# fbreitwieser/krakenuniq

Hardware: AMD Instinct MI355X
Metric: Mreads/s (150 bp) (higher is better)
Workload: dtype u64

## Files before the change

krakenuniq_amd/csrc/ku_api.cpp:

```cpp
#include "ku_build.h"
#include "ku_ctx.h"

static thread_local std::string g_last_error;
void ku_set_error(const std::string &s) { g_last_error = s; }

extern "C" const char *ku_strerror(int status) {
  switch (status) {
    case KU_OK: return "ok";
    case KU_EINVAL: return "invalid argument";
    case KU_EDATA: return "malformed database / index / taxonomy data";
    case KU_ENOINPUT: return "cannot open input";
    case KU_ENOMEM: return "out of memory";
    case KU_EHIP: return "HIP runtime error or no usable gfx950 device";
    case KU_ESTATE: return "call order violated";
    case KU_EUNSUP: return "not supported by this build";
    default: return "unknown status";
  }
}
extern "C" const char *ku_last_error(void) { return g_last_error.c_str(); }
extern "C" int ku_abi_version(void) { return KU_ABI_VERSION; }
extern "C" int ku_device_count(void) {
  int n = 0;
  if (hipGetDeviceCount(&n) != hipSuccess) return 0;
  return n;
// ... 151 lines not shown
  return n <= cap ? KU_OK : fail(KU_EINVAL, "ku_db_chunk_plan: bounds array too small");
}

int ku_db_raw(const ku_db *db, const uint8_t **pairs, const uint64_t **offsets) {
  if (!db || !pairs || !offsets) return KU_EINVAL;
  *pairs = db->pairs;
  *offsets = db->offsets;
  return KU_OK;
}

extern "C" int ku_db_values(const ku_db *db, uint32_t *out, uint64_t *n) {
  if (!db || !n) return fail(KU_EINVAL, "ku_db_values: null argument");
  std::lock_guard<std::mutex> lk(db->values_mu);
  if (!db->values_ready) {
    const uint64_t np = db->info.key_ct, ps = db->info.key_len + 4, kl = db->info.key_len;
    constexpr uint32_t SMALL = 1u << 26;
    std::vector<std::atomic<uint64_t>> bits(SMALL / 64);
    for (auto &w : bits) w.store(0, std::memory_order_relaxed);
    unsigned nthr = std::max(1u, std::min(16u, std::thread::hardware_concurrency()));
    if (np < (1u << 20)) nthr = 1;
    std::vector<std::vector<uint32_t>> large(nthr);
    std::vector<std::thread> team;
    for (unsigned t = 0; t < nthr; ++t)
      team.emplace_back([&, t] {
        const uint64_t lo = np * t / nthr, hi = np * (t + 1) / nthr;
        uint32_t last = 0;
        for (uint64_t i = lo; i < hi; ++i) {
          uint32_t v;
          memcpy(&v, db->pairs + i * ps + kl, 4);
          if (v == last) continue;
          last = v;
          if (v >= SMALL) {
            large[t].push_back(v);
            if (large[t].size() >= (1u << 20)) {
              std::sort(large[t].begin(), large[t].end());
              large[t].erase(std::unique(large[t].begin(), large[t].end()), large[t].end());
            }
            continue;
          }
          std::atomic<uint64_t> &w = bits[v >> 6];
          const uint64_t m = 1ull << (v & 63);
          if (!(w.load(std::memory_order_relaxed) & m)) w.fetch_or(m, std::memory_order_relaxed);
        }
      });
    for (auto &th : team) th.join();
    std::vector<uint32_t> &vals = db->values;
    for (uint64_t wi = 0; wi < bits.size(); ++wi) {
      uint64_t w = bits[wi].load(std::memory_order_relaxed);
      if (wi == 0) w &= ~1ull;
      while (w) {
        vals.push_back((uint32_t)(wi * 64 + (uint64_t)__builtin_ctzll(w)));
        w &= w - 1;
      }
    }
    const size_t n_small = vals.size();
    for (auto &l : large) vals.insert(vals.end(), l.begin(), l.end());
    std::sort(vals.begin() + n_small, vals.end());
    vals.erase(std::unique(vals.begin() + n_small, vals.end()), vals.end());
    db->values_ready = true;
  }
  const uint64_t count = db->values.size();
  if (out) {
    if (count > *n) return fail(KU_EINVAL, "ku_db_values: output array too small");
    memcpy(out, db->values.data(), count * 4);
  }
  *n = count;
  return KU_OK;
}

extern "C" int ku_tax_open(const char *path, ku_tax **out) {
  if (!path || !out) return fail(KU_EINVAL, "ku_tax_open: null argument");
  *out = nullptr;
  FILE *f = fopen(path, "r");
  if (!f) return fail(KU_ENOINPUT, std::string("unable to open taxonomy index file ") + path);
  ku_tax *t = new ku_tax();
  char *line = nullptr;
  size_t lcap = 0;
  ssize_t ll;
  while ((ll = getline(&line, &lcap, f)) > 0) {
    if (line[ll - 1] == '\n') line[--ll] = 0;
    if (ll == 0) continue;
    char *p = line, *end;
    unsigned long id = strtoul(p, &end, 10);
    if (end == p) continue;
    p = end;
    unsigned long par = strtoul(p, &end, 10);
    if (end == p) continue;
    p = end;
    if (*p) ++p;
    char *tab = strchr(p, '\t');
    std::string name, rank;
    if (tab) { name.assign(p, tab - p); rank.assign(tab + 1); } else name.assign(p);
    if ((uint32_t)id > 1 && id == par) {
      free(line); fclose(f); delete t;
      return fail(KU_EDATA, "taxDB: the parent of " + std::to_string(id) + " is itself");
    }
    t->add((uint32_t)id, (uint32_t)par, name, rank);
  }
  free(line);
  fclose(f);
  t->add(0, 0, "unclassified", "no rank");
  t->finish();
  *out = t;
  return KU_OK;
}

extern "C" int ku_tax_from_arrays(const uint32_t *ids, const uint32_t *parents, uint64_t n, ku_tax **out) {
  if (!out || (n && (!ids || !parents))) return fail(KU_EINVAL, "ku_tax_from_arrays: null argument");
  ku_tax *t = new ku_tax();
  for (uint64_t i = 0; i < n; ++i) t->add(ids[i], parents[i], "", "");
  t->add(0, 0, "unclassified", "no rank");
  t->finish();
  *out = t;
  return KU_OK;
}
extern "C" void ku_tax_close(ku_tax *t) { delete t; }
extern "C" uint64_t ku_tax_size(const ku_tax *t) { return t ? t->ids.size() : 0; }
extern "C" int ku_tax_ids(const ku_tax *t, uint32_t *ids) {
  if (!t || (!ids && !t->ids.empty())) return fail(KU_EINVAL, "ku_tax_ids: null argument");
  if (!t->ids.empty()) memcpy(ids, t->ids.data(), t->ids.size() * 4);
  return KU_OK;
}
extern "C" uint32_t ku_tax_parent(const ku_tax *t, uint32_t taxid) {
  if (!t || taxid == 0) return KU_AMBIG;
  auto it = t->row.find(taxid);
  return it == t->row.end() ? KU_AMBIG : t->parent_map[it->second];
}

hipStream_t ku_ctx_stream_of(ku_ctx *ctx) { return ctx->stream; }
unsigned long long *ku_ctx_exact_unique_of(ku_ctx *ctx) { return ctx->d_exact_unique; }
int ku_ctx_device_of(const ku_ctx *ctx) { return ctx->device; }
int ku_ctx_cus_of(const ku_ctx *ctx) { return ctx->n_cu; }
uint32_t ku_ctx_k_of(const ku_ctx *ctx) { return ctx->m.db.k; }

int ctx_activate(ku_ctx *ctx) {
  if (hipSetDevice(ctx->device) != hipSuccess) return fail(KU_EHIP, "hipSetDevice failed");
  return KU_OK;
}

extern "C" int ku_ctx_create(int device, ku_ctx **out) {
  if (!out) return fail(KU_EINVAL, "ku_ctx_create: null argument");
  *out = nullptr;
  KU_TRY(ku_check_device(device));
  hipDeviceProp_t prop;
  HIP_TRY(hipGetDeviceProperties(&prop, device));
  if (strncmp(prop.gcnArchName, "gfx950", 6) != 0)
    return fail(KU_EHIP, std::string("device is ") + prop.gcnArchName + ", this library is built for gfx950 only");
  ku_ctx *ctx = new ku_ctx();
  ctx->device = device;
  ctx->n_cu = prop.multiProcessorCount > 0 ? prop.multiProcessorCount : 256;
  HIP_TRY(hipSetDevice(device));
  HIP_TRY(hipStreamCreateWithFlags(&ctx->stream, hipStreamNonBlocking));
  HIP_TRY(hipMalloc((void **)&ctx->d_scalar, 128));
  if (const char *e = getenv("KU_LAYOUT")) ctx->hash_layout = strcmp(e, "sorted") != 0;
  if (const char *e = getenv("KU_LOAD_FACTOR")) {
    double f = atof(e);
    if (f >= 0.05 && f <= 0.9) { ctx->load_factor = f; ctx->load_factor_set = true; }
  }
  *out = ctx;
  return KU_OK;
}

void store_free(DbStore &d) {
  if (d.d_table) (void)hipFree(d.d_table);
  if (d.db_owned && d.d_pairs) (void)hipFree(d.d_pairs);
  if (d.offsets_owned && d.d_offsets) (void)hipFree(d.d_offsets);
  d = DbStore{};
}
void ctx_drop_count_cache(ku_ctx *ctx) {
  ctx->count_cache.clear();
  ctx->count_cache_store = ctx->count_cache_pairs = nullptr;
  ctx->count_cache_lines = 0;
}
static void ctx_free_db(ku_ctx *ctx) {
  ctx_drop_count_cache(ctx);
  if (ctx->pf.valid) store_free(ctx->pf.store);
  ctx->pf.valid = false;
  store_free(ctx->m);
  for (DbStore &e : ctx->extra) store_free(e);
  ctx->extra.clear();
  ctx->db_loaded = false;
}
void ctx_free_sparse(ku_ctx *ctx) {
  KuSparseDev &d = ctx->sp.dev;
  for (void *p : {(void *)d.l_key, (void *)d.l_first, (void *)d.u_key, (void *)d.u_distinct, (void *)d.u_last, (void *)d.u_maxfirst,
                  (void *)d.g_key, (void *)d.dense, (void *)d.err, (void *)ctx->sp.d_counters})
    if (p) (void)hipFree(p);
  for (DevBuf *b : {&ctx->sp.unit, &ctx->sp.carry_l, &ctx->sp.carry_u, &ctx->sp.out, &ctx->sp.u_cnt, &ctx->sp.u_flag, &ctx->sp.list, &ctx->sp.tail_row,
                    &ctx->sp.t_seqs, &ctx->sp.t_off, &ctx->sp.t_len, &ctx->sp.t_taxa, &ctx->sp.t_unit})
    b->release();
  ctx->sp = ku_ctx::Sparse{};
}
int sparse_give_up(ku_ctx *ctx, hipStream_t also) {
  (void)ctx_sync_all_streams(ctx);
  if (also) (void)hipStreamSynchronize(also);
  (void)hipGetLastError();
  ctx_free_sparse(ctx);
  ctx->sp.gave_up = true;
  return KU_OK;
}
static void ctx_free_tax(ku_ctx *ctx) {
  for (uint32_t **p : {&ctx->d_node_parent, &ctx->d_node_slot, &ctx->d_node_taxid, &ctx->d_slot_node, &ctx->d_slot_taxid,
                       &ctx->d_slot_anc_off, &ctx->d_slot_anc}) {
    if (*p) (void)hipFree(*p);
    *p = nullptr;
  }
  if (ctx->cnt.registers) (void)hipFree(ctx->cnt.registers);
  if (ctx->cnt.hll_floor) (void)hipFree(ctx->cnt.hll_floor);
  if (ctx->cnt.n_kmers) (void)hipFree(ctx->cnt.n_kmers);
  if (ctx->cnt.n_reads) (void)hipFree(ctx->cnt.n_reads);
  if (ctx->d_exact_set) (void)hipFree(ctx->d_exact_set);
  if (ctx->d_exact_unique) (void)hipFree(ctx->d_exact_unique);
  ctx->d_exact_set = ctx->d_exact_unique = nullptr;
  ctx->exact_mask = 0;
  ctx_free_sparse(ctx);
  ctx->cnt = KuCountsDev{};
  ctx->tax_set = false;
}

int ctx_sync_all_streams(ku_ctx *ctx) {
  int st = KU_OK;
  for (hipStream_t s : {ctx->stream, ctx->k_streams[0], ctx->k_streams[1], ctx->h2d_stream, ctx->d2h_stream, ctx->fetch_stream, ctx->pf.stream})
    if (s && hipStreamSynchronize(s) != hipSuccess && st == KU_OK) st = fail(KU_EHIP, "ku_ctx_synchronize: a stream of the context failed");
  return st;
}

extern "C" void ku_ctx_destroy(ku_ctx *ctx) {
  if (!ctx) return;
  rle_times_print();
  (void)hipSetDevice(ctx->device);
  (void)ctx_sync_all_streams(ctx);
  ctx_free_db(ctx);
  ctx_free_tax(ctx);
  for (DevBuf *b : {&ctx->b_seqs, &ctx->b_off, &ctx->b_len, &ctx->b_calls, &ctx->b_taxa, &ctx->b_hits, &ctx->b_ws, &ctx->b_runs,
                    &ctx->b_roff, &ctx->b_rcnt})
    b->release();
  if (ctx->d_scalar) (void)hipFree(ctx->d_scalar);
  if (ctx->pf.d_scalar) (void)hipFree(ctx->pf.d_scalar);
  if (ctx->pf.stream) (void)hipStreamDestroy(ctx->pf.stream);
  for (RleJob &j : ctx->rle) j.release();
  if (ctx->h2d_stream) (void)hipStreamDestroy(ctx->h2d_stream);
  if (ctx->d2h_stream) (void)hipStreamDestroy(ctx->d2h_stream);
  for (hipStream_t &ks : ctx->k_streams) if (ks) { (void)hipStreamDestroy(ks); ks = nullptr; }
  if (ctx->main_ev) (void)hipEventDestroy(ctx->main_ev);
  if (ctx->fetch_stream) (void)hipStreamDestroy(ctx->fetch_stream);
  if (ctx->stream) (void)hipStreamDestroy(ctx->stream);
  delete ctx;
}

static int store_scan_values(ku_ctx *ctx, DbStore &d) {
  d.values.clear();
  uint32_t *d_bitmap = nullptr, *d_list = nullptr, *d_count = ctx->d_scalar;
  const uint32_t cap = 1u << 24;
  HIP_TRY(hipMalloc((void **)&d_bitmap, 1ull << 29));
  if (hipMalloc((void **)&d_list, (size_t)cap * 4) != hipSuccess) { (void)hipFree(d_bitmap); return fail(KU_ENOMEM, "hipMalloc values list"); }
  int st = KU_OK;
  uint32_t count = 0;
  if (hipMemsetAsync(d_bitmap, 0, 1ull << 29, ctx->stream) != hipSuccess ||
      hipMemsetAsync(d_count, 0, 4, ctx->stream) != hipSuccess)
    st = fail(KU_EHIP, "memset failed");
  if (st == KU_OK) st = ku_launch_mark_values(d.d_pairs, d.db.n_pairs, d_bitmap, ctx->stream);
  if (st == KU_OK) st = ku_launch_collect_values(d_bitmap, d_list, cap, d_count, ctx->stream);
  if (st == KU_OK && hipMemcpyAsync(&count, d_count, 4, hipMemcpyDeviceToHost, ctx->stream) != hipSuccess) st = fail(KU_EHIP, "memcpy failed");
  if (st == KU_OK && hipStreamSynchronize(ctx->stream) != hipSuccess) st = fail(KU_EHIP, "value scan kernel failed");
  if (st == KU_OK && count > cap) st = fail(KU_EUNSUP, "more than 2^24 distinct taxids in the database");
  if (st == KU_OK) {
    d.values.resize(count);
    if (count && hipMemcpy(d.values.data(), d_list, (size_t)count * 4, hipMemcpyDeviceToHost) != hipSuccess) st = fail(KU_EHIP, "memcpy failed");
    std::sort(d.values.begin(), d.values.end());
    if (!d.values.empty() && d.values[0] == 0) d.values.erase(d.values.begin());
  }
  (void)hipFree(d_bitmap);
  (void)hipFree(d_list);
  return st;
}

static void fill_db_dev(DbStore &d, uint64_t n_pairs, uint64_t pair_base, uint32_t k, uint32_t nt, uint32_t idx_type,
                        uint64_t bin_lo, uint64_t bin_hi) {
  d.db.pairs = d.d_pairs;
  d.db.table = nullptr;
  d.db.n_lines = 0;
  d.db.offsets = d.d_offsets;
  d.db.pair_base = pair_base;
  d.db.n_pairs = n_pairs;
  d.db.bin_lo = bin_lo;
  d.db.bin_hi = bin_hi;
  d.db.k = k;
  d.db.nt = nt;
  d.db.xor_mask = idx_type == 1 ? 0u : ku_index2_xor_mask(nt);
}

int store_upload(ku_ctx *ctx, DbStore &d, const ku_db *db, uint64_t bin_lo, uint64_t bin_hi, bool scan_values, hipStream_t stream) {
  if (!stream) stream = ctx->stream;
  const uint64_t p0 = db->offsets[bin_lo], p1 = db->offsets[bin_hi], np = p1 - p0;
  const uint32_t kl = db->info.key_len, ps = kl + 4;
  HIP_TRY(hipMalloc((void **)&d.d_pairs, std::max<uint64_t>(np, 1) * 12));
  d.db_owned = true;
  if (kl == 8) {
    if (np) HIP_TRY(hipMemcpy(d.d_pairs, db->pairs + p0 * 12, np * 12, hipMemcpyHostToDevice));
  } else if (np) {
    void *d_raw = nullptr;
    HIP_TRY(hipMalloc(&d_raw, np * ps));
    hipError_t e = hipMemcpy(d_raw, db->pairs + p0 * ps, np * ps, hipMemcpyHostToDevice);
    int st = e == hipSuccess ? ku_launch_repack((const uint8_t *)d_raw, np, kl, d.d_pairs, stream) : KU_EHIP;
    if (st == KU_OK && hipStreamSynchronize(stream) != hipSuccess) st = KU_EHIP;
    (void)hipFree(d_raw);
    if (st != KU_OK) return fail(st, "pair repack failed");
  }
  const uint64_t no = bin_hi - bin_lo + 1;
  HIP_TRY(hipMalloc((void **)&d.d_offsets, no * 8));
  d.offsets_owned = true;
  HIP_TRY(hipMemcpy(d.d_offsets, db->offsets + bin_lo, no * 8, hipMemcpyHostToDevice));
  fill_db_dev(d, np, p0, db->info.k, db->info.nt, db->info.idx_type, bin_lo, bin_hi);
  return scan_values ? store_scan_values(ctx, d) : KU_OK;
}

extern "C" int ku_ctx_load_db(ku_ctx *ctx, const ku_db *db, uint64_t bin_lo, uint64_t bin_hi) {
  if (!ctx || !db) return fail(KU_EINVAL, "ku_ctx_load_db: null argument");
  KU_TRY(rle_idle(ctx, "ku_ctx_load_db"));
  if (bin_lo > bin_hi || bin_hi > db->info.n_bins) return fail(KU_EINVAL, "bin range out of bounds");
  KU_TRY(ctx_activate(ctx));
  ctx_free_tax(ctx);
  ctx_free_db(ctx);
  KU_TRY(store_upload(ctx, ctx->m, db, bin_lo, bin_hi));
  ctx->db_loaded = true;
  return KU_OK;
}

bool store_whole(const DbStore &d) { return d.db.bin_lo == 0 && d.db.bin_hi == (1ull << (2 * d.db.nt)); }

extern "C" int ku_ctx_add_db(ku_ctx *ctx, const ku_db *db) {
  if (!ctx || !db) return fail(KU_EINVAL, "ku_ctx_add_db: null argument");
  KU_TRY(rle_idle(ctx, "ku_ctx_add_db"));
  if (!ctx->db_loaded) return fail(KU_ESTATE, "load the first database before adding further ones");
  if (ctx->tax_set) return fail(KU_ESTATE, "add every database before the taxonomy is set");
  if (db->info.k != ctx->m.db.k)
    return fail(KU_EINVAL, "different k-mer sizes in the databases: " + std::to_string(ctx->m.db.k) + " vs " + std::to_string(db->info.k));
  if (!store_whole(ctx->m)) return fail(KU_EUNSUP, "hierarchical multi-database runs need the first database resident as a whole");
  if (ctx->extra.size() >= 7) return fail(KU_EUNSUP, "at most 8 databases");
  KU_TRY(ctx_activate(ctx));
  ctx->extra.emplace_back();
  int st = store_upload(ctx, ctx->extra.back(), db, 0, db->info.n_bins);
  if (st != KU_OK) { store_free(ctx->extra.back()); ctx->extra.pop_back(); }
  return st;
}

extern "C" int ku_ctx_adopt_db(ku_ctx *ctx, void *d_pairs, uint64_t n_pairs, const uint64_t *d_offsets, uint32_t k,
                               uint32_t nt, uint32_t idx_type, uint64_t bin_lo, uint64_t bin_hi) {
  if (!ctx || (!d_pairs && n_pairs) || !d_offsets) return fail(KU_EINVAL, "ku_ctx_adopt_db: null argument");
  KU_TRY(rle_idle(ctx, "ku_ctx_adopt_db"));
  if (k < 1 || k > 31 || nt < 1 || nt > 15 || nt > k || (idx_type != 1 && idx_type != 2) || bin_lo > bin_hi ||
      bin_hi > (1ull << (2 * nt)))
    return fail(KU_EINVAL, "ku_ctx_adopt_db: bad geometry");
  KU_TRY(ctx_activate(ctx));
  ctx_free_tax(ctx);
  ctx_free_db(ctx);
  ctx->m.d_pairs = (uint32_t *)d_pairs;
  ctx->m.d_offsets = const_cast<uint64_t *>(d_offsets);
  uint64_t pair_base = 0;
  HIP_TRY(hipMemcpy(&pair_base, d_offsets, 8, hipMemcpyDeviceToHost));
  fill_db_dev(ctx->m, n_pairs, pair_base, k, nt, idx_type, bin_lo, bin_hi);
  ctx->db_loaded = true;
  return store_scan_values(ctx, ctx->m);
}

extern "C" int ku_ctx_db_layout(ku_ctx *ctx, uint32_t *is_hash, uint64_t *resident_bytes) {
  if (!ctx) return fail(KU_EINVAL, "null context");
  if (!ctx->db_loaded) return fail(KU_ESTATE, "no database loaded");
  const bool hash = ctx->m.db.table != nullptr;
  if (is_hash) *is_hash = hash ? 1u : 0u;
  if (resident_bytes)
    *resident_bytes = (hash ? ctx->m.db.n_lines * 128 : ctx->m.db.n_pairs * 12) + (ctx->m.db.bin_hi - ctx->m.db.bin_lo + 1) * 8;
  return KU_OK;
}

static std::vector<uint32_t> ctx_all_values(const ku_ctx *ctx) {
  std::vector<uint32_t> v(ctx->m.values);
  for (const DbStore &e : ctx->extra) v.insert(v.end(), e.values.begin(), e.values.end());
  std::sort(v.begin(), v.end());
  v.erase(std::unique(v.begin(), v.end()), v.end());
  return v;
}

extern "C" int ku_ctx_db_values(ku_ctx *ctx, uint32_t *out, uint64_t *n) {
  if (!ctx || !n) return fail(KU_EINVAL, "ku_ctx_db_values: null argument");
  if (!ctx->db_loaded) return fail(KU_ESTATE, "no database loaded");
  const std::vector<uint32_t> v = ctx_all_values(ctx);
  if (out) {
    if (*n < v.size()) return fail(KU_EINVAL, "output array too small");
    if (!v.empty()) memcpy(out, v.data(), v.size() * 4);
// ... 294 lines not shown
```

krakenuniq_amd/csrc/ku_api_classify.cpp:

```cpp
#include "ku_ctx.h"

int check_ready(ku_ctx *ctx) {
  if (!ctx) return fail(KU_EINVAL, "null context");
  if (!ctx->db_loaded) return fail(KU_ESTATE, "no database loaded");
  if (!ctx->tax_set) return fail(KU_ESTATE, "taxonomy not set");
  return ctx_activate(ctx);
}

extern "C" int ku_lookup_device(ku_ctx *ctx, const void *d_seqs, uint64_t n_bytes, const ku_opts *opts,
                                uint32_t *d_taxa, void *stream) {
  KU_TRY(check_ready(ctx));
  KU_TRY(rle_idle(ctx, "ku_lookup_device"));
  if (n_bytes && (!d_seqs || !d_taxa)) return fail(KU_EINVAL, "ku_lookup_device: null buffer");
  const uint32_t flags = opts ? opts->flags : 0;
  const bool counts = !(flags & (KU_F_NO_COUNTS | KU_F_QUICK));
  hipStream_t s = stream ? (hipStream_t)stream : ctx->stream;
  const size_t nd = 1 + ctx->extra.size();
  for (size_t i = 0; i < nd; ++i) {
    const DbStore &d = i ? ctx->extra[i - 1] : ctx->m;
    int st = ku_launch_lookup(d.db, ctx->cnt, (const uint8_t *)d_seqs, n_bytes, d_taxa, counts && i + 1 == nd, i > 0,
                              (flags & KU_F_MERGE_CHUNK) != 0, ctx->n_cu, s);
    if (st != KU_OK) return fail(st, "lookup kernel launch failed");
  }
  return KU_OK;
}

int ku_ctx_route_info(const ku_ctx *ctx, uint64_t *bin_lo, uint64_t *bin_hi, int *is_hash, int *single_db) {
  if (!ctx || !ctx->db_loaded || !ctx->tax_set) return fail(KU_ESTATE, "no database / taxonomy on this context");
  if (bin_lo) *bin_lo = ctx->m.db.bin_lo;
  if (bin_hi) *bin_hi = ctx->m.db.bin_hi;
  if (is_hash) *is_hash = ctx->m.db.table != nullptr;
  if (single_db) *single_db = ctx->extra.empty();
  return KU_OK;
}
int ku_ctx_route_scan(ku_ctx *ctx, const void *d_seqs, uint64_t n_bytes, uint32_t *d_taxa, const KuRouteDev &rt, hipStream_t s) {
  KU_TRY(check_ready(ctx));
  int st = ku_launch_route_scan(ctx->m.db, (const uint8_t *)d_seqs, n_bytes, d_taxa, rt, ctx->n_cu, s);
  return st == KU_OK ? KU_OK : fail(st, "route scan kernel launch failed");
}
int ku_ctx_route_resolve_prepare(ku_ctx *ctx, const ku_opts *opts, hipStream_t s) {
  KU_TRY(check_ready(ctx));
  const uint32_t flags = opts ? opts->flags : 0;
  const uint32_t max_len = opts ? opts->max_read_len : 0;
  if (max_len == 0 || (flags & (KU_F_QUICK | KU_F_KEEP_SLOTS)) || getenv("KU_NO_FUSED")) return KU_EUNSUP;
  const uint32_t max_n = ku_max_kmers(ctx->m.db.k, max_len);
  if (max_n > ku_route_resolve_max_kmers()) return KU_EUNSUP;
  if (max_n > 128) {
    const uint64_t ws = ku_short_workspace_bytes(std::max(max_n, 193u), ctx->tax.n_slots, ~0ull >> 8, ctx->n_cu);
    if (ws > ctx->b_ws.cap) {
      HIP_TRY(hipStreamSynchronize(s));
      if (ctx->b_ws.reserve(ws) != KU_OK) { (void)hipGetLastError(); return KU_EUNSUP; }
    }
  }
  return KU_OK;
}
int ku_ctx_route_resolve(ku_ctx *ctx, const uint64_t *d_off, const uint32_t *d_len, uint64_t n_reads, const ku_opts *opts, uint32_t *d_calls,
                         uint32_t *d_taxa, uint32_t *d_hits, const uint32_t *d_kb, const uint32_t *d_ret, hipStream_t s) {
  const uint32_t flags = opts ? opts->flags : 0;
  const uint32_t max_len = opts ? opts->max_read_len : 0;
  const uint32_t max_n = ku_max_kmers(ctx->m.db.k, max_len);
  int st = ku_launch_route_resolve(ctx->m.db, ctx->tax, ctx->cnt, d_off, d_len, n_reads, max_n, flags, d_calls, d_taxa, d_hits, d_kb, d_ret,
                                   ctx->b_ws.p, ctx->b_ws.cap, ctx->n_cu, s);
  return st == KU_OK ? KU_OK : fail(st, "routed resolve kernel launch failed");
}
int ku_ctx_route_owner(ku_ctx *ctx, const void *d_rec, uint64_t n_rec, const uint32_t *d_kb, uint32_t *d_slots, bool do_counts, hipStream_t s) {
  KU_TRY(check_ready(ctx));
  int st = ku_launch_route_owner(ctx->m.db, ctx->cnt, d_rec, n_rec, d_kb, d_slots, do_counts, ctx->n_cu, s);
  return st == KU_OK ? KU_OK : fail(st, "route owner kernel launch failed");
}

int ku_exact_owned_step(ku_ctx *ctx, const void *d_seqs, const uint64_t *d_off, const uint32_t *d_len, uint64_t n_reads, uint64_t n_bytes,
                        const ku_opts *opts, uint32_t *d_taxa, hipStream_t s) {
  KU_TRY(check_ready(ctx));
  if (!ctx->d_exact_set) return fail(KU_ESTATE, "exact counting is not enabled on this context");
  if (!ctx->extra.empty()) return fail(KU_EUNSUP, "exact counting on a shard goes with one database");
  ku_opts o = opts ? *opts : ku_opts{0, 1, 0, 0};
  if (o.flags & (KU_F_QUICK | KU_F_NO_COUNTS)) return fail(KU_EUNSUP, "exact counting goes with the plain classification only");
  o.flags |= KU_F_KEEP_SLOTS | KU_F_MERGE_CHUNK;
  HIP_TRY(hipMemsetAsync(d_taxa, 0xFE, n_bytes * 4, s));
  KU_TRY(ku_lookup_device(ctx, d_seqs, n_bytes, &o, d_taxa, s));
  int st = ku_launch_exact(ctx->m.db.k, (const uint8_t *)d_seqs, d_off, d_len, n_reads, d_taxa, ctx->d_exact_set, ctx->exact_mask,
                           ctx->d_exact_unique, ctx->d_scalar + 6, ctx->n_cu, s);
  if (st != KU_OK) return fail(st, "exact counting kernel launch failed");
  return ku_launch_replace_u32(d_taxa, n_bytes, KU_FOREIGN_MARK, 0u, s);
}

extern "C" int ku_lookup_stats_device(ku_ctx *ctx, const void *d_seqs, uint64_t n_bytes, uint64_t *stats_out,
                                      void *stream) {
  KU_TRY(check_ready(ctx));
  KU_TRY(rle_idle(ctx, "ku_lookup_stats_device"));
  if (!stats_out || (n_bytes && !d_seqs)) return fail(KU_EINVAL, "ku_lookup_stats_device: null argument");
  hipStream_t s = stream ? (hipStream_t)stream : ctx->stream;
  unsigned long long *d_stats = (unsigned long long *)(ctx->d_scalar + 8);
  HIP_TRY(hipMemsetAsync(d_stats, 0, 32, s));
  int st = ku_launch_lookup_stats(ctx->m.db, (const uint8_t *)d_seqs, n_bytes, d_stats, ctx->n_cu, s);
  if (st != KU_OK) return fail(st, "stats kernel launch failed");
  HIP_TRY(hipMemcpyAsync(stats_out, d_stats, 32, hipMemcpyDeviceToHost, s));
  HIP_TRY(hipStreamSynchronize(s));
  return KU_OK;
}

extern "C" int ku_resolve_device(ku_ctx *ctx, const void *d_seqs, const uint64_t *d_seq_off, const uint32_t *d_seq_len,
                                 uint64_t n_reads, const ku_opts *opts, uint32_t *d_calls, uint32_t *d_taxa,
                                 uint32_t *d_hits, void *stream) {
  KU_TRY(check_ready(ctx));
  KU_TRY(rle_idle(ctx, "ku_resolve_device"));
  if (n_reads && (!d_seq_off || !d_seq_len || !d_calls || !d_taxa)) return fail(KU_EINVAL, "ku_resolve_device: null buffer");
  const uint32_t flags = opts ? opts->flags : 0;
  if ((flags & KU_F_QUICK) && !d_seqs) return fail(KU_EINVAL, "quick mode needs the sequence buffer");
  hipStream_t s = stream ? (hipStream_t)stream : ctx->stream;
  uint32_t max_len = opts ? opts->max_read_len : 0;
  if (max_len == 0 && n_reads) {
    KU_TRY(ku_launch_max_len(d_seq_len, n_reads, ctx->d_scalar + 4, s));
    HIP_TRY(hipMemcpyAsync(&max_len, ctx->d_scalar + 4, 4, hipMemcpyDeviceToHost, s));
    HIP_TRY(hipStreamSynchronize(s));
  }
  uint64_t ws = (flags & KU_F_QUICK) ? 0 : ku_resolve_workspace_bytes(max_len, ctx->m.db.k, ctx->n_cu);
  if (ws > ctx->b_ws.cap) {
    HIP_TRY(hipStreamSynchronize(s));
    if (ctx->b_ws.reserve(ws) != KU_OK) return fail(KU_ENOMEM, "resolve workspace allocation failed");
  }
  if (ws) HIP_TRY(hipMemsetAsync(ctx->b_ws.p, 0, ws, s));
  int st = ku_launch_resolve(ctx->m.db, ctx->tax, ctx->cnt, (const uint8_t *)d_seqs, d_seq_off, d_seq_len, n_reads, flags,
                             opts ? opts->min_hits : 1, max_len, d_calls, d_taxa, d_hits, ctx->b_ws.p, ctx->b_ws.cap,
                             ctx->n_cu, s);
  return st == KU_OK ? KU_OK : fail(st, "resolve kernel launch failed");
}

int classify_device_impl(ku_ctx *ctx, const void *d_seqs, uint64_t n_bytes, const uint64_t *d_seq_off,
                                const uint32_t *d_seq_len, uint64_t n_reads, const ku_opts *opts, uint32_t *d_calls,
                                uint32_t *d_taxa, uint32_t *d_hits, void *stream, const uint64_t *h_off, const uint32_t *h_len) {
  KU_TRY(check_ready(ctx));
  const uint32_t flags = opts ? opts->flags : 0;
  const bool exact = ctx->d_exact_set != nullptr;
  if (exact && !store_whole(ctx->m)) return fail(KU_EUNSUP, "exact counting on a shard runs through the multi-GPU driver (ku_mgpu_enable_exact)");
  if (exact && (flags & (KU_F_KEEP_SLOTS | KU_F_NO_COUNTS)))
    return fail(KU_EUNSUP, "exact counting goes with a whole classification (no slot output / count-less runs)");
  const bool sparse = ctx->sp.on && !(flags & KU_F_NO_COUNTS);
  if (sparse && !h_len) return fail(KU_EUNSUP, "the sparse-mode emulation runs through the host-buffer entry points (it needs the read lengths on the host)");
  if (sparse && (flags & KU_F_KEEP_SLOTS)) return fail(KU_EUNSUP, "the sparse-mode emulation does not combine with slot output");
  const uint32_t short_max = (getenv("KU_NO_FUSED") || !ctx->extra.empty() || exact || sparse) ? 0 : ku_short_max_kmers(ctx->m.db);
  if (short_max && !(flags & (KU_F_QUICK | KU_F_KEEP_SLOTS)) && n_reads) {
    if (!d_seqs || !d_seq_off || !d_seq_len || !d_calls || !d_taxa) return fail(KU_EINVAL, "ku_classify_batch_device: null buffer");
    hipStream_t s = stream ? (hipStream_t)stream : ctx->stream;
    uint32_t max_len = opts ? opts->max_read_len : 0;
    if (max_len == 0) {
      KU_TRY(ku_launch_max_len(d_seq_len, n_reads, ctx->d_scalar + 4, s));
      HIP_TRY(hipMemcpyAsync(&max_len, ctx->d_scalar + 4, 4, hipMemcpyDeviceToHost, s));
      HIP_TRY(hipStreamSynchronize(s));
    }
    const uint32_t max_n = ku_max_kmers(ctx->m.db.k, max_len);
    bool fused = max_n <= short_max;
    if (!fused && max_n <= ku_short_max_kmers_windowed(ctx->m.db) && !getenv("KU_NO_WINDOWED")) {
      const uint64_t ws = ku_short_workspace_bytes(max_n, ctx->tax.n_slots, n_reads, ctx->n_cu);
      if (ws > ctx->b_ws.cap) HIP_TRY(hipStreamSynchronize(s));
      fused = ctx->b_ws.reserve(ws) == KU_OK;
      if (!fused) (void)hipGetLastError();
    }
    if (fused) {
      int st = ku_launch_classify_short(ctx->m.db, ctx->tax, ctx->cnt, (const uint8_t *)d_seqs, n_bytes, d_seq_off, d_seq_len,
                                        n_reads, max_n, flags, d_calls, d_taxa, d_hits, ctx->b_ws.p, ctx->b_ws.cap, ctx->n_cu, s);
      return st == KU_OK ? KU_OK : fail(st, "fused short-read kernel launch failed");
    }
    ku_opts o = opts ? *opts : ku_opts{0, 1, 0, 0};
    o.max_read_len = max_len;
    KU_TRY(ku_lookup_device(ctx, d_seqs, n_bytes, &o, d_taxa, stream));
    return ku_resolve_device(ctx, d_seqs, d_seq_off, d_seq_len, n_reads, &o, d_calls, d_taxa, d_hits, stream);
  }
  KU_TRY(ku_lookup_device(ctx, d_seqs, n_bytes, opts, d_taxa, stream));
  if (sparse && n_reads) {
    int st = sparse_pass(ctx, d_seqs, d_seq_off, d_seq_len, h_off, h_len, n_reads, n_bytes, d_taxa,
                         (flags & KU_F_QUICK) ? std::max(1u, opts ? opts->min_hits : 1u) : 0u, stream ? (hipStream_t)stream : ctx->stream);
    if (st == KU_ENOMEM) {
      sparse_give_up(ctx, (hipStream_t)stream);
    } else if (st != KU_OK) return st;
  }
  if (exact) {
    if (n_reads && (!d_seqs || !d_seq_off || !d_seq_len || !d_taxa)) return fail(KU_EINVAL, "ku_classify_batch_device: null buffer");
    int st = ku_launch_exact(ctx->m.db.k, (const uint8_t *)d_seqs, d_seq_off, d_seq_len, n_reads, d_taxa, ctx->d_exact_set,
                             ctx->exact_mask, ctx->d_exact_unique, ctx->d_scalar + 6, ctx->n_cu,
                             stream ? (hipStream_t)stream : ctx->stream,
                             (flags & KU_F_QUICK) ? std::max(1u, opts ? opts->min_hits : 1u) : 0u);
    if (st != KU_OK) return fail(st, "exact counting kernel launch failed");
  }
  return ku_resolve_device(ctx, d_seqs, d_seq_off, d_seq_len, n_reads, opts, d_calls, d_taxa, d_hits, stream);
}

extern "C" int ku_classify_batch_device(ku_ctx *ctx, const void *d_seqs, uint64_t n_bytes, const uint64_t *d_seq_off,
                                        const uint32_t *d_seq_len, uint64_t n_reads, const ku_opts *opts,
                                        uint32_t *d_calls, uint32_t *d_taxa, uint32_t *d_hits, void *stream) {
  if (ctx) KU_TRY(rle_idle(ctx, "ku_classify_batch_device"));
  return classify_device_impl(ctx, d_seqs, n_bytes, d_seq_off, d_seq_len, n_reads, opts, d_calls, d_taxa, d_hits, stream, nullptr, nullptr);
}

extern "C" int ku_classify_batch(ku_ctx *ctx, const char *seqs, uint64_t n_bytes, const uint64_t *seq_off,
                                 const uint32_t *seq_len, uint64_t n_reads, const ku_opts *opts, uint32_t *calls,
                                 uint32_t *taxa, uint32_t *hits) {
  KU_TRY(check_ready(ctx));
  KU_TRY(rle_idle(ctx, "ku_classify_batch"));
  if ((n_bytes && !seqs) || (n_reads && (!seq_off || !seq_len || !calls))) return fail(KU_EINVAL, "ku_classify_batch: null buffer");
  if (n_reads == 0) return KU_OK;
  ku_opts o = opts ? *opts : ku_opts{0, 1, 0, 0};
  if (o.max_read_len == 0) for (uint64_t i = 0; i < n_reads; ++i) o.max_read_len = std::max(o.max_read_len, seq_len[i]);
  for (uint64_t i = 0; i < n_reads; ++i)
    if (seq_off[i] + seq_len[i] > n_bytes) return fail(KU_EINVAL, "read " + std::to_string(i) + " exceeds the sequence buffer");
  if (ctx->b_seqs.reserve(n_bytes + 16) || ctx->b_off.reserve(n_reads * 8) || ctx->b_len.reserve(n_reads * 4) ||
      ctx->b_calls.reserve(n_reads * 4) || ctx->b_taxa.reserve((n_bytes + 16) * 4) || ctx->b_hits.reserve(n_reads * 4))
    return fail(KU_ENOMEM, "device batch buffers");
  hipStream_t s = ctx->stream;
  HIP_TRY(hipMemcpyAsync(ctx->b_seqs.p, seqs, n_bytes, hipMemcpyHostToDevice, s));
  HIP_TRY(hipMemcpyAsync(ctx->b_off.p, seq_off, n_reads * 8, hipMemcpyHostToDevice, s));
  HIP_TRY(hipMemcpyAsync(ctx->b_len.p, seq_len, n_reads * 4, hipMemcpyHostToDevice, s));
  KU_TRY(classify_device_impl(ctx, ctx->b_seqs.p, n_bytes, (const uint64_t *)ctx->b_off.p, (const uint32_t *)ctx->b_len.p,
                              n_reads, &o, (uint32_t *)ctx->b_calls.p, (uint32_t *)ctx->b_taxa.p,
                              (uint32_t *)ctx->b_hits.p, s, seq_off, seq_len));
  HIP_TRY(hipMemcpyAsync(calls, ctx->b_calls.p, n_reads * 4, hipMemcpyDeviceToHost, s));
  if (taxa) HIP_TRY(hipMemcpyAsync(taxa, ctx->b_taxa.p, n_bytes * 4, hipMemcpyDeviceToHost, s));
  if (hits) HIP_TRY(hipMemcpyAsync(hits, ctx->b_hits.p, n_reads * 4, hipMemcpyDeviceToHost, s));
  HIP_TRY(hipStreamSynchronize(s));
  return KU_OK;
}

int rle_and_fetch(ku_ctx *ctx, const uint32_t *d_taxa, const uint64_t *d_off, const uint32_t *d_len, uint64_t n_reads,
                         uint64_t runs_cap, bool quick, uint32_t *calls, uint32_t *hits, uint64_t *run_off,
                         uint32_t *run_cnt, uint64_t *n_runs) {
  hipStream_t s = ctx->stream;
  unsigned long long *d_counter = (unsigned long long *)(ctx->d_scalar + 2);
  if (quick) {
    HIP_TRY(hipMemsetAsync(d_counter, 0, 8, s));
    HIP_TRY(hipMemsetAsync(ctx->b_roff.p, 0, n_reads * 8, s));
    HIP_TRY(hipMemsetAsync(ctx->b_rcnt.p, 0, n_reads * 4, s));
  } else {
    KU_TRY(ku_launch_rle(d_taxa, ctx->m.db.k, d_off, d_len, n_reads, runs_cap , ctx->b_runs.p, runs_cap, d_counter,
                         (uint64_t *)ctx->b_roff.p, (uint32_t *)ctx->b_rcnt.p, ctx->n_cu, s));
  }
  unsigned long long total = 0;
  HIP_TRY(hipMemcpyAsync(&total, d_counter, 8, hipMemcpyDeviceToHost, s));
  HIP_TRY(hipMemcpyAsync(calls, ctx->b_calls.p, n_reads * 4, hipMemcpyDeviceToHost, s));
  if (hits) HIP_TRY(hipMemcpyAsync(hits, ctx->b_hits.p, n_reads * 4, hipMemcpyDeviceToHost, s));
  HIP_TRY(hipMemcpyAsync(run_off, ctx->b_roff.p, n_reads * 8, hipMemcpyDeviceToHost, s));
  HIP_TRY(hipMemcpyAsync(run_cnt, ctx->b_rcnt.p, n_reads * 4, hipMemcpyDeviceToHost, s));
  HIP_TRY(hipStreamSynchronize(s));
  if (total > runs_cap) return fail(KU_EHIP, "run-length encoder overflowed its bound");
  *n_runs = ctx->n_runs = total;
  ctx->fetch_runs_src = ctx->b_runs.p;
  ctx->last_calls_dev = ctx->b_calls.p;
  return KU_OK;
}
```

krakenuniq_amd/csrc/ku_api_rle.cpp:

```cpp
#include "ku_ctx.h"


static int sparse_tail_insert(ku_ctx *ctx, const KuSparseDev &d, const std::vector<char> &text, const std::vector<uint32_t> &lens,
                              uint32_t unit, hipStream_t s, uint32_t *pos_end) {
  ku_ctx::Sparse &sp = ctx->sp;
  const uint64_t n_reads = lens.size(), n_bytes = text.size();
  if (pos_end) *pos_end = (uint32_t)n_bytes;
  if (n_reads == 0) return KU_OK;
  std::vector<uint64_t> off(n_reads);
  uint64_t at = 0;
  for (uint64_t r = 0; r < n_reads; ++r) { off[r] = at; at += (uint64_t)lens[r] + 1; }
  if (at != n_bytes) return fail(KU_ESTATE, "sparse-mode emulation: the open unit's reads are inconsistent");
  if (sp.t_seqs.reserve(n_bytes + 16) || sp.t_off.reserve(n_reads * 8) || sp.t_len.reserve(n_reads * 4) || sp.t_taxa.reserve((n_bytes + 16) * 4) ||
      sp.t_unit.reserve(n_reads * 4))
    return fail(KU_ENOMEM, "device memory for the open work unit's reads");
  HIP_TRY(hipMemcpyAsync(sp.t_seqs.p, text.data(), n_bytes, hipMemcpyHostToDevice, s));
  HIP_TRY(hipMemcpyAsync(sp.t_off.p, off.data(), n_reads * 8, hipMemcpyHostToDevice, s));
  HIP_TRY(hipMemcpyAsync(sp.t_len.p, lens.data(), n_reads * 4, hipMemcpyHostToDevice, s));
  std::vector<uint32_t> units(n_reads, unit);
  HIP_TRY(hipMemcpyAsync(sp.t_unit.p, units.data(), n_reads * 4, hipMemcpyHostToDevice, s));
  HIP_TRY(hipStreamSynchronize(s));
  int st = ku_launch_lookup(ctx->m.db, ctx->cnt, (const uint8_t *)sp.t_seqs.p, n_bytes, (uint32_t *)sp.t_taxa.p, false, false, false,
                            ctx->n_cu, s);
  if (st != KU_OK) return fail(st, "lookup kernel launch failed");
// ... 58 lines not shown
    HIP_TRY(hipMemcpyAsync(&c, sp.d_counters, 8, hipMemcpyDeviceToHost, s));
    HIP_TRY(hipMemcpyAsync(&err, sp.dev.err, 4, hipMemcpyDeviceToHost, s));
    HIP_TRY(hipStreamSynchronize(s));
    if (err) return fail(KU_ENOMEM, "sparse-mode emulation: a device table is full");
    sp.g_count = c;
  }
  sp.tail_open = false;
  sp.tail_text.clear();
  sp.tail_len.clear();
  return KU_OK;
}

struct RleTimes {
  double t[10] = {};
  double x[6] = {};
  double kernel_ms = 0;
  double kernel_sum_ms = 0, cover_end = 0;
  unsigned long long reads = 0;
  static inline const bool on = getenv("KU_RLE_TIMES") != nullptr;
  static inline hipEvent_t ref = nullptr;
  static double now() { timespec ts; clock_gettime(CLOCK_MONOTONIC, &ts); return (double)ts.tv_sec + 1e-9 * (double)ts.tv_nsec; }
  struct Lap {
    double &slot;
    const double t0 = on ? now() : 0.0;
    ~Lap() { if (on) slot += now() - t0; }
  };
  void count_finish() { if (on) t[4] += 1; }
  void count_exact_pass(double units, double n_reads) { if (on) { x[2] += 1; x[3] += units; x[4] += n_reads; } }
  void add_kernels(hipEvent_t k0, hipEvent_t k1, uint64_t n_reads) {
    float ms = 0, a = 0, b = 0;
    if (ref && hipEventElapsedTime(&ms, k0, k1) == hipSuccess && hipEventElapsedTime(&a, ref, k0) == hipSuccess &&
        hipEventElapsedTime(&b, ref, k1) == hipSuccess) {
      kernel_sum_ms += ms;
      kernel_ms += std::max(0.0, (double)b - std::max((double)a, cover_end));
      cover_end = std::max(cover_end, (double)b);
      reads += n_reads;
    } else (void)hipGetLastError();
  }
  void print() const {
    if (on && t[4] > 0)
      fprintf(stderr, "ku_classify_batch_rle over %.0f batches: checks %.3f s, plan + enqueue %.3f s, waiting for the device %.3f s, behind the wait %.3f s; "
                      "kernels %.3f ms for %llu reads (HIP events on their streams: the time the batches' intervals cover; their sum is %.3f ms); of the enqueue: buffers + plan %.3f s, uploads %.3f s, launches %.3f s, "
                      "copies back + events %.3f s; of buffers + plan: room in the emulation's run-wide set %.3f s\n",
              t[4], t[0], t[1], t[2], t[3], kernel_ms, reads, kernel_sum_ms, t[5], t[6], t[7], t[8], t[9]);
    if (on && x[2] > 0)
      fprintf(stderr, "ku_classify_batch_rle, behind the wait: flagging again %.3f s, %.0f exact passes over %.0f work units (%.0f reads) %.3f s, of it %.3f s waiting for their kernels\n", x[0], x[2],
              x[3], x[4], x[1], x[5]);
  }
};
static RleTimes g_rle;
void rle_times_print() { g_rle.print(); }

static int sparse_fast_exact(ku_ctx *ctx, RleJob &j, const std::vector<uint32_t> &flagged, const std::vector<uint8_t> &flag_all,
                             bool last_is_open, hipStream_t s) {
  ku_ctx::Sparse &sp = ctx->sp;
  const uint32_t *h_len = j.b.seq_len;
  const std::vector<uint64_t> &unit_first_read = j.unit_first_read;
  const uint32_t *d_u_cnt = (const uint32_t *)j.u_cnt.p;
  const void *d_runs = j.runs_in_ctx ? ctx->b_runs.p : j.runs.p;
  const uint64_t *d_roff = (const uint64_t *)(j.runs_in_ctx ? ctx->b_roff.p : j.roff.p);
  const uint32_t *d_rcnt = (const uint32_t *)(j.runs_in_ctx ? ctx->b_rcnt.p : j.rcnt.p);
  const bool with_tail = j.cont_tail && !flagged.empty() && flagged[0] == 0 && !j.tail_len.empty();
  const uint64_t tail_bytes = with_tail ? j.tail_text.size() : 0;
  size_t at = 0;
  bool first_pass = true;
  while (at < flagged.size()) {
    size_t end = at;
    uint64_t bases = first_pass ? tail_bytes : 0, n_list = 0;
    while (end < flagged.size() && end - at < KU_SPARSE_MAX_UNITS) {
      const uint32_t u = flagged[end];
      uint64_t ub = 0;
      for (uint64_t r = unit_first_read[u]; r < unit_first_read[u + 1]; ++r) ub += h_len[r];
      if (end > at && bases + ub > (1ull << 25)) break;
      bases += ub;
      n_list += unit_first_read[u + 1] - unit_first_read[u];
      ++end;
    }
    const bool has_open = last_is_open && end == flagged.size();
    std::vector<uint32_t> list(3 * n_list);
    uint64_t li = 0;
    for (size_t f = at; f < end; ++f) {
      const uint32_t u = flagged[f];
      for (uint64_t r = unit_first_read[u]; r < unit_first_read[u + 1]; ++r, ++li) {
        list[li] = (uint32_t)r;
        list[n_list + li] = (uint32_t)(f - at) | (flag_all[f] ? 0x80000000u : 0u);
        list[2 * n_list + li] = u;
      }
    }
    if (sp.list.reserve(std::max<uint64_t>(n_list, 1) * 12) != KU_OK) return fail(KU_ENOMEM, "device memory for the flagged work units' reads");
    KU_TRY(sparse_reserve_global(ctx, bases + sp.n_carry_l, s));
    KuSparseDev d;
    KU_TRY(sparse_pass_tables(ctx, bases + sp.n_carry_l + sp.n_carry_u, &d, s));
    if (first_pass && j.cont_carry)
      KU_TRY(ku_launch_sparse_carry_in(d, (const unsigned long long *)sp.carry_l.p, sp.n_carry_l, (const uint32_t *)sp.carry_u.p, sp.n_carry_u, s));
    uint32_t pos_base = 0;
    if (first_pass && with_tail) KU_TRY(sparse_tail_insert(ctx, d, j.tail_text, j.tail_len, 0u, s, &pos_base));
    if (n_list) HIP_TRY(hipMemcpyAsync(sp.list.p, list.data(), n_list * 12, hipMemcpyHostToDevice, s));
    const uint32_t *dl = (const uint32_t *)sp.list.p;
    KU_TRY(ku_launch_sparse_insert_runs(d, ctx->m.db.k, (const uint8_t *)j.seqs.p, (const uint64_t *)j.off.p, (const uint32_t *)j.len.p,
                                        dl, dl + n_list, dl + 2 * n_list, n_list, d_runs, d_roff, d_rcnt, ctx->d_slot_taxid, ctx->tax.n_slots,
                                        d_u_cnt, ctx->n_cu, s, pos_base));
    const uint32_t n_local = (uint32_t)(end - at);
    KU_TRY(ku_launch_sparse_close(d, has_open ? n_local - 1 : n_local, s, !j.cont_carry));
    if (first_pass && j.cont_carry) sp.n_carry_l = sp.n_carry_u = 0;
    unsigned long long c[3] = {0, 0, 0};
    if (has_open) {
      HIP_TRY(hipMemsetAsync(sp.d_counters + 1, 0, 16, s));
      KU_TRY(ku_launch_sparse_carry_out(d, n_local - 1, (unsigned long long *)sp.carry_l.p, (uint32_t *)sp.carry_u.p, sp.d_counters + 1,
                                        sp.cap_carry_l, sp.cap_carry_u, s));
    }
    HIP_TRY(hipMemcpyAsync(c, sp.d_counters, 24, hipMemcpyDeviceToHost, s));
    { RleTimes::Lap lap{g_rle.x[5]}; HIP_TRY(hipStreamSynchronize(s)); }
    sp.g_count = std::max<uint64_t>(sp.g_count, c[0]);
    if (has_open) {
      sp.n_carry_l = std::min<uint64_t>(c[1], sp.cap_carry_l);
      sp.n_carry_u = std::min<uint64_t>(c[2], sp.cap_carry_u);
    }
    first_pass = false;
    at = end;
  }
  return KU_OK;
}

static bool rle_fused_eligible(ku_ctx *ctx, uint32_t flags, uint32_t max_n, uint64_t n_bytes, uint64_t n_reads, bool monotonic) {
  if (getenv("KU_NO_FUSED") || getenv("KU_NO_FUSED_RLE") || !ctx->extra.empty() || ctx->d_exact_set) return false;
  if (flags & (KU_F_QUICK | KU_F_KEEP_SLOTS)) return false;
  const uint32_t short_max = ku_short_max_kmers(ctx->m.db);
  if (!short_max) return false;
  if (max_n > short_max && (max_n > ku_short_max_kmers_windowed(ctx->m.db) || getenv("KU_NO_WINDOWED"))) return false;
  if (n_reads >= (1ull << 32)) return false;
  const bool sparse = ctx->sp.on && !(flags & KU_F_NO_COUNTS);
  if (sparse) {
    const ku_ctx::Sparse &sp = ctx->sp;
    if (getenv("KU_NO_SPARSE_FAST") || !monotonic || sp.unit_nt == 0 || sp.unit_nt > (1ull << 24) || n_bytes + (1ull << 26) >= (1ull << 32)) return false;
    const uint64_t max_units = n_bytes / sp.unit_nt + 2;
    if (max_units * ctx->tax.n_slots > (1ull << 29)) return false;
  }
  return true;
}

static uint64_t rle_workspace_bytes(const ku_ctx *ctx, uint32_t max_n, uint64_t n_reads) {
  if (max_n <= ku_short_max_kmers(ctx->m.db) || max_n > ku_short_max_kmers_windowed(ctx->m.db)) return 0;
  return ku_short_workspace_bytes(max_n, ctx->tax.n_slots, n_reads, ctx->n_cu);
}

struct RlePlan {
  std::vector<uint64_t> seg;
  uint64_t total_waves = 0;
  uint32_t chunk = 0;
  uint64_t runs_cap = 0;
  uint64_t ws = 0;
  uint64_t n_seg() const { return seg.size() - 1; }
};
static RlePlan rle_plan(const ku_ctx *ctx, uint64_t n_bytes, uint64_t n_reads, uint32_t max_n, const uint64_t *seq_off, bool test_hook) {
  RlePlan p;
  uint64_t n_seg = 1;
  constexpr uint64_t seg_bytes = 16ull << 20;
  if (seq_off && !getenv("KU_NO_H2D_OVERLAP")) n_seg = std::min<uint64_t>(8, std::max<uint64_t>(1, n_bytes / seg_bytes));
  p.seg.assign(n_seg + 1, 0);
  for (uint64_t g = 1; g < n_seg; ++g) {
    const uint64_t target = n_bytes / n_seg * g;
    p.seg[g] = std::max<uint64_t>(p.seg[g - 1], (uint64_t)(std::lower_bound(seq_off, seq_off + n_reads, target) - seq_off));
  }
  p.seg[n_seg] = n_reads;
  uint64_t max_seg_reads = 0;
  for (uint64_t g = 0; g < n_seg; ++g) {
    p.total_waves += ku_short_grid_waves(p.seg[g + 1] - p.seg[g], max_n, ctx->n_cu);
    max_seg_reads = std::max(max_seg_reads, p.seg[g + 1] - p.seg[g]);
  }
  const uint64_t reads_per_wave = n_reads / std::max<uint64_t>(p.total_waves, 1);
  p.chunk = reads_per_wave >= 64 ? 256u : (reads_per_wave >= 16 ? 64u : 16u);
  p.runs_cap = n_bytes / 6 + 4 * n_reads + p.total_waves * p.chunk + 4096;
  if (const char *e = test_hook ? getenv("KU_RUNS_CAP") : nullptr) p.runs_cap = std::max<uint64_t>(1, (uint64_t)atoll(e));
  p.ws = rle_workspace_bytes(ctx, max_n, max_seg_reads);
  return p;
}

int rle_idle(const ku_ctx *ctx, const char *who) {
  if (ctx->rle_in_flight) return fail(KU_ESTATE, std::string(who) + ": batches are in flight (ku_classify_batch_rle_finish first)");
  return KU_OK;
}

extern "C" uint64_t ku_device_rle_runs_cap(const ku_ctx *ctx, uint64_t n_bytes, uint64_t n_reads, uint32_t max_read_len) {
  if (!ctx || !ctx->tax_set) return 0;
  return rle_plan(ctx, n_bytes, n_reads, ku_max_kmers(ctx->m.db.k, max_read_len), nullptr, false).runs_cap;
}

extern "C" int ku_classify_batch_device_rle(ku_ctx *ctx, const void *d_seqs, uint64_t n_bytes, const uint64_t *d_seq_off,
                                            const uint32_t *d_seq_len, uint64_t n_reads, const ku_opts *opts, uint32_t *d_calls,
                                            ku_run *d_runs, uint64_t runs_cap, uint64_t *d_run_off, uint32_t *d_run_cnt,
                                            uint64_t *d_n_runs, void *stream) {
  KU_TRY(check_ready(ctx));
  KU_TRY(rle_idle(ctx, "ku_classify_batch_device_rle"));
  if (!d_n_runs || (n_reads && (!d_seqs || !d_seq_off || !d_seq_len || !d_calls || !d_runs || !d_run_off || !d_run_cnt)))
    return fail(KU_EINVAL, "ku_classify_batch_device_rle: null buffer");
  const ku_opts o = opts ? *opts : ku_opts{0, 1, 0, 0};
  hipStream_t s = stream ? (hipStream_t)stream : ctx->stream;
  HIP_TRY(hipMemsetAsync(d_n_runs, 0, 8, s));
  if (n_reads == 0) return KU_OK;
  if (o.max_read_len == 0) return fail(KU_EINVAL, "ku_classify_batch_device_rle: opts->max_read_len (the longest read of the batch) is required");
  const uint32_t max_n = ku_max_kmers(ctx->m.db.k, o.max_read_len);
  if (ctx->sp.on && !(o.flags & KU_F_NO_COUNTS))
    return fail(KU_EUNSUP, "the sparse-mode emulation runs through the host-buffer entry points (it needs the read lengths on the host)");
  if (!store_whole(ctx->m) || !rle_fused_eligible(ctx, o.flags, max_n, n_bytes, n_reads, true))
    return fail(KU_EUNSUP, "ku_classify_batch_device_rle: the fused kernel does not apply to this context / these options (ku_classify_batch_device does)");
  const RlePlan p = rle_plan(ctx, n_bytes, n_reads, max_n, nullptr, false);
  if (p.ws > ctx->b_ws.cap) HIP_TRY(hipStreamSynchronize(s));
  if (ctx->b_ws.reserve(p.ws)) return fail(KU_ENOMEM, "device memory for the windowed kernel's workspace");
  KuRunsOut ro{};
  ro.runs = (uint2 *)d_runs;
  ro.counter = (unsigned long long *)d_n_runs;
  ro.cap = runs_cap;
  ro.chunk = p.chunk;
  ro.run_off = d_run_off;
  ro.run_cnt = d_run_cnt;
  if (p.total_waves * p.chunk <= runs_cap && p.total_waves * p.chunk < (1ull << 31)) {
    HIP_TRY(hipMemsetD32Async((hipDeviceptr_t)d_n_runs, (int)(p.total_waves * p.chunk), 1, s));
    ro.pre_base1 = 1;
  }
  int st = ku_launch_classify_short(ctx->m.db, ctx->tax, ctx->cnt, (const uint8_t *)d_seqs, n_bytes, d_seq_off, d_seq_len, n_reads, max_n, o.flags,
                                    d_calls, nullptr, nullptr, ctx->b_ws.p, ctx->b_ws.cap, ctx->n_cu, s, &ro, nullptr);
  return st == KU_OK ? KU_OK : fail(st, "fused kernel launch failed");
}


static int plan_work_units(ku_ctx *ctx, RleJob &j, const RleBatch &b, bool sparse) {
  const ku_ctx::Sparse &sp = ctx->sp;
  j.sparse = sparse;
  j.cont_carry = j.cont_tail = j.open_after = false;
  j.n_units = 0;
  j.kmers = 0;
  j.unit_first_read.clear();
  j.tail_text.clear();
  j.tail_len.clear();
  if (!sparse) return KU_OK;
  if (j.pin_unit.reserve(b.n_reads * 4)) return fail(KU_ENOMEM, "page-locked memory for the work-unit plan");
  uint32_t *h_unit = (uint32_t *)j.pin_unit.p;
  uint64_t acc = sp.acc_nt;
  uint32_t cur = 0;
  j.cont_carry = sp.open;
  j.cont_tail = sp.tail_open && !sp.open;
  j.unit_first_read.push_back(0);
  for (uint64_t r = 0; r < b.n_reads; ++r) {
    h_unit[r] = cur;
    acc += b.seq_len[r];
    if (acc >= sp.unit_nt) { ++cur; acc = 0; j.unit_first_read.push_back(r + 1); }
  }
  j.open_after = acc > 0;
  j.acc_after = acc;
  j.n_units = cur + (j.unit_first_read.back() < b.n_reads ? 1u : 0u);
  if (j.unit_first_read.back() < b.n_reads) j.unit_first_read.push_back(b.n_reads);
  for (uint64_t r = 0; r < b.n_reads; ++r) j.kmers += ku_max_kmers(ctx->m.db.k, b.seq_len[r]);
  return KU_OK;
}

static int sparse_fast_view(ku_ctx *ctx, RleJob &j, KuSparseFast *sf) {
  ku_ctx::Sparse &sp = ctx->sp;
  uint64_t in_flight_kmers = 0;
  for (const RleJob &q : ctx->rle) if (q.busy && &q != &j && q.sparse) in_flight_kmers += q.kmers;
  { RleTimes::Lap lap{g_rle.t[9]}; KU_TRY(sparse_reserve_global(ctx, j.kmers + in_flight_kmers + sp.n_carry_l, ctx->stream)); }
  sf->g_key = sp.dev.g_key;
  sf->g_mask = sp.dev.g_mask;
  sf->g_count = sp.dev.g_count;
  sf->dense = sp.dev.dense;
  sf->u_cnt = (uint32_t *)j.u_cnt.p;
  sf->err = sp.dev.err;
  sf->n_slots = ctx->tax.n_slots;
  sf->unit_base = 0;
  ctx->m.seen_dirty = true;
  return KU_OK;
}

static int queue_uploads_and_launches(ku_ctx *ctx, RleJob &j, const RleBatch &b, const RlePlan &p, hipStream_t s, KuSparseFast *sf, bool *clock_started) {
  const bool sparse = sf != nullptr;
  unsigned long long *h_tot = (unsigned long long *)j.pin.p;
  const uint32_t *h_unit = (const uint32_t *)j.pin_unit.p;
  HIP_TRY(hipEventRecord(ctx->main_ev, ctx->stream));
  HIP_TRY(hipStreamWaitEvent(s, ctx->main_ev, 0));
  unsigned long long *d_counter = j.d_counter;
  if (sparse) {
    if (ku_launch_zero3(d_counter, 2, j.u_cnt.p, std::max<uint64_t>((uint64_t)j.n_units * ctx->tax.n_slots, 1), j.u_flag.p,
                        ((uint64_t)std::max<uint32_t>(j.n_units, 1) + 3) / 4, s) != KU_OK)
      return fail(KU_EHIP, "clearing the batch counters failed");
  }
  h_tot[3] = p.total_waves * (unsigned long long)p.chunk;
  HIP_TRY(hipMemcpyAsync(d_counter, &h_tot[3], 8, hipMemcpyHostToDevice, s));
  KuRunsOut ro{};
  ro.runs = (uint2 *)j.runs.p;
  ro.counter = d_counter;
  ro.cap = p.runs_cap;
  ro.chunk = p.chunk;
  if (RleTimes::on) { KU_TRY(ensure_event(j.t_k0, hipEventDefault)); KU_TRY(ensure_event(j.t_k1, hipEventDefault)); }
  uint64_t waves_before = 0;
  for (uint64_t g = 0; g < p.n_seg(); ++g) {
    const uint64_t a = p.seg[g], e = p.seg[g + 1];
    const uint64_t lo = g == 0 ? 0 : b.seq_off[a], hi = g + 1 == p.n_seg() ? b.n_bytes : b.seq_off[e];
    hipStream_t cs = ctx->h2d_stream;
    {
      RleTimes::Lap lap{g_rle.t[6]};
      if (hi > lo) HIP_TRY(hipMemcpyAsync((char *)j.seqs.p + lo, b.seqs + lo, hi - lo, hipMemcpyHostToDevice, cs));
      if (e > a) {
        HIP_TRY(hipMemcpyAsync((uint64_t *)j.off.p + a, b.seq_off + a, (e - a) * 8, hipMemcpyHostToDevice, cs));
        HIP_TRY(hipMemcpyAsync((uint32_t *)j.len.p + a, b.seq_len + a, (e - a) * 4, hipMemcpyHostToDevice, cs));
        if (sparse) HIP_TRY(hipMemcpyAsync((uint32_t *)j.unit.p + a, h_unit + a, (e - a) * 4, hipMemcpyHostToDevice, cs));
      }
      HIP_TRY(hipEventRecord(j.seg_events[g], cs));
      HIP_TRY(hipStreamWaitEvent(s, j.seg_events[g], 0));
    }
    if (e == a) continue;
    RleTimes::Lap lap{g_rle.t[7]};
    ro.run_off = (uint64_t *)j.roff.p + a;
    ro.run_cnt = (uint32_t *)j.rcnt.p + a;
    ro.pre_base1 = (uint32_t)(1 + waves_before);
    waves_before += ku_short_grid_waves(e - a, b.max_n, ctx->n_cu);
    if (sparse) sf->unit_of = (const uint32_t *)j.unit.p + a;
    if (RleTimes::on && !*clock_started) {
      if (!RleTimes::ref) { KU_TRY(ensure_event(RleTimes::ref, hipEventDefault)); HIP_TRY(hipEventRecord(RleTimes::ref, s)); }
      HIP_TRY(hipEventRecord(j.t_k0, s));
      *clock_started = true;
    }
    int st = ku_launch_classify_short(ctx->m.db, ctx->tax, ctx->cnt, (const uint8_t *)j.seqs.p, b.n_bytes, (const uint64_t *)j.off.p + a,
                                      (const uint32_t *)j.len.p + a, e - a, b.max_n, b.o.flags, (uint32_t *)j.calls.p + a, nullptr, nullptr,
                                      j.ws.p, j.ws.cap, ctx->n_cu, s, &ro, sf);
    if (st != KU_OK) { (void)hipStreamSynchronize(ctx->h2d_stream); (void)hipStreamSynchronize(s); return fail(st, "fused kernel launch failed"); }
  }
  return KU_OK;
}

static int queue_open_unit_step(ku_ctx *ctx, RleJob &j, hipStream_t s) {
  ku_ctx::Sparse &sp = ctx->sp;
  if (ctx->prev_kernels_done) HIP_TRY(hipStreamWaitEvent(s, ctx->prev_kernels_done, 0));
  if (j.cont_tail && j.n_units)
    KU_TRY(ku_launch_add_u32((uint32_t *)j.u_cnt.p, (const uint32_t *)sp.tail_row.p, ctx->tax.n_slots, s));
  KU_TRY(ku_launch_sparse_flag_units((const uint32_t *)j.u_cnt.p, (uint64_t)j.n_units * ctx->tax.n_slots, ctx->tax.n_slots, sp.dev.dense,
                                     (uint8_t *)j.u_flag.p, s));
  if (j.open_after && !(j.cont_carry && j.n_units == 1))
    HIP_TRY(hipMemcpyAsync(sp.tail_row.p, (const uint32_t *)j.u_cnt.p + (size_t)(j.n_units - 1) * ctx->tax.n_slots, (size_t)ctx->tax.n_slots * 4,
                           hipMemcpyDeviceToDevice, s));
  return KU_OK;
}

static int queue_copies_back(ku_ctx *ctx, RleJob &j, const RleBatch &b, uint64_t runs_cap, hipStream_t s) {
  unsigned long long *h_tot = (unsigned long long *)j.pin.p;
  const hipStream_t ds = ctx->d2h_stream;
  HIP_TRY(hipEventRecord(j.kernels_done, s));
  ctx->prev_kernels_done = j.kernels_done;
  HIP_TRY(hipStreamWaitEvent(ds, j.kernels_done, 0));
  HIP_TRY(hipMemcpyAsync(b.calls, j.calls.p, b.n_reads * 4, hipMemcpyDeviceToHost, ds));
  HIP_TRY(hipMemcpyAsync(b.run_off, j.roff.p, b.n_reads * 8, hipMemcpyDeviceToHost, ds));
  HIP_TRY(hipMemcpyAsync(b.run_cnt, j.rcnt.p, b.n_reads * 4, hipMemcpyDeviceToHost, ds));
  HIP_TRY(hipMemcpyAsync(&h_tot[0], j.d_counter, 8, hipMemcpyDeviceToHost, ds));
  j.runs_copied = b.runs ? std::min<uint64_t>(b.runs_cap, runs_cap) : 0;
  if (j.runs_copied) HIP_TRY(hipMemcpyAsync(b.runs, j.runs.p, j.runs_copied * 8, hipMemcpyDeviceToHost, ds));
  if (j.sparse) {
    HIP_TRY(hipMemcpyAsync((uint8_t *)j.pin.p + 64, j.u_flag.p, std::max<uint32_t>(j.n_units, 1), hipMemcpyDeviceToHost, ds));
    HIP_TRY(hipMemcpyAsync(&h_tot[1], ctx->sp.dev.g_count, 8, hipMemcpyDeviceToHost, ds));
    HIP_TRY(hipMemcpyAsync(&h_tot[2], ctx->sp.dev.err, 4, hipMemcpyDeviceToHost, ds));
  }
  HIP_TRY(hipEventRecord(j.done, ds));
  return KU_OK;
}

static void advance_emulation_state(ku_ctx::Sparse &sp, RleJob &j, const RleBatch &b) {
  const bool whole_batch_one_open_unit = j.n_units == 1 && j.open_after;
  if (j.cont_tail && !whole_batch_one_open_unit) {
    j.tail_text.swap(sp.tail_text);
    j.tail_len.swap(sp.tail_len);
    sp.tail_text.clear();
    sp.tail_len.clear();
  }
  if (j.cont_carry && whole_batch_one_open_unit) {
  } else if (j.open_after) {
    if (!(j.cont_tail && whole_batch_one_open_unit)) { sp.tail_text.clear(); sp.tail_len.clear(); }
    sparse_tail_append(sp, b.seqs, b.seq_off, b.seq_len, j.unit_first_read[j.n_units - 1], b.n_reads);
    sp.tail_open = true;
    sp.open = false;
  } else {
    sp.tail_open = false;
    sp.open = false;
    sp.tail_text.clear();
    sp.tail_len.clear();
  }
  sp.acc_nt = j.acc_after;
}

static int rle_job_enqueue(ku_ctx *ctx, RleJob &j, const RleBatch &b) {
  RleTimes::Lap lap_all{g_rle.t[1]};
  hipStream_t &ks = ctx->k_streams[(&j - &ctx->rle[0]) & 1];
  KU_TRY(ensure_stream(ks));
  KU_TRY(ensure_event(ctx->main_ev));
  const hipStream_t s = ks;
  const bool sparse = ctx->sp.on && !(b.o.flags & KU_F_NO_COUNTS);
  RlePlan p;
  KuSparseFast sf{};
  {
    RleTimes::Lap lap{g_rle.t[5]};
    p = rle_plan(ctx, b.n_bytes, b.n_reads, b.max_n, b.monotonic ? b.seq_off : nullptr, true);
    KU_TRY(plan_work_units(ctx, j, b, sparse));
    KU_TRY(j.reserve(b.n_bytes, b.n_reads, p.runs_cap, p.ws, p.n_seg(), sparse, j.n_units, ctx->tax.n_slots));
    KU_TRY(ensure_stream(ctx->h2d_stream));
    KU_TRY(ensure_stream(ctx->d2h_stream));
    if (sparse) {
      if (ctx->sp.tail_row.reserve((size_t)ctx->tax.n_slots * 4)) return fail(KU_ENOMEM, "device memory for the work-unit counters");
      KU_TRY(sparse_fast_view(ctx, j, &sf));
    }
  }
  bool clock_started = false;
  KU_TRY(queue_uploads_and_launches(ctx, j, b, p, s, sparse ? &sf : nullptr, &clock_started));
  {
    RleTimes::Lap lap{g_rle.t[8]};
    if (sparse) KU_TRY(queue_open_unit_step(ctx, j, s));
    if (clock_started) HIP_TRY(hipEventRecord(j.t_k1, s));
    KU_TRY(queue_copies_back(ctx, j, b, p.runs_cap, s));
  }
  if (sparse && j.n_units) advance_emulation_state(ctx->sp, j, b);
  j.b = b;
  j.runs_cap = p.runs_cap;
  j.settled = false;
  j.runs_in_ctx = false;
  j.busy = true;
  return KU_OK;
}

static int rle_job_finish(ku_ctx *ctx, RleJob &j, uint64_t *n_runs, bool *classified) {
  hipStream_t s = ctx->stream;
  *classified = false;
  ctx->last_runs_copied = 0;
  if (j.settled) {
    j.busy = false;
    *n_runs = ctx->n_runs = j.n_runs;
    *classified = true;
    return KU_OK;
  }
  { RleTimes::Lap lap{g_rle.t[2]}; HIP_TRY(hipEventSynchronize(j.done)); }
  RleTimes::Lap lap_rest{g_rle.t[3]};
  g_rle.count_finish();
  if (RleTimes::on && j.t_k0 && j.b.n_reads) g_rle.add_kernels(j.t_k0, j.t_k1, j.b.n_reads);
  j.busy = false;
  ku_ctx::Sparse &sp = ctx->sp;
  const unsigned long long *h_tot = (const unsigned long long *)j.pin.p;
  const uint8_t *h_flag = (const uint8_t *)j.pin.p + 64;
  const unsigned long long total = h_tot[0];
  if (j.b.hits) memset(j.b.hits, 0, j.b.n_reads * 4);
  ctx->last_calls_dev = j.calls.p;
  if (total > j.runs_cap) {
    if (ctx->b_taxa.reserve((j.b.n_bytes + 16) * 4) || ctx->b_runs.reserve((j.b.n_bytes + 1) * 8) || ctx->b_roff.reserve(j.b.n_reads * 8) ||
        ctx->b_rcnt.reserve(j.b.n_reads * 4) || ctx->b_calls.reserve(j.b.n_reads * 4))
      return fail(KU_ENOMEM, "device batch buffers");
    if (ctx->b_ws.reserve(rle_workspace_bytes(ctx, j.b.max_n, j.b.n_reads))) return fail(KU_ENOMEM, "device batch buffers");
    int st = ku_launch_classify_short(ctx->m.db, ctx->tax, ctx->cnt, (const uint8_t *)j.seqs.p, j.b.n_bytes, (const uint64_t *)j.off.p,
                                      (const uint32_t *)j.len.p, j.b.n_reads, j.b.max_n, j.b.o.flags | KU_F_NO_COUNTS, (uint32_t *)ctx->b_calls.p,
                                      (uint32_t *)ctx->b_taxa.p, nullptr, ctx->b_ws.p, ctx->b_ws.cap, ctx->n_cu, s);
    if (st != KU_OK) return fail(st, "fused kernel launch failed");
    KU_TRY(rle_and_fetch(ctx, (const uint32_t *)ctx->b_taxa.p, (const uint64_t *)j.off.p, (const uint32_t *)j.len.p, j.b.n_reads, j.b.n_bytes + 1,
                         false, j.b.calls, nullptr, j.b.run_off, j.b.run_cnt, n_runs));
    j.runs_in_ctx = true;
  } else {
    *n_runs = ctx->n_runs = total;
    ctx->fetch_runs_src = j.runs.p;
    ctx->last_runs_copied = j.runs_copied;
  }
  *classified = true;
  if (j.sparse && sp.on) {
    if ((uint32_t)h_tot[2]) return fail(KU_ENOMEM, "sparse-mode emulation: the run-wide set is full");
    sp.g_count = std::max<uint64_t>(sp.g_count, h_tot[1]);
    std::vector<uint32_t> flagged;
    std::vector<uint8_t> flag_all;
    const bool carry_stays_open = j.cont_carry && j.n_units == 1 && j.open_after;
    bool any_flag = false;
    for (uint32_t u = 0; u < j.n_units; ++u) any_flag |= !(u + 1 == j.n_units && j.open_after) && h_flag[u];
    {
      RleTimes::Lap lap{g_rle.x[0]};
      if (any_flag && !getenv("KU_NO_REFLAG")) {
        KU_TRY(ensure_stream(ctx->fetch_stream));
        hipStream_t fs = ctx->fetch_stream;
        const size_t fb = ((size_t)j.n_units + 3) & ~(size_t)3;
        HIP_TRY(hipMemsetAsync(j.u_flag.p, 0, fb, fs));
        KU_TRY(ku_launch_sparse_flag_units((const uint32_t *)j.u_cnt.p, (uint64_t)j.n_units * ctx->tax.n_slots, ctx->tax.n_slots, sp.dev.dense,
                                           (uint8_t *)j.u_flag.p, fs));
        HIP_TRY(hipMemcpyAsync((uint8_t *)j.pin.p + 64, j.u_flag.p, j.n_units, hipMemcpyDeviceToHost, fs));
        HIP_TRY(hipStreamSynchronize(fs));
      }
      for (uint32_t u = 0; u < j.n_units; ++u) {
        const bool open = u + 1 == j.n_units && j.open_after;
        if (u == 0 && j.cont_carry) { flagged.push_back(u); flag_all.push_back(1); }
        else if (!open && h_flag[u]) { flagged.push_back(u); flag_all.push_back(0); }
      }
    }
    if (!flagged.empty()) {
      RleTimes::Lap lap{g_rle.x[1]};
      for (const RleJob &q : ctx->rle)
        if (q.busy && q.kernels_done) HIP_TRY(hipStreamWaitEvent(s, q.kernels_done, 0));
      KU_TRY(sparse_fast_exact(ctx, j, flagged, flag_all, carry_stays_open, s));
      uint64_t n_flagged_reads = 0;
      for (uint32_t u : flagged) n_flagged_reads += j.unit_first_read[u + 1] - j.unit_first_read[u];
      g_rle.count_exact_pass((double)flagged.size(), (double)n_flagged_reads);
    }
  }
  return KU_OK;
}

int rle_drain_batches(ku_ctx *ctx) {
  for (RleJob &q : ctx->rle)
    if (q.busy && q.done) HIP_TRY(hipEventSynchronize(q.done));
  return KU_OK;
}

static RleJob &rle_next_job(ku_ctx *ctx) {
  RleJob &j = ctx->rle[(ctx->rle_head + ctx->rle_in_flight) % KU_RLE_MAX_IN_FLIGHT];
  static const int counter_at[KU_RLE_MAX_IN_FLIGHT] = {26, 20, 22, 24};
  if (!j.d_counter) j.d_counter = (unsigned long long *)(ctx->d_scalar + counter_at[&j - &ctx->rle[0]]);
  return j;
}

static int rle_check_batch(RleBatch &b) {
  if ((b.n_bytes && !b.seqs) || (b.n_reads && (!b.seq_off || !b.seq_len || !b.calls || !b.run_off || !b.run_cnt)))
    return fail(KU_EINVAL, "ku_classify_batch_rle: null buffer");
  b.o.flags &= ~KU_F_KEEP_SLOTS;
  RleTimes::Lap lap{g_rle.t[0]};
  if (b.o.max_read_len == 0) for (uint64_t i = 0; i < b.n_reads; ++i) b.o.max_read_len = std::max(b.o.max_read_len, b.seq_len[i]);
  b.monotonic = true;
  for (uint64_t i = 0; i < b.n_reads; ++i) {
    if (b.seq_off[i] + b.seq_len[i] > b.n_bytes) return fail(KU_EINVAL, "read " + std::to_string(i) + " exceeds the sequence buffer");
    if (i && b.seq_off[i] < b.seq_off[i - 1] + b.seq_len[i - 1]) b.monotonic = false;
  }
  return KU_OK;
}

static int rle_staged_batch(ku_ctx *ctx, const RleBatch &b, uint64_t *n_runs) {
  const uint64_t n_bytes = b.n_bytes, n_reads = b.n_reads;
  const uint64_t runs_cap = n_bytes + 1;
  if (ctx->b_seqs.reserve(n_bytes + 16) || ctx->b_off.reserve(n_reads * 8) || ctx->b_len.reserve(n_reads * 4) ||
      ctx->b_calls.reserve(n_reads * 4) || ctx->b_taxa.reserve((n_bytes + 16) * 4) || ctx->b_hits.reserve(n_reads * 4) ||
      ctx->b_runs.reserve(runs_cap * 8) || ctx->b_roff.reserve(n_reads * 8) || ctx->b_rcnt.reserve(n_reads * 4))
    return fail(KU_ENOMEM, "device batch buffers");
  hipStream_t s = ctx->stream;
  HIP_TRY(hipMemcpyAsync(ctx->b_seqs.p, b.seqs, n_bytes, hipMemcpyHostToDevice, s));
  HIP_TRY(hipMemcpyAsync(ctx->b_off.p, b.seq_off, n_reads * 8, hipMemcpyHostToDevice, s));
  HIP_TRY(hipMemcpyAsync(ctx->b_len.p, b.seq_len, n_reads * 4, hipMemcpyHostToDevice, s));
  KU_TRY(classify_device_impl(ctx, ctx->b_seqs.p, n_bytes, (const uint64_t *)ctx->b_off.p, (const uint32_t *)ctx->b_len.p,
                              n_reads, &b.o, (uint32_t *)ctx->b_calls.p, (uint32_t *)ctx->b_taxa.p,
                              (uint32_t *)ctx->b_hits.p, s, b.seq_off, b.seq_len));
  return rle_and_fetch(ctx, (const uint32_t *)ctx->b_taxa.p, (const uint64_t *)ctx->b_off.p, (const uint32_t *)ctx->b_len.p, n_reads,
                       runs_cap, (b.o.flags & KU_F_QUICK) != 0, b.calls, b.hits, b.run_off, b.run_cnt, n_runs);
}

static void rle_warm_up(ku_ctx *ctx, uint64_t n_reads) {
  (void)ku_launch_warm_scratch(ctx->n_cu, ctx->stream);
  const RleTimes keep = g_rle;
  const uint64_t wn = (std::min<uint64_t>(std::max<uint64_t>(n_reads, 1), 65536) + 1) & ~1ull, stride = 101;
  const size_t per_slot = (size_t)wn * (4 + 4 + 4 + 8) + (size_t)wn * 8 * 8;
  PinBuf w;
  if (w.reserve((size_t)wn * (stride + 12) + KU_RLE_MAX_IN_FLIGHT * per_slot + 4096) == 0) {
    memset(w.p, 0, w.cap);
    char *text = (char *)w.p;
    uint64_t *w_off = (uint64_t *)(text + ((wn * stride + 63) & ~63ull));
    uint32_t *w_len = (uint32_t *)(w_off + wn);
    char *slots = (char *)(w_len + wn);
    for (uint64_t r = 0; r < wn; ++r) {
      char *t = text + r * stride;
      for (int i = 0; i < 100; ++i) t[i] = "ACGTTGCAAGCTTCGA"[(i * 7 + i / 16 + r) & 15];
      t[100] = '\n';
      w_off[r] = r * stride;
      w_len[r] = 100;
    }
    const ku_opts wo = {KU_F_NO_COUNTS, 1, 100, 0};
    uint64_t w_runs = 0;
    int flying = 0;
    for (int rep = 0; rep < 12; ++rep) {
      if (flying == 3) { (void)ku_classify_batch_rle_finish(ctx, &w_runs); --flying; }
      char *sl = slots + (size_t)(rep % KU_RLE_MAX_IN_FLIGHT) * per_slot;
      uint64_t *roff = (uint64_t *)sl;
      uint32_t *calls = (uint32_t *)(roff + wn), *hits = calls + wn, *rcnt = hits + wn;
      ku_run *runs = (ku_run *)(rcnt + wn);
      if (ku_classify_batch_rle_enqueue(ctx, text, wn * stride, w_off, w_len, wn, &wo, calls, hits, roff, rcnt, runs, wn * 8) == KU_OK) ++flying;
    }
    while (flying-- > 0) (void)ku_classify_batch_rle_finish(ctx, &w_runs);
    if (ctx->fetch_stream) {
      (void)hipMemcpyAsync(w.p, ctx->rle[0].seqs.p, std::min<size_t>(ctx->rle[0].seqs.cap, 1u << 20), hipMemcpyDeviceToHost, ctx->fetch_stream);
      (void)hipStreamSynchronize(ctx->fetch_stream);
    }
    (void)hipDeviceSynchronize();
    w.release();
  }
  (void)hipGetLastError();
  g_rle = keep;
}

extern "C" int ku_classify_batch_rle_reserve(ku_ctx *ctx, uint64_t n_bytes, uint64_t n_reads, uint32_t max_read_len, uint32_t n_jobs) {
  KU_TRY(check_ready(ctx));
  KU_TRY(rle_idle(ctx, "ku_classify_batch_rle_reserve"));
  if (!ku_short_max_kmers(ctx->m.db)) return KU_OK;
  KU_TRY(ensure_stream(ctx->h2d_stream));
  KU_TRY(ensure_stream(ctx->d2h_stream));
  KU_TRY(ensure_stream(ctx->fetch_stream));
  const RlePlan p = rle_plan(ctx, n_bytes, n_reads, ku_max_kmers(ctx->m.db.k, max_read_len), nullptr, false);
  const bool sparse = ctx->sp.on && ctx->sp.unit_nt;
  const uint64_t n_units = sparse ? n_bytes / ctx->sp.unit_nt + 2 : 0;
  for (uint32_t q = 0; q < std::min<uint32_t>(n_jobs, KU_RLE_MAX_IN_FLIGHT); ++q)
    KU_TRY(ctx->rle[q].reserve(n_bytes, n_reads, p.runs_cap, p.ws, 2, sparse, n_units, ctx->tax.n_slots));
  if (sparse && ctx->sp.tail_row.reserve((size_t)ctx->tax.n_slots * 4)) return fail(KU_ENOMEM, "device memory for the work-unit counters");
  if (!getenv("KU_NO_WARMUP")) rle_warm_up(ctx, n_reads);
  return KU_OK;
}

extern "C" int ku_classify_batch_rle_in_flight(const ku_ctx *ctx) { return ctx ? ctx->rle_in_flight : 0; }
extern "C" uint64_t ku_classify_batch_rle_copied(const ku_ctx *ctx) { return ctx ? ctx->last_runs_copied : 0; }

static int rle_run_job(ku_ctx *ctx, RleJob &j, const RleBatch &b, bool to_end, uint64_t *n_runs) {
  for (int attempt = 0;; ++attempt) {
    bool classified = false;
    int st = rle_job_enqueue(ctx, j, b);
    if (to_end && st == KU_OK) st = rle_job_finish(ctx, j, n_runs, &classified);
    if (to_end) j.busy = false;
    if (st != KU_ENOMEM || attempt || !(ctx->sp.on && !(b.o.flags & KU_F_NO_COUNTS))) return st;
    sparse_give_up(ctx);
    if (classified) return KU_OK;
  }
}

extern "C" int ku_classify_batch_rle_enqueue(ku_ctx *ctx, const char *seqs, uint64_t n_bytes, const uint64_t *seq_off,
                                             const uint32_t *seq_len, uint64_t n_reads, const ku_opts *opts, uint32_t *calls,
                                             uint32_t *hits, uint64_t *run_off, uint32_t *run_cnt, ku_run *runs, uint64_t runs_cap) {
  KU_TRY(check_ready(ctx));
  if (ctx->rle_in_flight >= KU_RLE_MAX_IN_FLIGHT)
    return fail(KU_ESTATE, "ku_classify_batch_rle_enqueue: " + std::to_string(KU_RLE_MAX_IN_FLIGHT) + " batches are in flight (ku_classify_batch_rle_finish first)");
  RleBatch b{seqs, n_bytes, seq_off, seq_len, n_reads, opts ? *opts : ku_opts{0, 1, 0, 0}, 0, true, calls, hits, run_cnt, run_off, runs, runs_cap};
  KU_TRY(rle_check_batch(b));
  b.max_n = ku_max_kmers(ctx->m.db.k, b.o.max_read_len);
  RleJob &j = rle_next_job(ctx);
  const bool fused = n_reads && rle_fused_eligible(ctx, b.o.flags, b.max_n, n_bytes, n_reads, b.monotonic);
  const bool in_steps = fused && !(ctx->sp.on && !(b.o.flags & KU_F_NO_COUNTS) && ctx->sp.open);
  if (in_steps) {
    KU_TRY(rle_run_job(ctx, j, b, false, nullptr));
    ++ctx->rle_in_flight;
    return KU_OK;
  }
  if (ctx->rle_in_flight) return fail(KU_ESTATE, "ku_classify_batch_rle_enqueue: this batch takes a path that cannot overlap with the batch in flight "
                                                 "(ku_classify_batch_rle_finish first, then enqueue it again)");
  uint64_t nr = 0;
  ctx->n_runs = 0;
  if (fused) KU_TRY(rle_run_job(ctx, j, b, true, &nr));
  else if (n_reads) {
    KU_TRY(rle_staged_batch(ctx, b, &nr));
    j.runs_in_ctx = true;
  }
  j.settled = true;
  j.busy = true;
  j.n_runs = nr;
  j.runs_copied = 0;
  ++ctx->rle_in_flight;
  return KU_OK;
}

extern "C" int ku_classify_batch_rle_finish(ku_ctx *ctx, uint64_t *n_runs) {
  if (!ctx || !n_runs) return fail(KU_EINVAL, "ku_classify_batch_rle_finish: null argument");
  *n_runs = 0;
  if (!ctx->rle_in_flight) return fail(KU_ESTATE, "ku_classify_batch_rle_finish: no batch is in flight");
  KU_TRY(ctx_activate(ctx));
  RleJob &j = ctx->rle[ctx->rle_head];
  ctx->rle_head = (ctx->rle_head + 1) % KU_RLE_MAX_IN_FLIGHT;
  --ctx->rle_in_flight;
  bool classified = false;
  int st = rle_job_finish(ctx, j, n_runs, &classified);
  j.busy = false;
  if (st == KU_ENOMEM && classified && ctx->sp.on) st = sparse_give_up(ctx);
  return st;
}

extern "C" int ku_classify_batch_rle(ku_ctx *ctx, const char *seqs, uint64_t n_bytes, const uint64_t *seq_off,
                                     const uint32_t *seq_len, uint64_t n_reads, const ku_opts *opts, uint32_t *calls,
                                     uint32_t *hits, uint64_t *run_off, uint32_t *run_cnt, uint64_t *n_runs) {
  if (!n_runs) return fail(KU_EINVAL, "ku_classify_batch_rle: null buffer");
  *n_runs = 0;
  KU_TRY(check_ready(ctx));
  KU_TRY(rle_idle(ctx, "ku_classify_batch_rle"));
  KU_TRY(ku_classify_batch_rle_enqueue(ctx, seqs, n_bytes, seq_off, seq_len, n_reads, opts, calls, hits, run_off, run_cnt, nullptr, 0));
  return ku_classify_batch_rle_finish(ctx, n_runs);
}

extern "C" int ku_ctx_replace_calls(ku_ctx *ctx, const uint32_t *new_calls, uint64_t n_reads, uint64_t *n_dropped) {
  KU_TRY(check_ready(ctx));
  if (n_dropped) *n_dropped = 0;
  if (n_reads == 0) return KU_OK;
  if (!new_calls) return fail(KU_EINVAL, "ku_ctx_replace_calls: null argument");
  KU_TRY(rle_idle(ctx, "ku_ctx_replace_calls"));
  if (!ctx->last_calls_dev) return fail(KU_ESTATE, "ku_ctx_replace_calls: the context holds no batch");
  if (ctx->b_hits.reserve(n_reads * 4) != KU_OK) return fail(KU_ENOMEM, "device batch buffers");
  hipStream_t s = ctx->stream;
  unsigned long long *d_dropped = (unsigned long long *)(ctx->d_scalar + 16);
  HIP_TRY(hipMemsetAsync(d_dropped, 0, 8, s));
  HIP_TRY(hipMemcpyAsync(ctx->b_hits.p, new_calls, n_reads * 4, hipMemcpyHostToDevice, s));
  KU_TRY(ku_launch_replace_calls((const uint32_t *)ctx->last_calls_dev, (const uint32_t *)ctx->b_hits.p, n_reads, ctx->d_node_taxid, ctx->tax.n_nodes,
                                 ctx->cnt.n_reads, d_dropped, s));
  HIP_TRY(hipMemcpyAsync((void *)ctx->last_calls_dev, ctx->b_hits.p, n_reads * 4, hipMemcpyDeviceToDevice, s));
  unsigned long long dropped = 0;
  HIP_TRY(hipMemcpyAsync(&dropped, d_dropped, 8, hipMemcpyDeviceToHost, s));
  HIP_TRY(hipStreamSynchronize(s));
  if (n_dropped) *n_dropped = dropped;
  return KU_OK;
}

extern "C" int ku_fetch_runs(ku_ctx *ctx, ku_run *runs, uint64_t n_runs) {
  if (!ctx) return fail(KU_EINVAL, "ku_fetch_runs: null context");
  if (n_runs > ctx->n_runs) return fail(KU_EINVAL, "ku_fetch_runs: the last batch holds " + std::to_string(ctx->n_runs) + " runs");
  if (n_runs == 0) return KU_OK;
  if (!runs) return fail(KU_EINVAL, "ku_fetch_runs: null buffer");
  if (!ctx->fetch_runs_src) return fail(KU_ESTATE, "ku_fetch_runs: no batch was classified");
  KU_TRY(ctx_activate(ctx));
  if (!ctx->fetch_stream) HIP_TRY(hipStreamCreateWithFlags(&ctx->fetch_stream, hipStreamNonBlocking));
  HIP_TRY(hipMemcpyAsync(runs, ctx->fetch_runs_src, n_runs * 8, hipMemcpyDeviceToHost, ctx->fetch_stream));
  HIP_TRY(hipStreamSynchronize(ctx->fetch_stream));
  return KU_OK;
}
```

krakenuniq_amd/csrc/ku_ctx.h:

```cpp
#pragma once
#include <fcntl.h>
#include <sys/mman.h>
#include <sys/stat.h>
#include <time.h>
#include <unistd.h>

#include <algorithm>
#include <atomic>
#include <mutex>
#include <thread>
#include <cstdio>
#include <cstdlib>
#include <cstring>
#include <string>
#include <unordered_map>
#include <vector>

#include "ku_host.h"
#include "ku_internal.h"

void ku_set_error(const std::string &s);
static inline int fail(int code, const std::string &msg) {
  ku_set_error(msg);
  return code;
// ... 9 lines not shown
  do {                          \
    int s_ = (expr);            \
    if (s_ != KU_OK) return s_; \
  } while (0)

static inline int ensure_stream(hipStream_t &s) { if (!s) HIP_TRY(hipStreamCreateWithFlags(&s, hipStreamNonBlocking)); return KU_OK; }
static inline int ensure_event(hipEvent_t &e, unsigned flags = hipEventDisableTiming) { if (!e) HIP_TRY(hipEventCreateWithFlags(&e, flags)); return KU_OK; }
static inline uint32_t ku_max_kmers(uint32_t k, uint32_t len) { return len >= k ? len - k + 1 : 0; }

struct ku_db {
  const uint8_t *pairs = nullptr;
  const uint64_t *offsets = nullptr;
  ku_db_info info{};
  void *map_kdb = nullptr, *map_idx = nullptr;
  size_t map_kdb_sz = 0, map_idx_sz = 0;
  mutable std::mutex values_mu;
  mutable std::vector<uint32_t> values;
  mutable bool values_ready = false;
};

struct DevBuf {
  void *p = nullptr;
  size_t cap = 0;
  int reserve(size_t bytes) {
    if (bytes <= cap) return KU_OK;
    if (p) (void)hipFree(p);
    p = nullptr; cap = 0;
    size_t want = bytes + bytes / 4 + 256;
    if (hipMalloc(&p, want) != hipSuccess) {
      if (hipMalloc(&p, bytes) != hipSuccess) { p = nullptr; return KU_ENOMEM; }
      want = bytes;
    }
    cap = want;
    return KU_OK;
  }
  void release() { if (p) (void)hipFree(p); p = nullptr; cap = 0; }
};

struct PinBuf {
  void *p = nullptr;
  size_t cap = 0;
  int reserve(size_t bytes) {
    if (bytes <= cap) return KU_OK;
    if (p) (void)hipHostFree(p);
    p = nullptr; cap = 0;
    const size_t want = bytes + bytes / 4 + 256;
    if (hipHostMalloc(&p, want, hipHostMallocDefault) != hipSuccess) { (void)hipGetLastError(); p = nullptr; return KU_ENOMEM; }
    cap = want;
    return KU_OK;
  }
  void release() { if (p) (void)hipHostFree(p); p = nullptr; cap = 0; }
};

struct RleBatch {
  const char *seqs;
  uint64_t n_bytes;
  const uint64_t *seq_off;
  const uint32_t *seq_len;
  uint64_t n_reads;
  ku_opts o;
  uint32_t max_n;
  bool monotonic;
  uint32_t *calls, *hits, *run_cnt;
  uint64_t *run_off;
  ku_run *runs;
  uint64_t runs_cap;
};

struct RleJob {
  DevBuf seqs, off, len, calls, runs, roff, rcnt, ws, unit, u_cnt, u_flag;
  PinBuf pin;
  PinBuf pin_unit;
  unsigned long long *d_counter = nullptr;
  hipEvent_t kernels_done = nullptr, done = nullptr;
  hipEvent_t t_k0 = nullptr, t_k1 = nullptr;
  std::vector<hipEvent_t> seg_events;
  bool busy = false;
  bool settled = false;
  bool runs_in_ctx = false;
  uint64_t runs_copied = 0;
  uint64_t n_runs = 0;
  RleBatch b{};
  uint64_t runs_cap = 0;
  bool sparse = false;
  bool cont_carry = false;
  bool cont_tail = false;
  bool open_after = false;
  uint32_t n_units = 0;
  uint64_t kmers = 0;
  uint64_t acc_after = 0;
  std::vector<uint64_t> unit_first_read;
  std::vector<char> tail_text;
  std::vector<uint32_t> tail_len;
  int reserve(uint64_t n_bytes, uint64_t n_reads, uint64_t runs_cap_, uint64_t ws_bytes, size_t n_seg, bool sparse_, uint64_t units, uint64_t n_slots) {
    if (seqs.reserve(n_bytes + 16) || off.reserve(n_reads * 8) || len.reserve(n_reads * 4) || calls.reserve(n_reads * 4) ||
        runs.reserve(runs_cap_ * 8) || roff.reserve(n_reads * 8) || rcnt.reserve(n_reads * 4) || ws.reserve(ws_bytes))
      return fail(KU_ENOMEM, "device batch buffers");
    units = std::max<uint64_t>(units, 1);
    if (sparse_ && (pin_unit.reserve(n_reads * 4) || unit.reserve(n_reads * 4) || u_cnt.reserve(std::max<uint64_t>(units * n_slots, 1) * 4) ||
                    u_flag.reserve((units + 3) & ~3ull)))
      return fail(KU_ENOMEM, "device memory for the work-unit counters");
    if (pin.reserve(64 + (size_t)units + 64)) return fail(KU_ENOMEM, "page-locked memory for the batch totals");
    KU_TRY(ensure_event(done));
    KU_TRY(ensure_event(kernels_done));
    seg_events.resize(std::max(seg_events.size(), n_seg), nullptr);
    for (hipEvent_t &e : seg_events) KU_TRY(ensure_event(e));
    return KU_OK;
  }
  void release() {
    for (DevBuf *d : {&seqs, &off, &len, &calls, &runs, &roff, &rcnt, &ws, &unit, &u_cnt, &u_flag}) d->release();
    pin.release();
    pin_unit.release();
    for (hipEvent_t *e : {&kernels_done, &done, &t_k0, &t_k1}) { if (*e) (void)hipEventDestroy(*e); *e = nullptr; }
    for (hipEvent_t e : seg_events) if (e) (void)hipEventDestroy(e);
    seg_events.clear();
  }
};

struct DbStore {
  bool db_owned = false, offsets_owned = false;
  bool hash_layout = true;
  bool seen_dirty = false;
  void *d_table = nullptr;
  uint64_t n_dup = 0;
  uint64_t table_lines = 0;
  uint32_t *d_pairs = nullptr;
  uint64_t *d_offsets = nullptr;
  KuDbDev db{};
  std::vector<uint32_t> values;
  std::vector<unsigned long long> slot_counts;
};

struct ku_ctx {
  int device = 0;
  int n_cu = 256;
  hipStream_t stream = nullptr;
  bool db_loaded = false, tax_set = false;
  bool hash_layout = true;
  double load_factor = 0.2;
  bool load_factor_set = false;
  DbStore m;
  std::vector<DbStore> extra;
  std::vector<uint32_t> h_node_taxid, h_slot_taxid;
  uint32_t *d_node_parent = nullptr, *d_node_slot = nullptr, *d_node_taxid = nullptr, *d_slot_node = nullptr,
           *d_slot_taxid = nullptr, *d_slot_anc_off = nullptr, *d_slot_anc = nullptr;
  KuTaxDev tax{};
  KuCountsDev cnt{};
  DevBuf b_seqs, b_off, b_len, b_calls, b_taxa, b_hits, b_ws, b_runs, b_roff, b_rcnt;
  hipStream_t h2d_stream = nullptr, d2h_stream = nullptr, fetch_stream = nullptr;
  hipStream_t k_streams[2] = {nullptr, nullptr};
  hipEvent_t main_ev = nullptr;
  hipEvent_t prev_kernels_done = nullptr;
  uint32_t *d_scalar = nullptr;
  RleJob rle[KU_RLE_MAX_IN_FLIGHT];
  int rle_head = 0, rle_in_flight = 0;
  const void *fetch_runs_src = nullptr;
  const void *last_calls_dev = nullptr;
  uint64_t last_runs_copied = 0;
  std::vector<unsigned long long> count_cache;
  const void *count_cache_store = nullptr, *count_cache_pairs = nullptr;
  uint64_t count_cache_lines = 0;
  uint64_t n_runs = 0;
  unsigned long long *d_exact_set = nullptr, *d_exact_unique = nullptr;
  uint64_t exact_mask = 0;
  struct Prefetch {
    bool valid = false;
    const ku_db *db = nullptr;
    uint64_t bin_lo = 0, bin_hi = 0;
    DbStore store;
    hipStream_t stream = nullptr;
    uint32_t *d_scalar = nullptr;
  } pf;
  struct Sparse {
    bool on = false;
    uint64_t unit_nt = 500000;
    uint64_t acc_nt = 0;
    bool open = false;
    KuSparseDev dev{};
    unsigned long long *d_counters = nullptr;
    DevBuf unit, carry_l, carry_u, out;
    DevBuf u_cnt, u_flag, list;
    uint64_t n_carry_l = 0, n_carry_u = 0, cap_carry_l = 0, cap_carry_u = 0;
    uint64_t g_count = 0;
    bool gave_up = false;
    bool tail_open = false;
    std::vector<char> tail_text;
    std::vector<uint32_t> tail_len;
    DevBuf tail_row;
    DevBuf t_seqs, t_off, t_len, t_taxa, t_unit;
  } sp;
};


struct ku_batch {
  ku_ctx *ctx = nullptr;
  uint64_t n_bytes = 0, n_reads = 0;
  uint32_t max_len = 0;
  bool finished = false;
  void *d_seqs = nullptr;
  uint64_t *d_off = nullptr;
  uint32_t *d_len = nullptr, *d_taxa = nullptr;
  std::vector<uint64_t> h_off;
  std::vector<uint32_t> h_len;
};

int ctx_activate(ku_ctx *ctx);
int ctx_sync_all_streams(ku_ctx *ctx);
void store_free(DbStore &d);
void ctx_drop_count_cache(ku_ctx *ctx);
void ctx_free_sparse(ku_ctx *ctx);
int sparse_give_up(ku_ctx *ctx, hipStream_t also = nullptr);
int store_upload(ku_ctx *ctx, DbStore &d, const ku_db *db, uint64_t bin_lo, uint64_t bin_hi, bool scan_values = true, hipStream_t stream = nullptr);
bool store_whole(const DbStore &d);
int store_finalize(ku_ctx *ctx, DbStore &d, hipStream_t stream = nullptr, uint32_t *d_scalar = nullptr);
int sparse_reserve_global(ku_ctx *ctx, uint64_t incoming, hipStream_t s);
int sparse_pass_tables(ku_ctx *ctx, uint64_t n_entries, KuSparseDev *view, hipStream_t s);
int sparse_pass(ku_ctx *ctx, const void *d_seqs, const uint64_t *d_off, const uint32_t *d_len, const uint64_t *h_off, const uint32_t *h_len, uint64_t n_reads, uint64_t n_bytes, const uint32_t *d_taxa, uint32_t quick_min_hits, hipStream_t s);
int sparse_close_open_unit(ku_ctx *ctx);
int ctx_seen_harvest(ku_ctx *ctx);
int check_ready(ku_ctx *ctx);
int classify_device_impl(ku_ctx *ctx, const void *d_seqs, uint64_t n_bytes, const uint64_t *d_seq_off, const uint32_t *d_seq_len, uint64_t n_reads, const ku_opts *opts, uint32_t *d_calls, uint32_t *d_taxa, uint32_t *d_hits, void *stream, const uint64_t *h_off, const uint32_t *h_len);
int rle_and_fetch(ku_ctx *ctx, const uint32_t *d_taxa, const uint64_t *d_off, const uint32_t *d_len, uint64_t n_reads, uint64_t runs_cap, bool quick, uint32_t *calls, uint32_t *hits, uint64_t *run_off, uint32_t *run_cnt, uint64_t *n_runs);
int sparse_tail_to_carry(ku_ctx *ctx);
int sparse_tail_close(ku_ctx *ctx);
void rle_times_print();
int rle_idle(const ku_ctx *ctx, const char *who);
int rle_drain_batches(ku_ctx *ctx);
```

krakenuniq_amd/csrc/ku_internal.h:

```cpp
#pragma once
#include <hip/hip_runtime.h>
#include <stdint.h>

#include <string>

#include "../../include/krakenuniq_amd.h"

struct KuDbDev {
  const uint32_t *pairs;
  const uint4 *table;
  uint64_t n_lines;
  const uint64_t *offsets;
  uint64_t pair_base;
  uint64_t n_pairs;
  uint64_t bin_lo, bin_hi;
  uint32_t k, nt;
  uint32_t xor_mask;
  uint32_t pad;
};

struct KuTaxDev {
  const uint32_t *node_parent;
  const uint32_t *node_slot;
  const uint32_t *node_taxid;
// ... 20 lines not shown
#define KU_ROUTE_MAX_RECORDS ((1u << 27) - 2u)
__host__ __device__ static inline uint32_t ku_route_maxn(uint32_t k, uint32_t nt) {
  const uint32_t w = k - nt + 1, room = 57u - k;
  const uint32_t a = w < room ? w : room;
  return a < 31u ? a : 31u;
}
struct KuRouteDev {
  const uint64_t *own_lo, *own_hi;
  unsigned long long *cursor;
  uint4 *q_rec;
  uint64_t cap;
  uint32_t world;
  uint32_t chunk;
};
struct KuSparseDev {
  unsigned long long *l_key;
  uint32_t *l_first;
  uint64_t l_mask;
  unsigned long long *u_key;
  uint32_t *u_distinct, *u_last, *u_maxfirst;
  uint64_t u_mask;
  unsigned long long *g_key;
  uint64_t g_mask;
  uint32_t *dense;
  uint32_t *err;
  unsigned long long *g_count;
};
#define KU_SPARSE_MAX_UNITS 16000u
#define KU_SPARSE_MAX_SLOTS (1u << 18)
int ku_launch_sparse_insert(const KuSparseDev &s, uint32_t k, const uint8_t *d_seqs, const uint64_t *d_seq_off,
                            const uint32_t *d_seq_len, const uint32_t *d_unit, uint64_t n_reads, const uint32_t *d_taxa,
                            uint32_t quick_min_hits, int n_cu, hipStream_t stream);
int ku_launch_sparse_clear(const KuSparseDev &s, hipStream_t stream);
int ku_launch_zero3(void *a, uint64_t a_dwords, void *b, uint64_t b_dwords, void *c, uint64_t c_dwords, hipStream_t stream);
int ku_launch_add_u32(uint32_t *dst, const uint32_t *src, uint64_t n, hipStream_t stream);
int ku_launch_sparse_close(const KuSparseDev &s, uint32_t n_closed, hipStream_t stream, bool skip_hits = false);
int ku_launch_sparse_carry_out(const KuSparseDev &s, uint32_t unit, unsigned long long *d_carry_l, uint32_t *d_carry_u,
                               unsigned long long *d_counters, uint64_t cap_l, uint64_t cap_u, hipStream_t stream);
int ku_launch_sparse_carry_in(const KuSparseDev &s, const unsigned long long *d_carry_l, uint64_t n_l, const uint32_t *d_carry_u,
                              uint64_t n_u, hipStream_t stream);
int ku_launch_sparse_flag_units(const uint32_t *d_u_cnt, uint64_t n_cells, uint32_t n_slots, const uint32_t *d_dense, uint8_t *d_unit_flag,
                                hipStream_t stream);
int ku_launch_sparse_insert_runs(const KuSparseDev &s, uint32_t k, const uint8_t *d_seqs, const uint64_t *d_seq_off, const uint32_t *d_seq_len,
                                 const uint32_t *d_list_read, const uint32_t *d_list_unit, const uint32_t *d_list_urow, uint64_t n_list,
                                 const void *d_runs, const uint64_t *d_run_off, const uint32_t *d_run_cnt, const uint32_t *d_slot_taxid,
                                 uint32_t n_slots, const uint32_t *d_u_cnt, int n_cu, hipStream_t stream, uint32_t pos_base = 0);
int ku_launch_sparse_rehash(const KuSparseDev &s, const unsigned long long *d_old_keys, uint64_t old_cells, hipStream_t stream);
int ku_launch_sparse_export(const KuSparseDev &s, unsigned long long *d_out, uint64_t cap, unsigned long long *d_counter,
                            hipStream_t stream);
int ku_launch_warm_scratch(int n_cu, hipStream_t stream);
int ku_launch_seen(int what, void *d_table, uint64_t n_lines, const KuSparseDev &s, unsigned long long *d_count, hipStream_t stream);

#define KU_ROLLUP_BINS 80
int ku_launch_rollup_dense(const uint8_t *d_registers, const uint32_t *d_member_off, const uint32_t *d_member_slot,
                           const uint8_t *d_clade_dense, uint32_t n_clades, uint32_t *d_hist, hipStream_t stream);
#define KU_ROLLUP_HOT 48
struct KuRollupPlan {
  const uint32_t *dense;
  const uint32_t *slot_fast;
  const uint32_t *slot_off, *slot_clade;
  const unsigned long long *set_off;
  const uint32_t *set_cells;
  const uint16_t *clade_hot;
  const uint32_t *hot_clades;
  uint32_t n_hot, pad;
  uint32_t *set, *hist, *err;
  const uint32_t *bm_of;
  uint32_t *bm;
};
int ku_launch_rollup_sparse(const unsigned long long *d_g_key, uint64_t g_cells, const KuRollupPlan &plan, int n_cu, hipStream_t stream);
int ku_launch_rollup_table(const void *d_table, uint64_t n_lines, const KuRollupPlan &plan, int n_cu, hipStream_t stream);
#define KU_BM_WORDS (1u << 20)
#define KU_BM_NONE 0xFFFFFFFFu
#define KU_FAST_SKIP 0xFFFFFFFFu
#define KU_FAST_WALK 0xFFFFFFFEu
int ku_launch_bitmap_or_children(uint32_t *d_bm, const uint32_t *d_parents, uint32_t n_parents, const uint32_t *d_child_off,
                                 const uint32_t *d_child, hipStream_t stream);
int ku_launch_bitmap_hist(const uint32_t *d_bm, const uint32_t *d_bm_clade, uint32_t n_bm, uint32_t *d_hist, hipStream_t stream);
int ku_launch_replace_calls(const uint32_t *d_old, const uint32_t *d_new, uint64_t n, const uint32_t *d_node_taxid, uint32_t n_nodes,
                            unsigned long long *d_n_reads, unsigned long long *d_dropped, hipStream_t stream);

struct ku_db;
int ku_db_raw(const ku_db *db, const uint8_t **pairs, const uint64_t **offsets);

struct ku_ctx;
int ku_ctx_sparse_on(const ku_ctx *ctx);
uint64_t ku_ctx_sparse_unit_nt(const ku_ctx *ctx);
int ku_ctx_sparse_pass_slots(ku_ctx *ctx, const void *d_seqs, const uint64_t *d_off, const uint32_t *d_len, const uint64_t *h_off,
                             const uint32_t *h_len, uint64_t n_reads, uint64_t n_bytes, const uint32_t *d_taxa, uint32_t quick_min_hits,
                             hipStream_t s);
int ku_ctx_sparse_move_open_unit(ku_ctx *src, ku_ctx *dst);
int ku_ctx_sparse_finish(ku_ctx *ctx, uint32_t *h_dense);
int ku_ctx_sparse_set_dense(ku_ctx *ctx, const uint32_t *h_dense);
int ku_ctx_sparse_absorb(ku_ctx *dst, ku_ctx *src);
int ku_launch_sparse_absorb(const KuSparseDev &s, const unsigned long long *d_keys, uint64_t n, hipStream_t stream);

int ku_ctx_route_info(const ku_ctx *ctx, uint64_t *bin_lo, uint64_t *bin_hi, int *is_hash, int *single_db);
int ku_ctx_route_scan(ku_ctx *ctx, const void *d_seqs, uint64_t n_bytes, uint32_t *d_taxa, const KuRouteDev &rt, hipStream_t s);
int ku_ctx_route_resolve_prepare(ku_ctx *ctx, const ku_opts *opts, hipStream_t s);
int ku_ctx_route_resolve(ku_ctx *ctx, const uint64_t *d_off, const uint32_t *d_len, uint64_t n_reads, const ku_opts *opts, uint32_t *d_calls,
                         uint32_t *d_taxa, uint32_t *d_hits, const uint32_t *d_kb, const uint32_t *d_ret, hipStream_t s);
int ku_ctx_route_owner(ku_ctx *ctx, const void *d_rec, uint64_t n_rec, const uint32_t *d_kb, uint32_t *d_slots, bool do_counts, hipStream_t s);
struct ku_ctx;
hipStream_t ku_ctx_stream_of(ku_ctx *ctx);
unsigned long long *ku_ctx_exact_unique_of(ku_ctx *ctx);
int ku_ctx_device_of(const ku_ctx *ctx);
int ku_ctx_cus_of(const ku_ctx *ctx);
uint32_t ku_ctx_k_of(const ku_ctx *ctx);
void ku_set_error(const std::string &s);

int ku_launch_lookup(const KuDbDev &db, const KuCountsDev &cnt, const uint8_t *d_seqs, uint64_t n_bytes,
                     uint32_t *d_taxa, bool do_counts, bool prior, bool merge_chunk, int n_cu, hipStream_t stream);
int ku_launch_route_scan(const KuDbDev &db, const uint8_t *d_seqs, uint64_t n_bytes, uint32_t *d_taxa, const KuRouteDev &rt, int n_cu,
                         hipStream_t stream);
unsigned ku_route_scan_grid(uint64_t n_bytes, int n_cu);
uint64_t ku_route_prefix_work_bytes(uint64_t n_rec);
int ku_launch_route_prefix(const void *d_rec, uint64_t n_rec, uint64_t cap, const unsigned long long *d_cursor, uint32_t *d_kb,
                           unsigned long long *d_tot, void *d_work, hipStream_t stream);
int ku_launch_route_owner(const KuDbDev &db, const KuCountsDev &cnt, const void *d_rec, uint64_t n_rec, const uint32_t *d_kb,
                          uint32_t *d_slots, bool do_counts, int n_cu, hipStream_t stream);
int ku_launch_route_gather(uint32_t *d_taxa, uint64_t n, const uint32_t *d_kb, const uint32_t *d_ret, hipStream_t stream);
int ku_launch_lookup_stats(const KuDbDev &db, const uint8_t *d_seqs, uint64_t n_bytes, unsigned long long *d_stats,
                           int n_cu, hipStream_t stream);
int ku_launch_resolve(const KuDbDev &db, const KuTaxDev &tax, const KuCountsDev &cnt, const uint8_t *d_seqs,
                      const uint64_t *d_seq_off, const uint32_t *d_seq_len, uint64_t n_reads, uint32_t flags,
                      uint32_t min_hits, uint32_t max_read_len, uint32_t *d_calls, uint32_t *d_taxa,
                      uint32_t *d_hits, void *d_workspace, uint64_t workspace_bytes, int n_cu,
                      hipStream_t stream);
struct KuRunsOut {
  uint2 *runs;
  unsigned long long *counter;
  unsigned long long cap;
  uint64_t *run_off;
  uint32_t *run_cnt;
  uint32_t chunk;
  uint32_t pre_base1;
};
struct KuSparseFast {
  unsigned long long *g_key;
  uint64_t g_mask;
  unsigned long long *g_count;
  const uint32_t *dense;
  uint32_t *u_cnt;
  const uint32_t *unit_of;
  uint32_t *err;
  uint32_t n_slots;
  uint32_t unit_base;
};
struct KuRouteIn {
  const uint32_t *kb;
  const uint32_t *ret;
};
#define KU_SPARSE_SWITCH_INSERTS 1025u
uint32_t ku_short_max_kmers(const KuDbDev &db);
uint32_t ku_short_max_kmers_windowed(const KuDbDev &db);
uint64_t ku_short_workspace_bytes(uint32_t max_kmers, uint32_t n_slots, uint64_t n_reads, int n_cu);
int ku_launch_classify_short(const KuDbDev &db, const KuTaxDev &tax, const KuCountsDev &cnt, const uint8_t *d_seqs,
                             uint64_t n_bytes, const uint64_t *d_seq_off, const uint32_t *d_seq_len, uint64_t n_reads,
                             uint32_t max_kmers, uint32_t flags, uint32_t *d_calls, uint32_t *d_taxa, uint32_t *d_hits,
                             void *d_workspace, uint64_t workspace_bytes, int n_cu, hipStream_t stream,
                             const KuRunsOut *runs_out = nullptr, const KuSparseFast *sparse = nullptr);
uint32_t ku_route_resolve_max_kmers();
int ku_launch_route_resolve(const KuDbDev &db, const KuTaxDev &tax, const KuCountsDev &cnt, const uint64_t *d_seq_off,
                            const uint32_t *d_seq_len, uint64_t n_reads, uint32_t max_kmers, uint32_t flags, uint32_t *d_calls,
                            uint32_t *d_taxa, uint32_t *d_hits, const uint32_t *d_kb, const uint32_t *d_ret, void *d_workspace,
                            uint64_t workspace_bytes, int n_cu, hipStream_t stream, const KuRunsOut *runs_out = nullptr);
uint64_t ku_short_grid_waves(uint64_t n_reads, uint32_t max_kmers, int n_cu);
uint64_t ku_resolve_workspace_bytes(uint32_t max_read_len, uint32_t k, int n_cu);
int ku_launch_exact(uint32_t k, const uint8_t *d_seqs, const uint64_t *d_seq_off, const uint32_t *d_seq_len, uint64_t n_reads,
                    const uint32_t *d_taxa, unsigned long long *d_set, uint64_t mask, unsigned long long *d_unique,
                    uint32_t *d_overflow, int n_cu, hipStream_t stream, uint32_t quick_min_hits = 0);
int ku_launch_rle(const uint32_t *d_taxa, uint32_t k, const uint64_t *d_seq_off, const uint32_t *d_seq_len,
                  uint64_t n_reads, uint64_t n_bytes, void *d_runs, uint64_t runs_cap, unsigned long long *d_counter,
                  uint64_t *d_run_off, uint32_t *d_run_cnt, int n_cu, hipStream_t stream);
int ku_launch_max_len(const uint32_t *d_seq_len, uint64_t n_reads, uint32_t *d_out, hipStream_t stream);
int ku_launch_quick_chunked(const KuTaxDev &tax, const KuCountsDev &cnt, uint32_t k, const uint64_t *d_seq_off,
                            const uint32_t *d_seq_len, uint64_t n_reads, uint32_t flags, uint32_t min_hits, uint32_t *d_calls,
                            uint32_t *d_taxa, uint32_t *d_hits, int n_cu, hipStream_t stream);
int ku_launch_merge_max_u32(uint32_t *dst, const uint32_t *src, uint64_t n, hipStream_t stream);
int ku_launch_merge_max_u8(uint8_t *dst, const uint8_t *src, uint64_t n, hipStream_t stream);
int ku_launch_replace_u32(uint32_t *p, uint64_t n, uint32_t from, uint32_t to, hipStream_t stream);
#define KU_FOREIGN_MARK 0xFEFEFEFEu
int ku_exact_owned_step(ku_ctx *ctx, const void *d_seqs, const uint64_t *d_off, const uint32_t *d_len, uint64_t n_reads, uint64_t n_bytes,
                        const ku_opts *opts, uint32_t *d_taxa, hipStream_t s);
int ku_launch_merge_add_u64(unsigned long long *dst, const unsigned long long *src, uint64_t n, hipStream_t stream);
int ku_launch_repack(const uint8_t *d_raw, uint64_t n_pairs, uint32_t key_len, uint32_t *d_pairs,
                     hipStream_t stream);
int ku_launch_mark_values(const uint32_t *d_pairs, uint64_t n_pairs, uint32_t *d_bitmap, hipStream_t stream);
int ku_launch_collect_values(const uint32_t *d_bitmap, uint32_t *d_out, uint32_t cap, uint32_t *d_count,
                             hipStream_t stream);
int ku_launch_remap_values(uint32_t *d_pairs, uint64_t n_pairs, const uint32_t *d_slot_taxid, uint32_t n_slots,
                           uint32_t *d_err, hipStream_t stream);
int ku_launch_build_table(const uint32_t *d_pairs, uint64_t n_pairs, void *d_table, uint64_t n_lines, uint32_t k,
                          uint32_t m, uint32_t xor_mask, unsigned long long *d_spilled, hipStream_t stream);
int ku_launch_count_table(const void *d_table, uint64_t n_lines, unsigned long long *d_counts, hipStream_t stream);
int ku_launch_count_slots(const uint32_t *d_pairs, uint64_t n_pairs, unsigned long long *d_counts,
                          uint32_t n_slots, hipStream_t stream);
```

krakenuniq_amd/csrc/ku_short.hip:

```cpp
#include <cstdlib>
#include <type_traits>

#include "ku_device.h"

#define KS_WAVES 4
#ifndef KS_KCT_LOG2
#define KS_KCT_LOG2 8
#endif
#define KS_FLOOR_EVERY 64u
#define KS_HQ 64
#define KS_PAD 16
#ifdef KU_ABLATION
#define KS_ABL(bit) ((ablate & (bit)) != 0)
#else
#define KS_ABL(bit) false
#endif

template <int ITEMS> struct KsGeom {
  static constexpr int MAXN = 64 * ITEMS;
  static constexpr int NWORDS = (MAXN + 31 + 15) / 16 + 3;
  static constexpr int NCODES = (MAXN + 64) / 16 + 4;
  static constexpr int NAMB = (NWORDS + 1) / 2 + 2;
  static constexpr int NMM = MAXN + 64 + 32;
  static constexpr int TCAP_LOG2 = ITEMS <= 2 ? 8 : (ITEMS <= 4 ? 9 : 10);
  static constexpr int KCT_LOG2 = KS_KCT_LOG2;
  static constexpr int RCT_LOG2 = 6;
};

template <int ITEMS, bool WIN, bool SCAN, bool HQ> struct KsWaveLds {
  using G = KsGeom<ITEMS>;
  static constexpr int TCAP = 1 << G::TCAP_LOG2;
  std::conditional_t<HQ, uint2, uint32_t> hq[HQ ? KS_HQ : 0];
  uint32_t codes[SCAN ? G::NCODES : 0];
  uint32_t amb[SCAN ? G::NAMB : 0];
  uint32_t mm[SCAN ? G::NMM : 0];
  uint32_t tkey[TCAP];
  uint32_t tcnt[TCAP];
  uint32_t kk[SCAN ? 1 << G::KCT_LOG2 : 0], kc[SCAN ? 1 << G::KCT_LOG2 : 0];
  uint32_t rk[1 << G::RCT_LOG2], rc[1 << G::RCT_LOG2];
  uint32_t misc[4];
  uint16_t tlist[WIN ? TCAP : G::MAXN];
};

struct __attribute__((packed, aligned(4))) KsQuad {
  uint32_t x, y, z, w;
};
__device__ __forceinline__ uint64_t ks_quad_key(const KsQuad &q) { return ((uint64_t)q.y << 32) | q.x; }
__device__ __forceinline__ uint4 ks_quad_header(const KsQuad &q) { return make_uint4(q.x, q.y, q.z, q.w); }

__device__ __forceinline__ bool ks_less64(uint64_t a, uint64_t b) { return (int64_t)(a - b) < 0; }

__device__ __forceinline__ void ks_wave_sync() {
  __builtin_amdgcn_fence(__ATOMIC_RELEASE, "wavefront");
  __builtin_amdgcn_wave_barrier();
  __builtin_amdgcn_fence(__ATOMIC_ACQUIRE, "wavefront");
}

template <int LOG2>
__device__ __forceinline__ void ks_ct_flush(uint32_t *key, uint32_t *cnt, uint32_t *used, unsigned long long *global,
                                            uint32_t lane, uint32_t *hot = nullptr) {
  ks_wave_sync();
  for (uint32_t i = lane; i < (1u << LOG2); i += 64) {
    uint32_t kk = key[i];
#ifdef KS_DIAG_NOHOT
    if (kk == 1) kk = 0;
#endif
    if (hot && kk == 1) { *hot += cnt[i]; kk = 0; }
    if (kk) atomicAdd(&global[kk - 1], (unsigned long long)cnt[i]);
    key[i] = 0;
    cnt[i] = 0;
  }
  if (lane == 0) *used = 0;
  ks_wave_sync();
}

__device__ __forceinline__ uint32_t ks_bmin4(uint32_t a, uint32_t b) {
  const uint32_t m = ((((a | 0x80808080u) - b) & 0x80808080u) >> 7) * 0xFFu;
  return (b & m) | (a & ~m);
}

#define KS_RCT_SLOT 0x40000000u
__device__ __forceinline__ uint32_t ks_rct_node(uint32_t id, const KuTaxDev &tax) {
  return (id & KS_RCT_SLOT) ? ((id & ~KS_RCT_SLOT) ? tax.slot_node[id & ~KS_RCT_SLOT] : 0u) : id;
}
template <int LOG2>
__device__ __forceinline__ void ks_rct_add(uint32_t *key, uint32_t *cnt, uint32_t *used, uint32_t id, const KuTaxDev &tax,
                                           unsigned long long *global) {
  uint32_t h = (id * 2654435761u) >> (32 - LOG2);
#pragma unroll 1
  for (int probe = 0; probe < 8; ++probe) {
    uint32_t cur = key[h];
    if (cur == 0) { key[h] = id + 1; *used += 1; cur = id + 1; }
    if (cur == id + 1) { cnt[h] += 1; return; }
    h = (h + 1) & ((1u << LOG2) - 1);
  }
  atomicAdd(&global[ks_rct_node(id, tax)], 1ull);
}
template <int LOG2>
__device__ __forceinline__ void ks_rct_flush(uint32_t *key, uint32_t *cnt, uint32_t *used, const KuTaxDev &tax,
                                             unsigned long long *global, uint32_t lane, uint32_t *hot = nullptr) {
  ks_wave_sync();
  for (uint32_t i = lane; i < (1u << LOG2); i += 64) {
    uint32_t kk = key[i];
#ifdef KS_DIAG_NOHOT
    if (kk - 1 == KS_RCT_SLOT) kk = 0;
#endif
    if (hot && kk - 1 == KS_RCT_SLOT) { *hot += cnt[i]; kk = 0; }
    if (kk) atomicAdd(&global[ks_rct_node(kk - 1, tax)], (unsigned long long)cnt[i]);
    key[i] = 0;
    cnt[i] = 0;
  }
  if (lane == 0) *used = 0;
  ks_wave_sync();
}

template <int LOG2, bool TRACK>
__device__ __forceinline__ void ks_tab_add(uint32_t *t_key, uint32_t *t_cnt, uint32_t *n_distinct, uint32_t slot, uint32_t count) {
  uint32_t h = (slot * 2654435761u) >> (32 - LOG2);
  for (;;) {
    uint32_t cur = __hip_atomic_load(&t_key[h], __ATOMIC_RELAXED, __HIP_MEMORY_SCOPE_WORKGROUP);
    if (cur == 0) {
      uint32_t old = atomicCAS(&t_key[h], 0u, slot + 1);
      if (TRACK && old == 0) atomicAdd(n_distinct, 1u);
      cur = old == 0 ? slot + 1 : old;
    }
    if (cur == slot + 1) {
      atomicAdd(&t_cnt[h], count);
      break;
    }
    h = (h + 1) & ((1u << LOG2) - 1);
  }
}

template <int LOG2>
__device__ __forceinline__ uint32_t ks_tab_resolve(uint32_t *t_key, uint32_t *t_cnt, uint16_t *t_list, uint32_t *list_len,
                                                   const KuTaxDev &tax, uint32_t lane, uint32_t *urow = nullptr) {
  constexpr uint32_t TCAP = 1u << LOG2;
  if (lane == 0) *list_len = 0;
  ks_wave_sync();
  for (uint32_t i = lane; i < TCAP; i += 64)
    if (t_key[i]) t_list[atomicAdd(list_len, 1u)] = (uint16_t)i;
  ks_wave_sync();
  const uint32_t n_list = *list_len;
  uint32_t my_max = 0;
  for (uint32_t e = lane; e < n_list; e += 64) {
    const uint32_t pos = t_list[e];
    const uint32_t sl = t_key[pos] - 1;
    if (urow) atomicAdd(&urow[sl], t_cnt[pos] & 0xffffu);
    uint32_t score = 0;
    for (uint32_t i = tax.slot_anc_off[sl], i_end = tax.slot_anc_off[sl + 1]; i < i_end; ++i) {
      const uint32_t s = tax.slot_anc[i];
      uint32_t h = (s * 2654435761u) >> (32 - LOG2);
// ... 24 lines not shown
    res = firstt ? node : ku_lca_nodes(tax.node_parent, res, node);
    firstt = false;
    last = my_min;
  }
  ks_wave_sync();
  for (uint32_t e = lane; e < n_list; e += 64) {
    const uint32_t pos = t_list[e];
    t_key[pos] = 0;
    t_cnt[pos] = 0;
  }
  ks_wave_sync();
  return res;
}

__device__ __forceinline__ uint32_t ks_gload(const uint32_t *p) {
  return __hip_atomic_load(p, __ATOMIC_RELAXED, __HIP_MEMORY_SCOPE_AGENT);
}
__device__ __noinline__ void ks_floor_scan(const uint8_t *registers, uint32_t *hll_floor, uint32_t rs, uint32_t lane) {
  const uint4 *row = reinterpret_cast<const uint4 *>(registers + (size_t)rs * KU_HLL_M) + 4 * lane;
  const uint32_t cur = ks_gload(&hll_floor[rs]);
  uint32_t lo = 0x7f7f7f7fu;
#pragma unroll
  for (int q = 0; q < 4; ++q) {
    const uint4 x = row[q];
    lo = ks_bmin4(lo, ks_bmin4(ks_bmin4(x.x, x.y), ks_bmin4(x.z, x.w)));
  }
  lo = min(min(lo & 0xffu, (lo >> 8) & 0xffu), min((lo >> 16) & 0xffu, lo >> 24));
  lo = ku_wave_min_u32(lo);
  if (lane == 0 && lo > cur) atomicMax(&hll_floor[rs], lo);
}

__device__ __noinline__ void ks_hq_drain(const uint2 *q, uint32_t fill, uint8_t *registers, uint32_t lane) {
  ks_wave_sync();
  if (lane < fill) {
    const uint2 e = q[lane];
    uint8_t *r = registers + (size_t)e.x * KU_HLL_M + (e.y & (KU_HLL_M - 1u));
    ku_hll_raise(r, (uint32_t)*r, e.y >> KU_HLL_P);
  }
  ks_wave_sync();
}

__device__ __noinline__ void ks_spill_add(uint32_t *g_key, uint32_t *g_cnt, uint32_t mask, uint32_t slot, uint32_t count) {
  uint32_t h = (slot * 2654435761u) & mask;
  for (;;) {
    uint32_t cur = ks_gload(&g_key[h]);
    if (cur == 0) {
      uint32_t old = atomicCAS(&g_key[h], 0u, slot + 1);
      cur = old == 0 ? slot + 1 : old;
    }
    if (cur == slot + 1) {
      atomicAdd(&g_cnt[h], count);
      break;
    }
    h = (h + 1) & mask;
  }
}
__device__ __noinline__ void ks_spill_migrate(uint32_t *t_key, uint32_t *t_cnt, uint32_t tcap, uint32_t *g_key, uint32_t *g_cnt,
                                              uint32_t mask, bool wipe, uint32_t lane) {
  if (wipe) {
    for (uint32_t i = lane; i <= mask; i += 64) { g_key[i] = 0; g_cnt[i] = 0; }
    __threadfence();
  }
  ks_wave_sync();
  for (uint32_t i = lane; i < tcap; i += 64) {
    const uint32_t kk = t_key[i];
    if (kk) {
      ks_spill_add(g_key, g_cnt, mask, kk - 1, t_cnt[i] & 0xffffu);
      t_key[i] = 0;
      t_cnt[i] = 0;
    }
  }
  ks_wave_sync();
}
__device__ __noinline__ uint32_t ks_spill_resolve(uint32_t *g_key, uint32_t *g_cnt, uint32_t mask, const uint32_t *slot_anc_off,
                                                  const uint32_t *slot_anc, const uint32_t *slot_node, const uint32_t *node_parent,
                                                  uint32_t lane) {
  __threadfence();
  uint32_t my_max = 0;
  for (uint32_t pos = lane; pos <= mask; pos += 64) {
    const uint32_t kk = ks_gload(&g_key[pos]);
    if (!kk) continue;
    uint32_t score = 0;
    for (uint32_t i = slot_anc_off[kk - 1], i_end = slot_anc_off[kk]; i < i_end; ++i) {
      const uint32_t s = slot_anc[i];
      uint32_t h = (s * 2654435761u) & mask;
      for (;;) {
        const uint32_t cur = ks_gload(&g_key[h]);
        if (cur == s + 1) { score += ks_gload(&g_cnt[h]) & 0xffffu; break; }
        if (cur == 0) break;
        h = (h + 1) & mask;
      }
    }
    atomicAdd(&g_cnt[pos], score << 16);
    my_max = max(my_max, score);
  }
  my_max = ku_wave_max_u32(my_max);
  __threadfence();
  uint32_t last = 0, res = 0;
  bool firstt = true;
  for (;;) {
    uint32_t my_min = 0xFFFFFFFFu;
    for (uint32_t pos = lane; pos <= mask; pos += 64) {
      const uint32_t kk = ks_gload(&g_key[pos]);
      if (kk && (ks_gload(&g_cnt[pos]) >> 16) == my_max && kk - 1 > last) my_min = min(my_min, kk - 1);
    }
    my_min = ku_wave_min_u32(my_min);
    if (my_min == 0xFFFFFFFFu) break;
    const uint32_t node = slot_node[my_min];
    res = firstt ? node : ku_lca_nodes(node_parent, res, node);
    firstt = false;
    last = my_min;
  }
  for (uint32_t pos = lane; pos <= mask; pos += 64)
    if (ks_gload(&g_key[pos])) { g_key[pos] = 0; g_cnt[pos] = 0; }
  __threadfence();
  return res;
}

template <int ITEMS>
__device__ __forceinline__ uint32_t ks_g_insert_items(unsigned long long *g_key, uint64_t g_mask, const uint32_t (&slot)[ITEMS],
                                                      const uint64_t (&hash)[ITEMS], const bool (&want)[ITEMS], uint32_t *err) {
  unsigned long long key[ITEMS], old[ITEMS];
  uint64_t h[ITEMS];
#pragma unroll
  for (int j = 0; j < ITEMS; ++j) {
    key[j] = ((unsigned long long)(slot[j] + 1) << 32) | ks_encode(hash[j]);
    h[j] = ks_mix(key[j]) & g_mask;
  }
#pragma unroll
  for (int j = 0; j < ITEMS; ++j) old[j] = want[j] ? atomicCAS(&g_key[h[j]], 0ull, key[j]) : key[j];
  uint32_t fresh_n = 0;
#pragma unroll
  for (int j = 0; j < ITEMS; ++j) {
    bool fresh = want[j] && old[j] == 0ull;
    if (want[j] && old[j] != 0ull && old[j] != key[j]) {
      bool placed = false;
      for (uint32_t probe = 1; probe < 4096 && !placed; ++probe) {
        h[j] = (h[j] + 1) & g_mask;
        const unsigned long long o = atomicCAS(&g_key[h[j]], 0ull, key[j]);
        fresh = o == 0ull;
        placed = o == 0ull || o == key[j];
      }
      if (!placed) atomicOr(err, 4u);
    }
    fresh_n += (uint32_t)__popcll(__ballot(fresh));
  }
  return fresh_n;
}

#ifndef KS_OCC2
#define KS_OCC2 6
#endif
#define KS_OCC(ITEMS) ((ITEMS) == 2 ? KS_OCC2 : 4)
template <int ITEMS, bool DO_COUNTS, int KK, int MM, bool WIN, int OUT, bool ROUTE = false>
__global__ __launch_bounds__(64 * KS_WAVES, KS_OCC(ITEMS)) void ku_classify_short_kernel(
    KuDbDev db, KuTaxDev tax, KuCountsDev cnt, const uint8_t *__restrict__ seqs, uint64_t n_bytes,
    const uint64_t *__restrict__ seq_off, const uint32_t *__restrict__ seq_len, uint64_t n_reads,
    uint32_t *__restrict__ calls, uint32_t *__restrict__ taxa, uint32_t ablate, uint32_t floor_every,
    uint32_t *__restrict__ spill, uint32_t spill_cap, KuRunsOut ro, KuSparseFast sf, KuRouteIn rin) {
  using G = KsGeom<ITEMS>;
  constexpr uint32_t TCAP = 1u << G::TCAP_LOG2;
  using Lds = KsWaveLds<ITEMS, WIN, !ROUTE, DO_COUNTS && !ROUTE>;
  __shared__ Lds s_w[KS_WAVES];

  const uint32_t lane = threadIdx.x & 63u;
  const uint32_t wv = (uint32_t)__builtin_amdgcn_readfirstlane((int)(threadIdx.x >> 6));
  Lds &sw = s_w[wv];
  uint32_t *codes = sw.codes, *amb = sw.amb, *mmv = sw.mm;
  uint32_t *t_key = sw.tkey, *t_cnt = sw.tcnt;
  uint16_t *t_list = sw.tlist;
  uint16_t *amb16 = reinterpret_cast<uint16_t *>(amb);
  uint32_t *misc = sw.misc;
  const uint32_t k = KK ? (uint32_t)KK : db.k, m = KK ? (uint32_t)MM : db.nt, w = k - m + 1;
  const uint32_t key_shift = ku_key_shift(m);
  const uint32_t *tab = reinterpret_cast<const uint32_t *>(db.table);

  for (uint32_t i = lane; i < TCAP; i += 64) { t_key[i] = 0; t_cnt[i] = 0; }
  if (!ROUTE)
    for (uint32_t i = lane; i < (1u << G::KCT_LOG2); i += 64) { sw.kk[i] = 0; sw.kc[i] = 0; }
  for (uint32_t i = lane; i < (1u << G::RCT_LOG2); i += 64) { sw.rk[i] = 0; sw.rc[i] = 0; }
  if (lane < 4) misc[lane] = 0;
  ks_wave_sync();

  const uint32_t n_waves = gridDim.x * KS_WAVES;
  uint32_t *g_key = WIN ? spill + ((uint64_t)blockIdx.x * KS_WAVES + wv) * 2ull * spill_cap : nullptr;
  uint32_t *g_cnt = WIN ? g_key + spill_cap : nullptr;
  bool spill_used = false;
  unsigned long long ch_pos = 0, ch_end = 0;
  if (OUT != 0 && ro.pre_base1) {
    ch_pos = ((unsigned long long)(ro.pre_base1 - 1u) + (unsigned long long)blockIdx.x * KS_WAVES + wv) * ro.chunk;
    ch_end = ch_pos + ro.chunk;
  }
  auto runs_room = [&](uint32_t need, uint32_t keep, unsigned long long &keep_base) {
    if (ch_pos + need <= ch_end) return;
    const uint32_t want_min = keep ? 2u * (keep + need) : need;
    const uint32_t want = want_min > ro.chunk ? want_min : ro.chunk;
    unsigned long long b = 0;
    if (lane == 0) b = atomicAdd(ro.counter, (unsigned long long)want);
    b = ((unsigned long long)(uint32_t)__builtin_amdgcn_readfirstlane((int)(uint32_t)(b >> 32)) << 32) |
        (uint32_t)__builtin_amdgcn_readfirstlane((int)(uint32_t)b);
    if (keep) {
      __threadfence();
      for (uint32_t i = lane; i < keep; i += 64) {
        if (keep_base + i < ro.cap && b + i < ro.cap) {
          const uint32_t *src = reinterpret_cast<const uint32_t *>(ro.runs + keep_base + i);
          ro.runs[b + i] = make_uint2(ks_gload(src), ks_gload(src + 1));
        }
      }
      keep_base = b;
    }
    ch_pos = b + keep;
    ch_end = b + want;
  };
  uint32_t sp_fresh = 0;
  uint32_t fl_reads =
      floor_every ? (((uint32_t)blockIdx.x * KS_WAVES + wv) * 40503u >> 8) % floor_every : 0u;
  uint32_t fl_scan = 0;
  uint32_t hq_fill = 0;
  uint2 *hq = reinterpret_cast<uint2 *>(sw.hq);
  uint32_t len_n = 0;
  uint64_t off_n = 0;
  {
    const uint64_t r0 = (uint64_t)blockIdx.x * KS_WAVES + wv;
    if (ks_less64(r0, n_reads)) { len_n = seq_len[r0]; off_n = seq_off[r0]; }
  }
  constexpr uint32_t S1_LANES = ROUTE ? 0u : (uint32_t)((G::NWORDS * 4 + 63) / 64) * 64;
  constexpr bool AHEAD = !WIN && !ROUTE && S1_LANES == 64 && OUT != 2;
  uint32_t tx0 = 0, tx1 = 0;
#ifdef KU_ABLATION
  uint32_t tf0 = 0, tf1 = 0;
#endif
  auto text_request = [&](bool first) {
    const bool want = len_n >= k && ks_less64(off_n + len_n + 6, n_bytes);
    const uint32_t *tq = reinterpret_cast<const uint32_t *>(seqs + (off_n & ~3ull)) + (min(4 * lane, (len_n - 1u) & ~3u) >> 2);
    if (!want || (KS_ABL(2048u) && !first)) tq = reinterpret_cast<const uint32_t *>(seq_off);
    tx0 = tq[0];
    tx1 = tq[1];
  };
  if (AHEAD) text_request(true);
  for (uint64_t r = (uint64_t)blockIdx.x * KS_WAVES + wv; ks_less64(r, n_reads); r += n_waves) {
    const uint32_t rlen = len_n;
    const uint64_t roff = off_n;
    {
      const uint64_t rn = r + n_waves;
      const bool more = ks_less64(rn, n_reads);
      len_n = more ? seq_len[rn] : 0u;
      off_n = more ? seq_off[rn] : 0ull;
    }
    const uint32_t n_all = rlen >= k ? rlen - k + 1 : 0;
    uint32_t rd_first = 0, rd_cnt = 0, win0 = 0;
    bool rd_table = false, rd_spill = false;
    uint32_t call_node = 0;
    unsigned long long run_base = 0;
    uint32_t run_n = 0, run_prev = 0;
    bool run_has_prev = false;
    do {
    const uint32_t len = WIN ? min(rlen - win0, (uint32_t)G::MAXN + k - 1) : rlen;
    const uint64_t off = roff + win0;
    const uint32_t n = len >= k ? len - k + 1 : 0;
    if (DO_COUNTS) {
      if (!ROUTE && fl_scan) {
        ks_floor_scan(cnt.registers, cnt.hll_floor, fl_scan - 1u, lane);
        fl_scan = 0;
      }
      const uint32_t fill_k = misc[0], fill_r = misc[1];
      if (!ROUTE && fill_k > (1u << G::KCT_LOG2) / 2) ks_ct_flush<G::KCT_LOG2>(sw.kk, sw.kc, &misc[0], cnt.n_kmers, lane);
      if (!WIN || win0 == 0)
        if (fill_r > (1u << G::RCT_LOG2) / 2) ks_rct_flush<G::RCT_LOG2>(sw.rk, sw.rc, &misc[1], tax, cnt.n_reads, lane);
    }
    uint32_t v[ITEMS];
    bool amb_k[ITEMS];
    uint64_t hh[ITEMS];
#pragma unroll
    for (int j = 0; j < ITEMS; ++j) { v[j] = 0; amb_k[j] = false; hh[j] = 0; }

    if (ROUTE) {
      uint32_t tk[ITEMS], kbv[ITEMS];
#pragma unroll
      for (int j = 0; j < ITEMS; ++j) {
        const uint32_t p = j * 64 + lane;
        tk[j] = p < n ? taxa[off + p] : KU_ROUTE_MISS;
      }
#pragma unroll
      for (int j = 0; j < ITEMS; ++j) {
        amb_k[j] = tk[j] == KU_AMBIG;
        kbv[j] = tk[j] < KU_ROUTE_MISS ? rin.kb[tk[j] >> 5] : 0u;
      }
#pragma unroll
      for (int j = 0; j < ITEMS; ++j) v[j] = tk[j] < KU_ROUTE_MISS ? rin.ret[(uint64_t)kbv[j] + (tk[j] & 31u)] : 0u;
    } else if (n > 0) {
      constexpr bool S1_CLAMP = S1_LANES / 4 > (uint32_t)G::NCODES || S1_LANES / 4 > 2u * G::NAMB;
      static_assert(G::NCODES - 1 >= G::NWORDS && 2 * G::NAMB - 1 >= G::NWORDS + 1, "no dump element behind the code words");
      const bool text_inside = ks_less64(off + len + 6, n_bytes);
      const uint32_t *text = reinterpret_cast<const uint32_t *>(seqs + (off & ~3ull));
      const uint32_t text_sh = (uint32_t)off & 3u, last_dw = (len - 1u) & ~3u;
#pragma unroll
      for (uint32_t pl = lane; pl < S1_LANES; pl += 64) {
        const uint32_t b0 = 4 * pl;
        const uint32_t valid = len - min(b0, len);
        uint32_t c8 = 0, a4 = 0xFu;
        if (text_inside) {
          uint32_t d0 = tx0, d1 = tx1;
#ifdef KU_ABLATION
          if (AHEAD && KS_ABL(2048u)) {
            if (ks_less64(r, n_waves)) { tf0 = d0; tf1 = d1; }
            else { d0 = tf0; d1 = tf1; }
          }
#endif
          if (!AHEAD) {
            const uint32_t *q = text + (min(b0, last_dw) >> 2);
            d0 = q[0];
            d1 = q[1];
          }
          ku_pack_dword(__builtin_amdgcn_alignbyte(d1, d0, text_sh), c8, a4);
        } else if (b0 < len) {
          const uint64_t a = off + b0;
          uint32_t d = 0;
          for (uint32_t j = 0; j < 4; ++j) d |= (a + j < n_bytes ? (uint32_t)seqs[a + j] : (uint32_t)'N') << (8 * j);
          ku_pack_dword(d, c8, a4);
        }
        if (valid < 4) a4 |= (1u << (4 - valid)) - 1u;
        const uint32_t q4 = pl & 3u;
        uint32_t word = c8 << (24 - 8 * q4), ab = a4 << (12 - 4 * q4);
        word |= ku_quad_xor1(word);
        ab |= ku_quad_xor1(ab);
        word |= ku_quad_xor2(word);
        ab |= ku_quad_xor2(ab);
        const uint32_t wi = pl >> 2;
        codes[S1_CLAMP ? min(wi, (uint32_t)G::NCODES - 1u) : wi] = word;
        amb16[(S1_CLAMP ? min(wi, 2u * G::NAMB - 1u) : wi) ^ 1u] = (uint16_t)ab;
      }
      ks_wave_sync();

      const uint32_t P = n + w - 1;
      uint64_t canon[ITEMS];
      bool is_fwd[ITEMS], ok[ITEMS];
      uint32_t pk[ITEMS + 1], wr[ITEMS + 1];
      uint32_t tacc = 0xFFFFFFFFu;
      bool tie = false;
      static_assert(G::MAXN + 30 + 63 < G::NMM - 1, "the sentinels reach the dump slot");
      mmv[P + lane] = (0x03FFFFFFu - lane) << KU_PK_KEYSHIFT;
      const bool tail_round = P > (uint32_t)ITEMS * 64u;
      pk[ITEMS] = 0;
      wr[ITEMS] = (uint32_t)G::NMM - 1u;
#pragma unroll
      for (int j = 0; j <= ITEMS; ++j) {
        if (j == ITEMS && !tail_round) break;
        const uint32_t p = j * 64 + lane;
        wr[j] = p < P ? p : (uint32_t)G::NMM - 1u;
        const uint32_t wi = p >> 4, sh = (p & 15u) * 2;
        const uint32_t c0 = codes[wi], c1 = codes[wi + 1], c2 = codes[wi + 2];
        const uint64_t x = ((((uint64_t)c0 << 32) | c1) << sh >> 32 << 32) | ((((uint64_t)c1 << 32) | c2) << sh >> 32);
        const uint32_t mm = (uint32_t)(x >> (64 - 2 * m));
        const uint32_t mrc = ku_revcomp32(mm, m);
        pk[j] = ku_pk_make((mm < mrc ? mm : mrc) ^ db.xor_mask, key_shift, mm <= mrc);
        if ((m & 1u) == 0) tie |= p < P && mm == mrc;
        mmv[wr[j]] = pk[j];
        if (j < ITEMS) {
          const uint64_t fwd = x >> (64 - 2 * k);
          const uint64_t rc = ku_revcomp64(fwd, k);
          is_fwd[j] = fwd <= rc;
          canon[j] = is_fwd[j] ? fwd : rc;
          const uint32_t ai = p >> 5, as = p & 31u;
          const uint32_t a = __funnelshift_l(amb[ai + 1], amb[ai], as);
          amb_k[j] = p < n && (a >> (32 - k)) != 0;
          ok[j] = p < n && !amb_k[j];
        }
      }
      ks_wave_sync();

      uint32_t key[ITEMS], aoff[ITEMS];
      bool plus[ITEMS];
      if (KS_ABL(64u)) {
#pragma unroll
        for (int j = 0; j < ITEMS; ++j) { key[j] = 0; aoff[j] = 0; plus[j] = true; }
      } else {
        uint32_t blk = 1;
        uint32_t tj[ITEMS + 1];
#pragma unroll
        for (int j = 0; j <= ITEMS; ++j) tj[j] = 0xFFFFFFFFu;
        auto doubling = [&](auto nr_c) {
          constexpr int NR = decltype(nr_c)::value;
#pragma unroll
          for (uint32_t sft = 0; sft < 5; ++sft) {
            const uint32_t st = 1u << sft;
            if (2 * st > w) break;
            uint32_t nb[NR];
#pragma unroll
            for (int j = 0; j < NR; ++j) nb[j] = mmv[j * 64 + lane + st] + (st << 1);
            ks_wave_sync();
#pragma unroll
            for (int j = 0; j < NR; ++j) {
              tj[j] = min(tj[j], (pk[j] ^ nb[j]) - 2u);
              pk[j] = min(pk[j], nb[j]);
              mmv[wr[j]] = pk[j];
            }
            ks_wave_sync();
            blk = 2 * st;
          }
        };
        if (tail_round) doubling(std::integral_constant<int, ITEMS + 1>{});
        else doubling(std::integral_constant<int, ITEMS>{});
        if (w > blk) {
#pragma unroll
          for (int j = 0; j < ITEMS; ++j) {
            const uint32_t nbj = mmv[j * 64 + lane + (w - blk)] + ((w - blk) << 1);
            tj[j] = min(tj[j], (pk[j] ^ nbj) - 2u);
            pk[j] = min(pk[j], nbj);
          }
        }
#pragma unroll
        for (int j = 0; j <= ITEMS; ++j) tacc = min(tacc, j * 64 + lane < P ? tj[j] : 0xFFFFFFFFu);
        tie |= tacc < (1u << KU_PK_KEYSHIFT) - 2u;
#pragma unroll
        for (int j = 0; j < ITEMS; ++j) {
          const uint32_t t = (pk[j] >> 1) & 31u;
          key[j] = pk[j] >> KU_PK_KEYSHIFT;
          aoff[j] = is_fwd[j] ? t : w - 1 - t;
          plus[j] = ((pk[j] & 1u) != 0) == is_fwd[j];
        }
        if (__any(tie)) {
          ks_wave_sync();
#pragma unroll
          for (int j = 0; j <= ITEMS; ++j) {
            const uint32_t p = j * 64 + lane;
            if (p < P) {
              const uint32_t wi = p >> 4, sh = (p & 15u) * 2;
              const uint64_t two = ((uint64_t)codes[wi] << 32) | codes[wi + 1];
              const uint32_t mm = (uint32_t)((two << sh) >> (64 - 2 * m));
              const uint32_t mrc = ku_revcomp32(mm, m);
              mmv[p] = (mm < mrc ? mm : mrc) ^ db.xor_mask;
            }
          }
          ks_wave_sync();
#pragma unroll
          for (int j = 0; j < ITEMS; ++j) {
            const uint32_t p = j * 64 + lane;
            if (ok[j]) {
              uint32_t bin;
              key[j] = ku_anchor_exact(mmv + p, w, key_shift, is_fwd[j], aoff[j], bin);
              const uint32_t q = p + (is_fwd[j] ? aoff[j] : w - 1 - aoff[j]);
              const uint32_t wi = q >> 4, sh = (q & 15u) * 2;
              const uint64_t two = ((uint64_t)codes[wi] << 32) | codes[wi + 1];
              const uint32_t mmf = (uint32_t)((two << sh) >> (64 - 2 * m));
              const uint32_t rcm = ku_revcomp32(mmf, m);
              plus[j] = is_fwd[j] ? (mmf <= rcm) : (rcm <= mmf);
            }
          }
        }
      }
      const uint32_t *lp[ITEMS];
      uint32_t cand[ITEMS];
      bool act[ITEMS], ovf[ITEMS];
#pragma unroll
      for (int j = 0; j < ITEMS; ++j) {
        const uint64_t locus = ku_locus_assemble(canon[j], key[j], aoff[j], plus[j], k, m);
        hh[j] = ku_fmix64(canon[j]);
        const uint64_t line = ku_locus_line(locus, db.n_lines);
// ... 257 lines not shown
      } else if (!WIN && !KS_ABL(32u)) {
        uint32_t nm = 0;
#pragma unroll
        for (int j = 0; j < ITEMS; ++j) nm += (uint32_t)__popcll(__ballot(j * 64 + lane < n && !amb_k[j] && v[j] == 0));
        if (lane == 0 && nm) atomicAdd(&urow[0], nm);
        any_miss = nm != 0;
      } else {
        unsigned long long miss_any = 0;
#pragma unroll
        for (int j = 0; j < ITEMS; ++j) {
          const bool okc = j * 64 + lane < n && !amb_k[j];
          unsigned long long todo = __ballot(okc);
          while (todo) {
            const uint32_t lead = (uint32_t)__ffsll((long long)todo) - 1u;
            const uint32_t s0 = ku_wave_bcast(v[j], lead);
            const unsigned long long same = __ballot(okc && v[j] == s0);
            if (lane == lead) atomicAdd(&urow[s0], (uint32_t)__popcll(same));
            todo &= ~same;
          }
          miss_any |= __ballot(okc && v[j] == 0);
        }
        any_miss = miss_any != 0;
      }
      if (any_miss && sf.dense[0] == 0 && !KS_ABL(256u)) {
        bool want[ITEMS];
#pragma unroll
        for (int j = 0; j < ITEMS; ++j) want[j] = j * 64 + lane < n && !amb_k[j] && v[j] == 0;
        sp_fresh += ks_g_insert_items<ITEMS>(sf.g_key, sf.g_mask, v, hh, want, sf.err);
      }
    }

    if (uni) {
#pragma unroll
      for (int j = 0; j < ITEMS; ++j) tcode[j] = v[j] ? uni_code : 0u;
    } else if (!AHEAD) {
#pragma unroll
      for (int j = 0; j < ITEMS; ++j) tcode[j] = tax.slot_taxid[v[j]];
    }
    if (OUT == 0) {
#pragma unroll
      for (int j = 0; j < ITEMS; ++j) {
        const uint32_t p = j * 64 + lane;
        if (p < n && !KS_ABL(8u)) taxa[off + p] = amb_k[j] ? KU_AMBIG : tcode[j];
      }
    } else {
      unsigned long long sm[ITEMS];
      uint32_t carry = run_prev, w_runs = 0;
#pragma unroll
      for (int j = 0; j < ITEMS; ++j) {
        tcode[j] = amb_k[j] ? KU_AMBIG : tcode[j];
        uint32_t up = ku_wave_up1(tcode[j]);
        if (lane == 0) up = carry;
        const bool first = j == 0 && lane == 0 && !run_has_prev;
        sm[j] = __ballot(j * 64 + lane < n && (tcode[j] != up || first));
        w_runs += (uint32_t)__popcll(sm[j]);
        carry = (uint32_t)__builtin_amdgcn_readlane((int)tcode[j], 63);
      }
      if (!WIN || run_n == 0) {
        unsigned long long none = 0;
        runs_room(w_runs, 0u, none);
        run_base = ch_pos;
      } else {
        runs_room(w_runs, run_n, run_base);
      }
      uint32_t before = 0;
#pragma unroll
      for (int j = 0; j < ITEMS; ++j) {
        const unsigned long long at = ch_pos + before + (uint32_t)__popcll(sm[j] & ((1ull << lane) - 1ull));
        if (((sm[j] >> lane) & 1ull) && at < ro.cap) ro.runs[at] = make_uint2(tcode[j], win0 + j * 64 + lane);
        before += (uint32_t)__popcll(sm[j]);
      }
      ch_pos += w_runs;
      run_n += w_runs;
      run_prev = carry;
      run_has_prev = true;
    }
    if (!WIN) {
      if (OUT != 0 && lane == 0) {
        ro.run_off[r] = run_base;
        ro.run_cnt[r] = run_n;
      }
      if (lane == 0) {
        calls[r] = uni || AHEAD ? uni_code : tax.node_taxid[call_node];
        if (DO_COUNTS) ks_rct_add<G::RCT_LOG2>(sw.rk, sw.rc, &misc[1], uni ? (KS_RCT_SLOT | uni_slot) : call_node, tax, cnt.n_reads);
      }
      ks_wave_sync();
      break;
    }
    uint32_t nxt = win0 + (uint32_t)G::MAXN;
    if (!ROUTE && nxt < n_all) {
      uint32_t last1 = 0;
      if (lane < (uint32_t)G::NAMB) {
        const uint32_t lo = 32u * lane;
        uint32_t wd = lo < len ? amb[lane] : 0u;
        if (len - lo < 32u && lo < len) wd &= ~0u << (32u - (len - lo));
        if (wd) last1 = lo + 32u - (uint32_t)__builtin_ctz(wd);
      }
      last1 = ku_wave_max_u32(last1);
      if (last1 > (uint32_t)G::MAXN) {
        const uint32_t skip_to = min(win0 + last1, n_all);
        if (OUT == 0) {
          if (nxt + lane < skip_to) taxa[roff + nxt + lane] = KU_AMBIG;
        } else if (skip_to > nxt && run_prev != KU_AMBIG) {
          runs_room(1u, run_n, run_base);
          if (lane == 0 && ch_pos < ro.cap) ro.runs[ch_pos] = make_uint2(KU_AMBIG, nxt);
          ch_pos += 1;
          run_n += 1;
          run_prev = KU_AMBIG;
        }
        nxt = skip_to;
      }
    }
    ks_wave_sync();
    win0 = nxt;
    } while (win0 < n_all);
    if (WIN) {
      uint32_t code;
      if (!rd_table) code = rd_first ? tax.slot_taxid[rd_first] : 0u;
      else {
        call_node = rd_spill ? ks_spill_resolve(g_key, g_cnt, spill_cap - 1, tax.slot_anc_off, tax.slot_anc, tax.slot_node, tax.node_parent, lane)
                             : ks_tab_resolve<G::TCAP_LOG2>(t_key, t_cnt, t_list, &misc[2], tax, lane);
        if (lane == 0) misc[3] = 0;
        code = tax.node_taxid[call_node];
      }
      if (lane == 0) {
        calls[r] = code;
        if (OUT != 0) {
          ro.run_off[r] = run_base;
          ro.run_cnt[r] = run_n;
        }
        if (DO_COUNTS) ks_rct_add<G::RCT_LOG2>(sw.rk, sw.rc, &misc[1], rd_table ? call_node : (KS_RCT_SLOT | rd_first), tax, cnt.n_reads);
      }
      ks_wave_sync();
    }
  }
#ifndef KS_DIAG_NOFLUSH
  if (DO_COUNTS) {
    ks_wave_sync();
    if (lane < 2) misc[2 + lane] = 0;
    if (!ROUTE && hq_fill) ks_hq_drain(hq, hq_fill, cnt.registers, lane);
    if (!ROUTE && fl_scan) ks_floor_scan(cnt.registers, cnt.hll_floor, fl_scan - 1u, lane);
    if (!ROUTE) ks_ct_flush<G::KCT_LOG2>(sw.kk, sw.kc, &misc[0], cnt.n_kmers, lane, &misc[2]);
    ks_rct_flush<G::RCT_LOG2>(sw.rk, sw.rc, &misc[1], tax, cnt.n_reads, lane, &misc[3]);
    __syncthreads();
    if (wv == 0 && lane < 2) {
      unsigned long long sum = 0;
#pragma unroll
      for (int q = 0; q < KS_WAVES; ++q) sum += s_w[q].misc[2 + lane];
      if (sum) atomicAdd(lane == 0 ? &cnt.n_kmers[0] : &cnt.n_reads[0], sum);
    }
  }
#endif
  if (OUT == 2 && lane == 0 && sp_fresh) atomicAdd(sf.g_count, (unsigned long long)sp_fresh);
}

static uint32_t ks_one_pass_max() { return getenv("KU_SHORT_ONE_PASS_MAX") ? (uint32_t)atoi(getenv("KU_SHORT_ONE_PASS_MAX")) : 192u; }
uint32_t ku_short_max_kmers(const KuDbDev &db) {
  const bool whole = db.bin_lo == 0 && db.bin_hi == (1ull << (2 * db.nt));
  return (db.table && whole) ? ks_one_pass_max() : 0;
}
uint32_t ku_short_max_kmers_windowed(const KuDbDev &db) {
  return ku_short_max_kmers(db) ? 65535u : 0u;
}

static unsigned ks_grid(uint64_t n_reads, int items, int n_cu) {
  const char *oe = getenv("KU_SHORT_BLOCKS_PER_CU");
  const uint64_t per_cu = oe ? (uint64_t)atoi(oe) : (n_reads < 500000 ? 1ull : 2ull) * KS_OCC(items);
  const uint64_t want = (n_reads + KS_WAVES - 1) / KS_WAVES, cap = (uint64_t)n_cu * per_cu;
  return (unsigned)(want < cap ? want : cap);
}
static uint32_t ks_spill_cap(uint32_t max_kmers, uint32_t n_slots) {
  const uint32_t distinct = max_kmers < n_slots ? max_kmers : n_slots;
  uint32_t cap = 1024;
  while (cap < 2 * distinct) cap <<= 1;
  return cap;
}
uint64_t ku_short_workspace_bytes(uint32_t max_kmers, uint32_t n_slots, uint64_t n_reads, int n_cu) {
  if (max_kmers <= ks_one_pass_max()) return 0;
  return (uint64_t)ks_grid(n_reads, 2, n_cu) * KS_WAVES * 2ull * ks_spill_cap(max_kmers, n_slots) * 4ull;
}

uint64_t ku_short_grid_waves(uint64_t n_reads, uint32_t max_kmers, int n_cu) {
  const bool windowed = max_kmers > ks_one_pass_max();
  return (uint64_t)ks_grid(n_reads, max_kmers <= 128 || windowed ? 2 : 3, n_cu) * KS_WAVES;
}

int ku_launch_classify_short(const KuDbDev &db, const KuTaxDev &tax, const KuCountsDev &cnt, const uint8_t *d_seqs,
                             uint64_t n_bytes, const uint64_t *d_seq_off, const uint32_t *d_seq_len, uint64_t n_reads,
                             uint32_t max_kmers, uint32_t flags, uint32_t *d_calls, uint32_t *d_taxa, uint32_t *d_hits,
                             void *d_workspace, uint64_t workspace_bytes, int n_cu, hipStream_t stream,
                             const KuRunsOut *runs_out, const KuSparseFast *sparse) {
  if (n_reads == 0) return KU_OK;
  const bool counts = !(flags & KU_F_NO_COUNTS);
  if (flags & KU_F_KEEP_SLOTS) return KU_EINVAL;
  if (sparse && (!runs_out || !counts)) return KU_EINVAL;
  if (!runs_out && !d_taxa) return KU_EINVAL;
  if (d_hits && hipMemsetAsync(d_hits, 0, n_reads * 4, stream) != hipSuccess) return KU_EHIP;
  const char *ab = getenv("KU_ABLATE");
  const uint32_t ablate = ab ? (uint32_t)atoi(ab) : 0u;
  const char *fe = getenv("KU_HLL_FLOOR_EVERY");
  const uint32_t floor_every = fe ? (uint32_t)(atoi(fe) > 0 ? atoi(fe) : 0) : KS_FLOOR_EVERY;
  const bool windowed = max_kmers > ks_one_pass_max();
  const int items = max_kmers <= 128 || windowed ? 2 : 3;
  const dim3 grid(ks_grid(n_reads, items, n_cu)), block(64 * KS_WAVES);
  uint32_t spill_cap = 0;
  if (windowed) {
    if (max_kmers > 65535u) return KU_EINVAL;
    spill_cap = ks_spill_cap(max_kmers, tax.n_slots);
    if (!d_workspace || workspace_bytes < (uint64_t)grid.x * KS_WAVES * 2ull * spill_cap * 4ull) return KU_EINVAL;
  }
  const KuRunsOut ro = runs_out ? *runs_out : KuRunsOut{};
  const KuSparseFast sf = sparse ? *sparse : KuSparseFast{};
  const int out = sparse ? 2 : (runs_out ? 1 : 0);
#define KS_LAUNCH(I, C, K, M, W, O)                                                                                          \
  hipLaunchKernelGGL((ku_classify_short_kernel<I, C, K, M, W, O>), grid, block, 0, stream, db, tax, cnt, d_seqs, n_bytes,    \
                     d_seq_off, d_seq_len, n_reads, d_calls, d_taxa, ablate, floor_every, (uint32_t *)d_workspace, spill_cap, ro, sf,   \
                     KuRouteIn{})
  const int geo = !counts || db.k != 31 ? 0 : (db.nt == 13 ? 13 : (db.nt == 15 ? 15 : 0));
#define KS_GEO(I, W, O)                                      \
  do {                                                       \
    if (!counts) KS_LAUNCH(I, false, 0, 0, W, (O) == 2 ? 1 : (O)); \
    else if (geo == 13) KS_LAUNCH(I, true, 31, 13, W, O);    \
    else if (geo == 15) KS_LAUNCH(I, true, 31, 15, W, O);    \
    else KS_LAUNCH(I, true, 0, 0, W, O);                     \
  } while (0)
#define KS_OUT(I, W)                  \
  do {                                \
    if (out == 0) KS_GEO(I, W, 0);    \
    else if (out == 1) KS_GEO(I, W, 1); \
    else KS_GEO(I, W, 2);             \
  } while (0)
  if (windowed) KS_OUT(2, true);
  else if (max_kmers <= 128) KS_OUT(2, false);
  else KS_OUT(3, false);
#undef KS_OUT
#undef KS_GEO
#undef KS_LAUNCH
  return hipGetLastError() == hipSuccess ? KU_OK : KU_EHIP;
}

uint32_t ku_route_resolve_max_kmers() { return 65535u; }
int ku_launch_route_resolve(const KuDbDev &db, const KuTaxDev &tax, const KuCountsDev &cnt, const uint64_t *d_seq_off,
                            const uint32_t *d_seq_len, uint64_t n_reads, uint32_t max_kmers, uint32_t flags, uint32_t *d_calls,
                            uint32_t *d_taxa, uint32_t *d_hits, const uint32_t *d_kb, const uint32_t *d_ret, void *d_workspace,
                            uint64_t workspace_bytes, int n_cu, hipStream_t stream, const KuRunsOut *runs_out) {
  if (n_reads == 0) return KU_OK;
  if (!d_taxa || !d_kb || !d_seq_off || !d_seq_len || !d_calls || max_kmers > 65535u) return KU_EINVAL;
  if (flags & (KU_F_KEEP_SLOTS | KU_F_QUICK)) return KU_EINVAL;
  if (d_hits && hipMemsetAsync(d_hits, 0, n_reads * 4, stream) != hipSuccess) return KU_EHIP;
  const bool counts = !(flags & KU_F_NO_COUNTS), windowed = max_kmers > 128;
  const dim3 grid(ks_grid(n_reads, 2, n_cu)), block(64 * KS_WAVES);
  uint32_t spill_cap = 0;
  if (windowed) {
    spill_cap = ks_spill_cap(max_kmers, tax.n_slots);
    if (!d_workspace || workspace_bytes < (uint64_t)grid.x * KS_WAVES * 2ull * spill_cap * 4ull) return KU_EINVAL;
  }
  const KuRunsOut ro = runs_out ? *runs_out : KuRunsOut{};
  const KuRouteIn rin{d_kb, d_ret};
#define KS_RLAUNCH(C, W, O)                                                                                                     \
  hipLaunchKernelGGL((ku_classify_short_kernel<2, C, 0, 0, W, O, true>), grid, block, 0, stream, db, tax, cnt, (const uint8_t *)nullptr, \
                     (uint64_t)0, d_seq_off, d_seq_len, n_reads, d_calls, d_taxa, 0u, 0u, (uint32_t *)d_workspace, spill_cap, ro, \
                     KuSparseFast{}, rin)
#define KS_RSEL(W, O)                  \
  do {                                 \
    if (counts) KS_RLAUNCH(true, W, O); \
    else KS_RLAUNCH(false, W, O);      \
  } while (0)
  if (windowed) { if (runs_out) KS_RSEL(true, 1); else KS_RSEL(true, 0); }
  else { if (runs_out) KS_RSEL(false, 1); else KS_RSEL(false, 0); }
#undef KS_RSEL
#undef KS_RLAUNCH
  return hipGetLastError() == hipSuccess ? KU_OK : KU_EHIP;
}
```

Before: 623.7.

## Add dynamic chunked read claiming via atomic counter in fused short-read kernel

Replaces the static grid-stride read assignment in the fused short-read classify kernel with dynamic work stealing. Each wave starts with a fixed chunk of reads, then claims further chunks of 32 reads through an atomic counter held in a per-stream device cell. The grid drops to a single round of resident blocks when claiming is on. The last wave to finish resets the cell. This targets load imbalance across waves from uneven read cost, at the price of extra atomics and per-stream cell bookkeeping, and the RLE planning now has to account for flag-dependent grid sizes.

```diff
diff --git a/krakenuniq_amd/csrc/ku_api.cpp b/krakenuniq_amd/csrc/ku_api.cpp
--- a/krakenuniq_amd/csrc/ku_api.cpp
+++ b/krakenuniq_amd/csrc/ku_api.cpp
@@ -327,6 +327,8 @@
   HIP_TRY(hipSetDevice(device));
   HIP_TRY(hipStreamCreateWithFlags(&ctx->stream, hipStreamNonBlocking));
   HIP_TRY(hipMalloc((void **)&ctx->d_scalar, 128));
+  HIP_TRY(hipMalloc((void **)&ctx->claim.d, KU_CLAIM_CELLS * 8));
+  HIP_TRY(hipMemset(ctx->claim.d, 0, KU_CLAIM_CELLS * 8));
   if (const char *e = getenv("KU_LAYOUT")) ctx->hash_layout = strcmp(e, "sorted") != 0;
   if (const char *e = getenv("KU_LOAD_FACTOR")) {
     double f = atof(e);
@@ -411,6 +413,7 @@
                     &ctx->b_roff, &ctx->b_rcnt})
     b->release();
   if (ctx->d_scalar) (void)hipFree(ctx->d_scalar);
+  if (ctx->claim.d) (void)hipFree(ctx->claim.d);
   if (ctx->pf.d_scalar) (void)hipFree(ctx->pf.d_scalar);
   if (ctx->pf.stream) (void)hipStreamDestroy(ctx->pf.stream);
   for (RleJob &j : ctx->rle) j.release();
diff --git a/krakenuniq_amd/csrc/ku_api_classify.cpp b/krakenuniq_amd/csrc/ku_api_classify.cpp
--- a/krakenuniq_amd/csrc/ku_api_classify.cpp
+++ b/krakenuniq_amd/csrc/ku_api_classify.cpp
@@ -159,7 +159,7 @@
     }
     if (fused) {
       int st = ku_launch_classify_short(ctx->m.db, ctx->tax, ctx->cnt, (const uint8_t *)d_seqs, n_bytes, d_seq_off, d_seq_len,
-                                        n_reads, max_n, flags, d_calls, d_taxa, d_hits, ctx->b_ws.p, ctx->b_ws.cap, ctx->n_cu, s);
+                                        n_reads, max_n, flags, d_calls, d_taxa, d_hits, ctx->b_ws.p, ctx->b_ws.cap, ctx->n_cu, s, ctx->claim);
       return st == KU_OK ? KU_OK : fail(st, "fused short-read kernel launch failed");
     }
     ku_opts o = opts ? *opts : ku_opts{0, 1, 0, 0};
diff --git a/krakenuniq_amd/csrc/ku_api_rle.cpp b/krakenuniq_amd/csrc/ku_api_rle.cpp
--- a/krakenuniq_amd/csrc/ku_api_rle.cpp
+++ b/krakenuniq_amd/csrc/ku_api_rle.cpp
@@ -234,7 +234,7 @@
   uint64_t ws = 0;
   uint64_t n_seg() const { return seg.size() - 1; }
 };
-static RlePlan rle_plan(const ku_ctx *ctx, uint64_t n_bytes, uint64_t n_reads, uint32_t max_n, const uint64_t *seq_off, bool test_hook) {
+static RlePlan rle_plan(const ku_ctx *ctx, uint64_t n_bytes, uint64_t n_reads, uint32_t max_n, uint32_t flags, const uint64_t *seq_off, bool test_hook) {
   RlePlan p;
   uint64_t n_seg = 1;
   constexpr uint64_t seg_bytes = 16ull << 20;
@@ -247,7 +247,7 @@
   p.seg[n_seg] = n_reads;
   uint64_t max_seg_reads = 0;
   for (uint64_t g = 0; g < n_seg; ++g) {
-    p.total_waves += ku_short_grid_waves(p.seg[g + 1] - p.seg[g], max_n, ctx->n_cu);
+    p.total_waves += ku_short_grid_waves(p.seg[g + 1] - p.seg[g], max_n, ctx->n_cu, !(flags & KU_F_NO_COUNTS));
     max_seg_reads = std::max(max_seg_reads, p.seg[g + 1] - p.seg[g]);
   }
   const uint64_t reads_per_wave = n_reads / std::max<uint64_t>(p.total_waves, 1);
@@ -258,6 +258,14 @@
   return p;
 }
 
+static RlePlan rle_plan_any_flags(const ku_ctx *ctx, uint64_t n_bytes, uint64_t n_reads, uint32_t max_n) {
+  RlePlan p = rle_plan(ctx, n_bytes, n_reads, max_n, 0, nullptr, false);
+  const RlePlan q = rle_plan(ctx, n_bytes, n_reads, max_n, KU_F_NO_COUNTS, nullptr, false);
+  p.runs_cap = std::max(p.runs_cap, q.runs_cap);
+  p.ws = std::max(p.ws, q.ws);
+  return p;
+}
+
 int rle_idle(const ku_ctx *ctx, const char *who) {
   if (ctx->rle_in_flight) return fail(KU_ESTATE, std::string(who) + ": batches are in flight (ku_classify_batch_rle_finish first)");
   return KU_OK;
@@ -265,7 +273,7 @@
 
 extern "C" uint64_t ku_device_rle_runs_cap(const ku_ctx *ctx, uint64_t n_bytes, uint64_t n_reads, uint32_t max_read_len) {
   if (!ctx || !ctx->tax_set) return 0;
-  return rle_plan(ctx, n_bytes, n_reads, ku_max_kmers(ctx->m.db.k, max_read_len), nullptr, false).runs_cap;
+  return rle_plan_any_flags(ctx, n_bytes, n_reads, ku_max_kmers(ctx->m.db.k, max_read_len)).runs_cap;
 }
 
 extern "C" int ku_classify_batch_device_rle(ku_ctx *ctx, const void *d_seqs, uint64_t n_bytes, const uint64_t *d_seq_off,
@@ -286,7 +294,7 @@
     return fail(KU_EUNSUP, "the sparse-mode emulation runs through the host-buffer entry points (it needs the read lengths on the host)");
   if (!store_whole(ctx->m) || !rle_fused_eligible(ctx, o.flags, max_n, n_bytes, n_reads, true))
     return fail(KU_EUNSUP, "ku_classify_batch_device_rle: the fused kernel does not apply to this context / these options (ku_classify_batch_device does)");
-  const RlePlan p = rle_plan(ctx, n_bytes, n_reads, max_n, nullptr, false);
+  const RlePlan p = rle_plan(ctx, n_bytes, n_reads, max_n, o.flags, nullptr, false);
   if (p.ws > ctx->b_ws.cap) HIP_TRY(hipStreamSynchronize(s));
   if (ctx->b_ws.reserve(p.ws)) return fail(KU_ENOMEM, "device memory for the windowed kernel's workspace");
   KuRunsOut ro{};
@@ -301,7 +309,7 @@
     ro.pre_base1 = 1;
   }
   int st = ku_launch_classify_short(ctx->m.db, ctx->tax, ctx->cnt, (const uint8_t *)d_seqs, n_bytes, d_seq_off, d_seq_len, n_reads, max_n, o.flags,
-                                    d_calls, nullptr, nullptr, ctx->b_ws.p, ctx->b_ws.cap, ctx->n_cu, s, &ro, nullptr);
+                                    d_calls, nullptr, nullptr, ctx->b_ws.p, ctx->b_ws.cap, ctx->n_cu, s, ctx->claim, &ro, nullptr);
   return st == KU_OK ? KU_OK : fail(st, "fused kernel launch failed");
 }
 
@@ -394,7 +402,7 @@
     ro.run_off = (uint64_t *)j.roff.p + a;
     ro.run_cnt = (uint32_t *)j.rcnt.p + a;
     ro.pre_base1 = (uint32_t)(1 + waves_before);
-    waves_before += ku_short_grid_waves(e - a, b.max_n, ctx->n_cu);
+    waves_before += ku_short_grid_waves(e - a, b.max_n, ctx->n_cu, !(b.o.flags & KU_F_NO_COUNTS));
     if (sparse) sf->unit_of = (const uint32_t *)j.unit.p + a;
     if (RleTimes::on && !*clock_started) {
       if (!RleTimes::ref) { KU_TRY(ensure_event(RleTimes::ref, hipEventDefault)); HIP_TRY(hipEventRecord(RleTimes::ref, s)); }
@@ -403,7 +411,7 @@
     }
     int st = ku_launch_classify_short(ctx->m.db, ctx->tax, ctx->cnt, (const uint8_t *)j.seqs.p, b.n_bytes, (const uint64_t *)j.off.p + a,
                                       (const uint32_t *)j.len.p + a, e - a, b.max_n, b.o.flags, (uint32_t *)j.calls.p + a, nullptr, nullptr,
-                                      j.ws.p, j.ws.cap, ctx->n_cu, s, &ro, sf);
+                                      j.ws.p, j.ws.cap, ctx->n_cu, s, ctx->claim, &ro, sf);
     if (st != KU_OK) { (void)hipStreamSynchronize(ctx->h2d_stream); (void)hipStreamSynchronize(s); return fail(st, "fused kernel launch failed"); }
   }
   return KU_OK;
@@ -477,7 +485,7 @@
   KuSparseFast sf{};
   {
     RleTimes::Lap lap{g_rle.t[5]};
-    p = rle_plan(ctx, b.n_bytes, b.n_reads, b.max_n, b.monotonic ? b.seq_off : nullptr, true);
+    p = rle_plan(ctx, b.n_bytes, b.n_reads, b.max_n, b.o.flags, b.monotonic ? b.seq_off : nullptr, true);
     KU_TRY(plan_work_units(ctx, j, b, sparse));
     KU_TRY(j.reserve(b.n_bytes, b.n_reads, p.runs_cap, p.ws, p.n_seg(), sparse, j.n_units, ctx->tax.n_slots));
     KU_TRY(ensure_stream(ctx->h2d_stream));
@@ -532,7 +540,7 @@
     if (ctx->b_ws.reserve(rle_workspace_bytes(ctx, j.b.max_n, j.b.n_reads))) return fail(KU_ENOMEM, "device batch buffers");
     int st = ku_launch_classify_short(ctx->m.db, ctx->tax, ctx->cnt, (const uint8_t *)j.seqs.p, j.b.n_bytes, (const uint64_t *)j.off.p,
                                       (const uint32_t *)j.len.p, j.b.n_reads, j.b.max_n, j.b.o.flags | KU_F_NO_COUNTS, (uint32_t *)ctx->b_calls.p,
-                                      (uint32_t *)ctx->b_taxa.p, nullptr, ctx->b_ws.p, ctx->b_ws.cap, ctx->n_cu, s);
+                                      (uint32_t *)ctx->b_taxa.p, nullptr, ctx->b_ws.p, ctx->b_ws.cap, ctx->n_cu, s, ctx->claim);
     if (st != KU_OK) return fail(st, "fused kernel launch failed");
     KU_TRY(rle_and_fetch(ctx, (const uint32_t *)ctx->b_taxa.p, (const uint64_t *)j.off.p, (const uint32_t *)j.len.p, j.b.n_reads, j.b.n_bytes + 1,
                          false, j.b.calls, nullptr, j.b.run_off, j.b.run_cnt, n_runs));
@@ -676,7 +684,7 @@
   KU_TRY(ensure_stream(ctx->h2d_stream));
   KU_TRY(ensure_stream(ctx->d2h_stream));
   KU_TRY(ensure_stream(ctx->fetch_stream));
-  const RlePlan p = rle_plan(ctx, n_bytes, n_reads, ku_max_kmers(ctx->m.db.k, max_read_len), nullptr, false);
+  const RlePlan p = rle_plan_any_flags(ctx, n_bytes, n_reads, ku_max_kmers(ctx->m.db.k, max_read_len));
   const bool sparse = ctx->sp.on && ctx->sp.unit_nt;
   const uint64_t n_units = sparse ? n_bytes / ctx->sp.unit_nt + 2 : 0;
   for (uint32_t q = 0; q < std::min<uint32_t>(n_jobs, KU_RLE_MAX_IN_FLIGHT); ++q)
diff --git a/krakenuniq_amd/csrc/ku_ctx.h b/krakenuniq_amd/csrc/ku_ctx.h
--- a/krakenuniq_amd/csrc/ku_ctx.h
+++ b/krakenuniq_amd/csrc/ku_ctx.h
@@ -185,6 +185,7 @@
   hipEvent_t main_ev = nullptr;
   hipEvent_t prev_kernels_done = nullptr;
   uint32_t *d_scalar = nullptr;
+  KuClaimCells claim;
   RleJob rle[KU_RLE_MAX_IN_FLIGHT];
   int rle_head = 0, rle_in_flight = 0;
   const void *fetch_runs_src = nullptr;
diff --git a/krakenuniq_amd/csrc/ku_internal.h b/krakenuniq_amd/csrc/ku_internal.h
--- a/krakenuniq_amd/csrc/ku_internal.h
+++ b/krakenuniq_amd/csrc/ku_internal.h
@@ -196,20 +196,33 @@
   const uint32_t *ret;
 };
 #define KU_SPARSE_SWITCH_INSERTS 1025u
+#define KU_CLAIM_CELLS 32
+struct KuClaimCells {
+  uint32_t *d = nullptr;
+  hipStream_t owner[KU_CLAIM_CELLS] = {};
+  int n_bound = 0;
+  uint32_t *cell(hipStream_t stream) {
+    for (int i = 0; i < n_bound; ++i)
+      if (owner[i] == stream) return d + 2 * i;
+    if (!d || n_bound == KU_CLAIM_CELLS) return nullptr;
+    owner[n_bound] = stream;
+    return d + 2 * n_bound++;
+  }
+};
 uint32_t ku_short_max_kmers(const KuDbDev &db);
 uint32_t ku_short_max_kmers_windowed(const KuDbDev &db);
 uint64_t ku_short_workspace_bytes(uint32_t max_kmers, uint32_t n_slots, uint64_t n_reads, int n_cu);
 int ku_launch_classify_short(const KuDbDev &db, const KuTaxDev &tax, const KuCountsDev &cnt, const uint8_t *d_seqs,
                              uint64_t n_bytes, const uint64_t *d_seq_off, const uint32_t *d_seq_len, uint64_t n_reads,
                              uint32_t max_kmers, uint32_t flags, uint32_t *d_calls, uint32_t *d_taxa, uint32_t *d_hits,
-                             void *d_workspace, uint64_t workspace_bytes, int n_cu, hipStream_t stream,
+                             void *d_workspace, uint64_t workspace_bytes, int n_cu, hipStream_t stream, KuClaimCells &cells,
                              const KuRunsOut *runs_out = nullptr, const KuSparseFast *sparse = nullptr);
 uint32_t ku_route_resolve_max_kmers();
 int ku_launch_route_resolve(const KuDbDev &db, const KuTaxDev &tax, const KuCountsDev &cnt, const uint64_t *d_seq_off,
                             const uint32_t *d_seq_len, uint64_t n_reads, uint32_t max_kmers, uint32_t flags, uint32_t *d_calls,
                             uint32_t *d_taxa, uint32_t *d_hits, const uint32_t *d_kb, const uint32_t *d_ret, void *d_workspace,
                             uint64_t workspace_bytes, int n_cu, hipStream_t stream, const KuRunsOut *runs_out = nullptr);
-uint64_t ku_short_grid_waves(uint64_t n_reads, uint32_t max_kmers, int n_cu);
+uint64_t ku_short_grid_waves(uint64_t n_reads, uint32_t max_kmers, int n_cu, bool counts);
 uint64_t ku_resolve_workspace_bytes(uint32_t max_read_len, uint32_t k, int n_cu);
 int ku_launch_exact(uint32_t k, const uint8_t *d_seqs, const uint64_t *d_seq_off, const uint32_t *d_seq_len, uint64_t n_reads,
                     const uint32_t *d_taxa, unsigned long long *d_set, uint64_t mask, unsigned long long *d_unique,
diff --git a/krakenuniq_amd/csrc/ku_short.hip b/krakenuniq_amd/csrc/ku_short.hip
--- a/krakenuniq_amd/csrc/ku_short.hip
+++ b/krakenuniq_amd/csrc/ku_short.hip
@@ -1,3 +1,4 @@
+#include <algorithm>
 #include <cstdlib>
 #include <type_traits>
 
@@ -328,12 +329,16 @@
 #define KS_OCC2 6
 #endif
 #define KS_OCC(ITEMS) ((ITEMS) == 2 ? KS_OCC2 : 4)
+__host__ __device__ constexpr bool ks_claim_instance(int items, bool counts, bool win, int out, bool route) {
+  return !route && (items == 3 || !counts || (!win && out == 0));
+}
 template <int ITEMS, bool DO_COUNTS, int KK, int MM, bool WIN, int OUT, bool ROUTE = false>
 __global__ __launch_bounds__(64 * KS_WAVES, KS_OCC(ITEMS)) void ku_classify_short_kernel(
     KuDbDev db, KuTaxDev tax, KuCountsDev cnt, const uint8_t *__restrict__ seqs, uint64_t n_bytes,
     const uint64_t *__restrict__ seq_off, const uint32_t *__restrict__ seq_len, uint64_t n_reads,
     uint32_t *__restrict__ calls, uint32_t *__restrict__ taxa, uint32_t ablate, uint32_t floor_every,
-    uint32_t *__restrict__ spill, uint32_t spill_cap, KuRunsOut ro, KuSparseFast sf, KuRouteIn rin) {
+    uint32_t *__restrict__ spill, uint32_t spill_cap, KuRunsOut ro, KuSparseFast sf, KuRouteIn rin, uint32_t claim_chunk,
+    uint32_t *__restrict__ cell) {
   using G = KsGeom<ITEMS>;
   constexpr uint32_t TCAP = 1u << G::TCAP_LOG2;
   using Lds = KsWaveLds<ITEMS, WIN, !ROUTE, DO_COUNTS && !ROUTE>;
@@ -359,6 +364,7 @@
   ks_wave_sync();
 
   const uint32_t n_waves = gridDim.x * KS_WAVES;
+  const uint32_t wave_id = blockIdx.x * KS_WAVES + wv;
   uint32_t *g_key = WIN ? spill + ((uint64_t)blockIdx.x * KS_WAVES + wv) * 2ull * spill_cap : nullptr;
   uint32_t *g_cnt = WIN ? g_key + spill_cap : nullptr;
   bool spill_used = false;
@@ -394,17 +400,24 @@
   uint32_t fl_scan = 0;
   uint32_t hq_fill = 0;
   uint2 *hq = reinterpret_cast<uint2 *>(sw.hq);
+  const uint32_t chunk = ks_claim_instance(ITEMS, DO_COUNTS, WIN, OUT, ROUTE) ? claim_chunk : 0u;
+  uint64_t r = chunk ? (uint64_t)(wave_id * chunk) : (uint64_t)wave_id;
+  uint32_t r_next = 0;
+  uint32_t claim_left = chunk;
+  uint32_t claim_v = 0;
+  auto claim_request = [&]() {
+    if (lane == 0) claim_v = atomicAdd(cell, chunk);
+  };
+  if (chunk) claim_request();
   uint32_t len_n = 0;
   uint64_t off_n = 0;
-  {
-    const uint64_t r0 = (uint64_t)blockIdx.x * KS_WAVES + wv;
-    if (ks_less64(r0, n_reads)) { len_n = seq_len[r0]; off_n = seq_off[r0]; }
-  }
+  if (ks_less64(r, n_reads)) { len_n = seq_len[r]; off_n = seq_off[r]; }
   constexpr uint32_t S1_LANES = ROUTE ? 0u : (uint32_t)((G::NWORDS * 4 + 63) / 64) * 64;
   constexpr bool AHEAD = !WIN && !ROUTE && S1_LANES == 64 && OUT != 2;
   uint32_t tx0 = 0, tx1 = 0;
 #ifdef KU_ABLATION
   uint32_t tf0 = 0, tf1 = 0;
+  bool tf_have = false;
 #endif
   auto text_request = [&](bool first) {
     const bool want = len_n >= k && ks_less64(off_n + len_n + 6, n_bytes);
@@ -414,11 +427,20 @@
     tx1 = tq[1];
   };
   if (AHEAD) text_request(true);
-  for (uint64_t r = (uint64_t)blockIdx.x * KS_WAVES + wv; ks_less64(r, n_reads); r += n_waves) {
+  for (; ks_less64(r, n_reads); r = chunk ? (uint64_t)r_next : r + n_waves) {
     const uint32_t rlen = len_n;
     const uint64_t roff = off_n;
     {
-      const uint64_t rn = r + n_waves;
+      uint64_t rn = r + n_waves;
+      if (chunk) {
+        r_next = (uint32_t)r + 1u;
+        if (--claim_left == 0) {
+          r_next = n_waves * chunk + (uint32_t)__builtin_amdgcn_readfirstlane((int)claim_v);
+          claim_request();
+          claim_left = chunk;
+        }
+        rn = r_next;
+      }
       const bool more = ks_less64(rn, n_reads);
       len_n = more ? seq_len[rn] : 0u;
       off_n = more ? seq_off[rn] : 0ull;
@@ -479,7 +501,7 @@
           uint32_t d0 = tx0, d1 = tx1;
 #ifdef KU_ABLATION
           if (AHEAD && KS_ABL(2048u)) {
-            if (ks_less64(r, n_waves)) { tf0 = d0; tf1 = d1; }
+            if (!tf_have) { tf0 = d0; tf1 = d1; tf_have = true; }
             else { d0 = tf0; d1 = tf1; }
           }
 #endif
@@ -1043,6 +1065,15 @@
   }
 #endif
   if (OUT == 2 && lane == 0 && sp_fresh) atomicAdd(sf.g_count, (unsigned long long)sp_fresh);
+  if (chunk) {
+    __threadfence();
+    uint32_t through = 0;
+    if (lane == 0) through = atomicAdd(cell + 1, 1u);
+    if ((uint32_t)__builtin_amdgcn_readfirstlane((int)through) == n_waves - 1u) {
+      __threadfence();
+      if (lane == 0) { cell[0] = 0; cell[1] = 0; }
+    }
+  }
 }
 
 static uint32_t ks_one_pass_max() { return getenv("KU_SHORT_ONE_PASS_MAX") ? (uint32_t)atoi(getenv("KU_SHORT_ONE_PASS_MAX")) : 192u; }
@@ -1054,9 +1085,19 @@
   return ku_short_max_kmers(db) ? 65535u : 0u;
 }
 
-static unsigned ks_grid(uint64_t n_reads, int items, int n_cu) {
+#define KS_CLAIM_CHUNK 32u
+#define KS_CLAIM_MIN_PER_WAVE 768ull
+static uint32_t ks_chunk(uint64_t n_reads, int items, int n_cu, bool claims) {
+  if (!claims || n_reads >= (1ull << 31)) return 0;
+  if (const char *e = getenv("KU_SHORT_CLAIM")) return (uint32_t)std::min(std::max(atoi(e), 0), 4096);
+  if (getenv("KU_SHORT_BLOCKS_PER_CU")) return 0;
+  const uint64_t n_waves = (uint64_t)n_cu * KS_OCC(items) * KS_WAVES;
+  return n_reads < KS_CLAIM_MIN_PER_WAVE * n_waves ? 0u : KS_CLAIM_CHUNK;
+}
+static unsigned ks_grid(uint64_t n_reads, int items, int n_cu, bool claims) {
   const char *oe = getenv("KU_SHORT_BLOCKS_PER_CU");
-  const uint64_t per_cu = oe ? (uint64_t)atoi(oe) : (n_reads < 500000 ? 1ull : 2ull) * KS_OCC(items);
+  const bool one_round = n_reads < 500000 || ks_chunk(n_reads, items, n_cu, claims) != 0;
+  const uint64_t per_cu = oe ? (uint64_t)atoi(oe) : (one_round ? 1ull : 2ull) * KS_OCC(items);
   const uint64_t want = (n_reads + KS_WAVES - 1) / KS_WAVES, cap = (uint64_t)n_cu * per_cu;
   return (unsigned)(want < cap ? want : cap);
 }
@@ -1068,18 +1109,19 @@
 }
 uint64_t ku_short_workspace_bytes(uint32_t max_kmers, uint32_t n_slots, uint64_t n_reads, int n_cu) {
   if (max_kmers <= ks_one_pass_max()) return 0;
-  return (uint64_t)ks_grid(n_reads, 2, n_cu) * KS_WAVES * 2ull * ks_spill_cap(max_kmers, n_slots) * 4ull;
-}
-
-uint64_t ku_short_grid_waves(uint64_t n_reads, uint32_t max_kmers, int n_cu) {
+  return (uint64_t)std::max(ks_grid(n_reads, 2, n_cu, false), ks_grid(n_reads, 2, n_cu, true)) * KS_WAVES * 2ull * ks_spill_cap(max_kmers, n_slots) * 4ull;
+}
+
+uint64_t ku_short_grid_waves(uint64_t n_reads, uint32_t max_kmers, int n_cu, bool counts) {
   const bool windowed = max_kmers > ks_one_pass_max();
-  return (uint64_t)ks_grid(n_reads, max_kmers <= 128 || windowed ? 2 : 3, n_cu) * KS_WAVES;
+  const int items = max_kmers <= 128 || windowed ? 2 : 3;
+  return (uint64_t)ks_grid(n_reads, items, n_cu, ks_claim_instance(items, counts, windowed, 1, false)) * KS_WAVES;
 }
 
 int ku_launch_classify_short(const KuDbDev &db, const KuTaxDev &tax, const KuCountsDev &cnt, const uint8_t *d_seqs,
                              uint64_t n_bytes, const uint64_t *d_seq_off, const uint32_t *d_seq_len, uint64_t n_reads,
                              uint32_t max_kmers, uint32_t flags, uint32_t *d_calls, uint32_t *d_taxa, uint32_t *d_hits,
-                             void *d_workspace, uint64_t workspace_bytes, int n_cu, hipStream_t stream,
+                             void *d_workspace, uint64_t workspace_bytes, int n_cu, hipStream_t stream, KuClaimCells &cells,
                              const KuRunsOut *runs_out, const KuSparseFast *sparse) {
   if (n_reads == 0) return KU_OK;
   const bool counts = !(flags & KU_F_NO_COUNTS);
@@ -1093,7 +1135,12 @@
   const uint32_t floor_every = fe ? (uint32_t)(atoi(fe) > 0 ? atoi(fe) : 0) : KS_FLOOR_EVERY;
   const bool windowed = max_kmers > ks_one_pass_max();
   const int items = max_kmers <= 128 || windowed ? 2 : 3;
-  const dim3 grid(ks_grid(n_reads, items, n_cu)), block(64 * KS_WAVES);
+  const int out = sparse ? 2 : (runs_out ? 1 : 0);
+  const bool claims = ks_claim_instance(items, counts, windowed, out, false);
+  const dim3 grid(ks_grid(n_reads, items, n_cu, claims)), block(64 * KS_WAVES);
+  const uint32_t chunk = ks_chunk(n_reads, items, n_cu, claims);
+  uint32_t *cell = chunk ? cells.cell(stream) : nullptr;
+  if (chunk && !cell) return KU_EINVAL;
   uint32_t spill_cap = 0;
   if (windowed) {
     if (max_kmers > 65535u) return KU_EINVAL;
@@ -1102,11 +1149,10 @@
   }
   const KuRunsOut ro = runs_out ? *runs_out : KuRunsOut{};
   const KuSparseFast sf = sparse ? *sparse : KuSparseFast{};
-  const int out = sparse ? 2 : (runs_out ? 1 : 0);
 #define KS_LAUNCH(I, C, K, M, W, O)                                                                                          \
   hipLaunchKernelGGL((ku_classify_short_kernel<I, C, K, M, W, O>), grid, block, 0, stream, db, tax, cnt, d_seqs, n_bytes,    \
                      d_seq_off, d_seq_len, n_reads, d_calls, d_taxa, ablate, floor_every, (uint32_t *)d_workspace, spill_cap, ro, sf,   \
-                     KuRouteIn{})
+                     KuRouteIn{}, chunk, cell)
   const int geo = !counts || db.k != 31 ? 0 : (db.nt == 13 ? 13 : (db.nt == 15 ? 15 : 0));
 #define KS_GEO(I, W, O)                                      \
   do {                                                       \
@@ -1140,7 +1186,7 @@
   if (flags & (KU_F_KEEP_SLOTS | KU_F_QUICK)) return KU_EINVAL;
   if (d_hits && hipMemsetAsync(d_hits, 0, n_reads * 4, stream) != hipSuccess) return KU_EHIP;
   const bool counts = !(flags & KU_F_NO_COUNTS), windowed = max_kmers > 128;
-  const dim3 grid(ks_grid(n_reads, 2, n_cu)), block(64 * KS_WAVES);
+  const dim3 grid(ks_grid(n_reads, 2, n_cu, false)), block(64 * KS_WAVES);
   uint32_t spill_cap = 0;
   if (windowed) {
     spill_cap = ks_spill_cap(max_kmers, tax.n_slots);
@@ -1151,7 +1197,7 @@
 #define KS_RLAUNCH(C, W, O)                                                                                                     \
   hipLaunchKernelGGL((ku_classify_short_kernel<2, C, 0, 0, W, O, true>), grid, block, 0, stream, db, tax, cnt, (const uint8_t *)nullptr, \
                      (uint64_t)0, d_seq_off, d_seq_len, n_reads, d_calls, d_taxa, 0u, 0u, (uint32_t *)d_workspace, spill_cap, ro, \
-                     KuSparseFast{}, rin)
+                     KuSparseFast{}, rin, 0u, (uint32_t *)nullptr)
 #define KS_RSEL(W, O)                  \
   do {                                 \
     if (counts) KS_RLAUNCH(true, W, O); \
```

Result: faster. 669.3 (median of 6 runs) (+7.3%).
